# guxm2021/SVT_SpeechBrain

Measured on AMD Instinct MI355X. Metric: 10s@16kHz clips/sec encoder+CTC forward, wav2vec2-base, 1/2/4/8 MI355X, higher is better.
Workload: dtype bf16; 1 GPU; wav2vec2-base audio-only AMT forward (encoder + 20-way head + frame decode), 32 x 10 s @16 kHz mono clips per GPU; global_batch=32, per_gpu_batch=32, samples_per_clip=160000, frames_per_clip=499, parallelism=clips sharded over 1 rank(s), streams=2, inputs=resident in HBM

## Files before the change

include/svt_mi355.h:

```cpp
#ifndef SVT_MI355_H
#define SVT_MI355_H

#include <stddef.h>
#include <stdint.h>

#ifdef __cplusplus
extern "C" {
#endif

#define SVT_ABI_VERSION 1
#define SVT_MAX_CONV_LAYERS 8

typedef enum {
  SVT_OK = 0,
  SVT_ERR_INVALID = -1,
  SVT_ERR_KEY = -2,
  SVT_ERR_STATE = -3,
  SVT_ERR_WORKSPACE = -4,
  SVT_ERR_HIP = -5,
  SVT_ERR_NO_DEVICE = -6
} svt_status;

typedef enum { SVT_PREC_FP32 = 0, SVT_PREC_BF16 = 1, SVT_PREC_BF16X3 = 2, SVT_PREC_FP16X3 = 3 } svt_precision;
typedef enum { SVT_NORM_GROUP = 0, SVT_NORM_LAYER = 1 } svt_feat_norm;
typedef enum { SVT_F32 = 0 } svt_dtype;

typedef struct svt_encoder_config {
  int32_t struct_size;
  int32_t hidden_size;
  int32_t num_layers;
  int32_t num_heads;
  int32_t intermediate_size;
  int32_t num_conv_layers;
  int32_t conv_dim[SVT_MAX_CONV_LAYERS];
  int32_t conv_kernel[SVT_MAX_CONV_LAYERS];
  int32_t conv_stride[SVT_MAX_CONV_LAYERS];
  int32_t feat_extract_norm;
  int32_t conv_bias;
  int32_t stable_layer_norm;
  int32_t feat_proj_layer_norm;
  int32_t pos_conv_kernel;
  int32_t pos_conv_groups;
  float layer_norm_eps;
  int32_t normalize_wav;
  int32_t output_norm;
  int32_t precision;
  int32_t pos_conv_depth;
  int32_t rel_pos_buckets;
  int32_t rel_pos_max_distance;
  int32_t pos_conv_batch_norm;
} svt_encoder_config;

typedef struct svt_encoder svt_encoder;
typedef struct svt_linear svt_linear;
typedef struct svt_rca svt_rca;

typedef struct svt_frame {
  float p_on;
  float p_off;
  int32_t octave;
  int32_t pitch_class;
} svt_frame;

const char* svt_last_error(void);
int svt_abi_version(void);
int svt_operand_type(void);
int svt_device_count(void);

int svt_encoder_create(const svt_encoder_config* cfg, int device, svt_encoder** out);
void svt_encoder_destroy(svt_encoder* e);

typedef int (*svt_norm_reduce_fn)(double* sums_dev, int32_t n_doubles, void* stream, void* user);
int svt_encoder_set_norm_reduce(svt_encoder* enc, svt_norm_reduce_fn fn, void* user, int64_t global_clips);
int svt_encoder_load_param(svt_encoder* e, const char* key, const void* data_host, int dtype,
                           const int64_t* shape, int ndim);
int svt_encoder_finalize(svt_encoder* e);
int svt_encoder_get_param(svt_encoder* e, const char* key, void* out_host, int64_t capacity_elems);
int64_t svt_encoder_num_frames(const svt_encoder* e, int64_t n_samples);
int64_t svt_encoder_workspace_bytes(const svt_encoder* e, int32_t batch, int64_t n_samples);
int svt_encoder_forward(svt_encoder* e, const float* wav_dev, int32_t batch, int64_t n_samples,
                        float* feats_dev, void* workspace_dev, size_t workspace_bytes, void* stream);
int svt_encoder_forward_ex(svt_encoder* e, const float* wav_dev, int32_t batch, int64_t n_samples,
                           float* feats_dev, void* workspace_dev, size_t workspace_bytes, void* stream,
                           int32_t clips_per_norm_group);

int svt_encoder_forward_head(svt_encoder* enc, const svt_linear* head, const float* wav_dev, int32_t batch,
                             int64_t n_samples, float* logits_out_dev, svt_frame* frames_out_dev, int32_t n_octave,
                             int32_t n_class, void* workspace_dev, size_t workspace_bytes, void* stream,
                             int32_t clips_per_norm_group);

int svt_linear_create(int32_t in_features, int32_t out_features, int has_bias, int device, svt_linear** out);
void svt_linear_destroy(svt_linear* l);
int svt_linear_load(svt_linear* l, const float* weight_host , const float* bias_host );
int svt_linear_forward(svt_linear* l, const float* x_dev, int64_t rows, float* y_dev, void* stream);
int svt_decode_frames(const float* logits_dev, int64_t rows, int32_t n_out, int32_t n_octave,
                      int32_t n_class, svt_frame* frames_dev, int device, void* stream);
int svt_frames_to_notes(const svt_frame* frames_host, int32_t batch, int64_t frames_per_clip, const int64_t* n_frames,
                        float onset_thres, float offset_thres, double frame_size, int32_t n_octave, int32_t n_class,
                        double* t_on, double* t_off, int32_t* pitch, int32_t* lo, int32_t* hi, int64_t capacity_per_clip,
                        int64_t* n_notes);

int svt_rca_create(int32_t d_model, int32_t nhead, int32_t d_ffn, float alpha, int32_t max_len,
                   int32_t precision, int device, svt_rca** out);
void svt_rca_destroy(svt_rca* r);
int svt_rca_load_param(svt_rca* r, const char* key, const void* data_host, int dtype,
                       const int64_t* shape, int ndim);
int svt_rca_finalize(svt_rca* r);
int64_t svt_rca_workspace_bytes(const svt_rca* r, int32_t batch, int32_t t_audio);
int svt_rca_forward(svt_rca* r, const float* audio_dev, int32_t t_audio, const float* video_dev,
                    int32_t t_video, int32_t batch, float* out_dev, void* workspace_dev,
                    size_t workspace_bytes, void* stream);
int svt_rca_refresh_params(svt_rca* r, const float* const* params_dev, int32_t n, void* stream);
int64_t svt_rca_train_workspace_bytes(const svt_rca* r, int32_t batch, int32_t t_audio);
int svt_rca_forward_train(svt_rca* r, const float* audio_dev, int32_t t_audio, const float* video_dev, int32_t t_video, int32_t batch,
                          float* out_dev, void* workspace_dev, size_t workspace_bytes, void* stream);
int svt_rca_backward(svt_rca* r, const float* dout_dev, int32_t batch, int32_t t_audio, float* const* grads_dev, void* workspace_dev,
                     size_t workspace_bytes, void* stream);

int svt_ctc_greedy(const float* probs_dev, int32_t batch, int32_t t, int32_t v, const float* rel_lens_dev,
                   int32_t blank, int32_t* tokens_dev, int32_t* out_lens_dev, int device, void* stream);

int64_t svt_fbank_workspace_bytes(int32_t batch, int64_t n_samples, int32_t n_fft, int32_t hop, int32_t n_mels);
int svt_fbank(const float* wav_dev, int32_t batch, int64_t n_samples, int32_t sample_rate, int32_t n_fft,
              int32_t win_length, int32_t hop_length, int32_t n_mels, float f_min, float f_max, float top_db,
              float* out_dev, void* workspace_dev, size_t workspace_bytes, int device, void* stream);

int svt_debug_gemm(int32_t precision, const void* a_dev, const void* w_dev, void* c_dev, const float* bias_dev,
                   const float* resid_dev, int32_t m, int32_t n, int32_t k, int32_t a_rpb, int64_t a_bstride,
                   int64_t a_rstride, int64_t ldw, int32_t act, int32_t out_f32, int device, void* stream);

int svt_debug_gemm_pairs(int32_t precision, const float* a_dev, int64_t a_elems, const float* w_dev, float* c_dev, const float* bias_dev,
                         int32_t m, int32_t n, int32_t k, int32_t a_rpb, int64_t a_bstride, int64_t a_rstride, int32_t act,
                         int32_t out_kind, int device, void* stream, int32_t time_iters, float* ms_out);

typedef struct svt_debug_gemm_desc {
  int32_t struct_size;
  const void* a;
  const void* w;
  void* c;
  const float* bias;
  const float* resid;
  int32_t m, n, k;
  int32_t a_rpb;
  int64_t a_bstride, a_rstride;
  int64_t ldw, ldc;
  int32_t nz, nz2;
  int64_t a_z1, a_z2, w_z1, w_z2, c_z1, c_z2, bias_z2;
  float alpha;
  int32_t act, out_f32;
} svt_debug_gemm_desc;
int svt_debug_gemm_batched(int32_t precision, const svt_debug_gemm_desc* d, int device, void* stream);

typedef struct svt_video svt_video;
int svt_video_create(int32_t embed_dim, int32_t precision, int device, svt_video** out);
void svt_video_destroy(svt_video* v);
int svt_video_load_param(svt_video* v, const char* key, const void* data_host, int dtype, const int64_t* shape, int ndim);
int svt_video_finalize(svt_video* v);
int64_t svt_video_workspace_bytes(const svt_video* v, int32_t batch, int32_t t, int32_t h, int32_t w);
int svt_video_keep_workspace(svt_video* v, int keep);
int svt_video_forward(svt_video* v, const float* video_dev, int32_t batch, int32_t t, int32_t h, int32_t w, float* out_dev,
                      void* workspace_dev, size_t workspace_bytes, void* stream);
int svt_video_forward_ex(svt_video* v, const float* video_dev, int32_t batch, int32_t t, int32_t h, int32_t w, float* out_dev, int64_t out_ld,
                         int32_t zero_left, void* workspace_dev, size_t workspace_bytes, void* stream);
typedef struct svt_video_transform { double sub0, div0, mean, std; int32_t crop_h, crop_w; } svt_video_transform;
int svt_video_forward_u8(svt_video* v, const uint8_t* roi_dev, int32_t batch, int32_t t, int32_t h_in, int32_t w_in,
                         const svt_video_transform* tf, float* out_dev, int64_t out_ld, int32_t zero_left, void* workspace_dev,
                         size_t workspace_bytes, void* stream);

int svt_deltas(const float* x_dev, int64_t ldx, int32_t batch, int32_t t, int32_t c, int32_t window_length, float* out_dev,
               int64_t ldo, int device, void* stream);
int svt_context_window(const float* x_dev, int32_t batch, int32_t t, int32_t c, int32_t left_frames, int32_t right_frames,
                       float* out_dev, int device, void* stream);

int svt_bce_loss(const float* logits_dev, int64_t batch, int64_t t_pred, const float* targets_dev, int64_t t_tgt,
                 const float* rel_len_dev, const float* pos_weight_dev, int32_t allowed_len_diff, int32_t reduction,
                 float* out_dev, void* workspace_dev, size_t workspace_bytes, int device, void* stream);
int svt_nll_loss(const float* log_probs_dev, int64_t batch, int64_t t_pred, int32_t n_class, const int64_t* targets_dev,
                 int64_t t_tgt, const float* rel_len_dev, float label_smoothing, int32_t allowed_len_diff,
                 int32_t reduction, float* out_dev, void* workspace_dev, size_t workspace_bytes, int device, void* stream);
int svt_softmax(const float* x_dev, int64_t rows, int32_t n, int32_t apply_log, float* y_dev, int device, void* stream);

int svt_amt_objective_grad(const float* logits_dev, int64_t batch, int64_t t_pred, int32_t n_out, int32_t pitch_octave_num,
                           const float* onset_targets_dev, const float* offset_targets_dev, const int64_t* octave_targets_dev,
                           const int64_t* class_targets_dev, int64_t t_tgt, const float* rel_len_dev, float onset_pos_weight,
                           int32_t allowed_len_diff, float label_smoothing, float* terms_dev, float* terms_host, float* dlogits_dev,
                           void* workspace_dev, size_t* workspace_bytes, int device, void* stream);
int svt_linear_backward(const float* x_dev, const float* dy_dev, int64_t rows, int32_t in_features, int32_t out_features,
                        float* dweight_dev, float* dbias_dev, void* workspace_dev, size_t* workspace_bytes, int device, void* stream);
int svt_linear_backward_data(const float* dy_dev, const float* weight_dev, int64_t rows, int32_t in_features, int32_t out_features,
                             float* dx_dev, int device, void* stream);
int svt_clip_adadelta_step(int32_t n_tensors, float* const* params_dev, float* const* grads_dev, float* const* square_avg_dev,
                           float* const* acc_delta_dev, const int64_t* numels, float lr, double rho, float eps, float weight_decay,
                           int32_t maximize, float max_norm, float* total_norm_dev, void* workspace_dev, size_t* workspace_bytes,
                           int device, void* stream);

int svt_debug_attention(int32_t precision, const void* q, const void* k, const void* v, void* o, int32_t batch, int32_t t,
                        int32_t heads, int32_t head_dim, int64_t ldq, int64_t ldkv, int64_t ldo, float scale, int device,
                        void* stream);
int svt_debug_attention_bias(const void* q, const void* k, const void* v, void* o, int32_t batch, int32_t t, int32_t heads, int64_t ldq,
                             int64_t ldkv, int64_t ldo, float scale, const float* gate_dev, const float* pos_bias_dev, int device,
                             void* stream);
int svt_debug_attention_scores(int32_t precision, const void* q, const void* k, const void* v, void* o, int32_t batch, int32_t t,
                               int32_t heads, int32_t head_dim, int64_t ldq, int64_t ldkv, int64_t ldo, float scale,
                               const float* gate_dev, const float* pos_bias_dev, int device, void* stream);
int svt_debug_rca_wgrad(int32_t precision, const float* dy0, int64_t ldy0, const void* x0, const float* dy1, int64_t ldy1, const void* x1,
                        int64_t rows, int32_t n_out, int32_t n_in, float* dw, float* db, void* workspace_dev, size_t* workspace_bytes,
                        int device, void* stream);
int svt_debug_rca_attn_bwd(int32_t precision, const void* qkv, const void* qc, const void* o_self, const void* o_cross,
                           const float* dblend, float alpha, int32_t batch, int32_t t, int32_t heads, int32_t head_dim, float* dqkv,
                           float* dqc, void* workspace_dev, size_t* workspace_bytes, int device, void* stream);
int svt_debug_set(int key, int value);

int svt_prof_enable(int on);
int svt_prof_reset(void);
int svt_prof_read(int kind, int64_t* launches, double* total_ms, double* total_flops, double* total_bytes);
int svt_debug_clock(int64_t* out_dev, int device, void* stream);
int svt_debug_alloc(void** out, size_t bytes, int device);
int svt_debug_encoder_layout(const svt_encoder* e, int32_t batch, int64_t n_samples, int64_t* offsets, int n);
int svt_debug_free(void* p, int device);

#ifdef __cplusplus
}
#endif
#endif
```

svt_speechbrain_amd/_lib.py:

```python
from __future__ import annotations

import ctypes as C
import os
from typing import Optional

_HERE = os.path.dirname(os.path.abspath(__file__))
LIB_PATH = os.environ.get("SVT_LIB_PATH") or os.path.join(_HERE, "libsvt_mi355.so")
MAX_CONV = 8


class SvtError(RuntimeError):
    pass


class EncoderConfigC(C.Structure):
    _fields_ = [
        ("struct_size", C.c_int32),
        ("hidden_size", C.c_int32),
        ("num_layers", C.c_int32),
        ("num_heads", C.c_int32),
        ("intermediate_size", C.c_int32),
        ("num_conv_layers", C.c_int32),
        ("conv_dim", C.c_int32 * MAX_CONV),
        ("conv_kernel", C.c_int32 * MAX_CONV),
        ("conv_stride", C.c_int32 * MAX_CONV),
        ("feat_extract_norm", C.c_int32),
        ("conv_bias", C.c_int32),
        ("stable_layer_norm", C.c_int32),
        ("feat_proj_layer_norm", C.c_int32),
        ("pos_conv_kernel", C.c_int32),
        ("pos_conv_groups", C.c_int32),
        ("layer_norm_eps", C.c_float),
        ("normalize_wav", C.c_int32),
        ("output_norm", C.c_int32),
        ("precision", C.c_int32),
        ("pos_conv_depth", C.c_int32),
        ("rel_pos_buckets", C.c_int32),
        ("rel_pos_max_distance", C.c_int32),
        ("pos_conv_batch_norm", C.c_int32),
    ]


class VideoTransformC(C.Structure):
    _fields_ = [("sub0", C.c_double), ("div0", C.c_double), ("mean", C.c_double), ("std", C.c_double), ("crop_h", C.c_int32), ("crop_w", C.c_int32)]


class GemmDescC(C.Structure):
    _fields_ = [
        ("struct_size", C.c_int32),
        ("a", C.c_void_p), ("w", C.c_void_p), ("c", C.c_void_p), ("bias", C.c_void_p), ("resid", C.c_void_p),
        ("m", C.c_int32), ("n", C.c_int32), ("k", C.c_int32),
        ("a_rpb", C.c_int32),
        ("a_bstride", C.c_int64), ("a_rstride", C.c_int64),
        ("ldw", C.c_int64), ("ldc", C.c_int64),
        ("nz", C.c_int32), ("nz2", C.c_int32),
        ("a_z1", C.c_int64), ("a_z2", C.c_int64), ("w_z1", C.c_int64), ("w_z2", C.c_int64), ("c_z1", C.c_int64), ("c_z2", C.c_int64),
        ("bias_z2", C.c_int64),
        ("alpha", C.c_float),
        ("act", C.c_int32), ("out_f32", C.c_int32),
    ]


class FrameC(C.Structure):
    _fields_ = [("p_on", C.c_float), ("p_off", C.c_float), ("octave", C.c_int32), ("pitch_class", C.c_int32)]


_P = C.c_void_p
_I64P = C.POINTER(C.c_int64)
NORM_REDUCE_FN = C.CFUNCTYPE(C.c_int, C.c_void_p, C.c_int32, C.c_void_p, C.c_void_p)

SYMBOLS = {
    "svt_last_error": (C.c_char_p, []),
    "svt_abi_version": (C.c_int, []),
    "svt_device_count": (C.c_int, []),
    "svt_encoder_create": (C.c_int, [C.POINTER(EncoderConfigC), C.c_int, C.POINTER(_P)]),
    "svt_encoder_destroy": (None, [_P]),
    "svt_encoder_load_param": (C.c_int, [_P, C.c_char_p, _P, C.c_int, _I64P, C.c_int]),
    "svt_encoder_finalize": (C.c_int, [_P]),
    "svt_encoder_get_param": (C.c_int, [_P, C.c_char_p, _P, C.c_int64]),
    "svt_encoder_num_frames": (C.c_int64, [_P, C.c_int64]),
    "svt_encoder_workspace_bytes": (C.c_int64, [_P, C.c_int32, C.c_int64]),
    "svt_encoder_forward": (C.c_int, [_P, _P, C.c_int32, C.c_int64, _P, _P, C.c_size_t, _P]),
    "svt_encoder_forward_ex": (C.c_int, [_P, _P, C.c_int32, C.c_int64, _P, _P, C.c_size_t, _P, C.c_int32]),
    "svt_encoder_forward_head": (C.c_int, [_P, _P, _P, C.c_int32, C.c_int64, _P, _P, C.c_int32, C.c_int32, _P, C.c_size_t, _P, C.c_int32]),
    "svt_linear_create": (C.c_int, [C.c_int32, C.c_int32, C.c_int, C.c_int, C.POINTER(_P)]),
    "svt_linear_destroy": (None, [_P]),
    "svt_linear_load": (C.c_int, [_P, _P, _P]),
    "svt_linear_forward": (C.c_int, [_P, _P, C.c_int64, _P, _P]),
    "svt_decode_frames": (C.c_int, [_P, C.c_int64, C.c_int32, C.c_int32, C.c_int32, _P, C.c_int, _P]),
    "svt_rca_create": (C.c_int, [C.c_int32, C.c_int32, C.c_int32, C.c_float, C.c_int32, C.c_int32, C.c_int, C.POINTER(_P)]),
    "svt_rca_destroy": (None, [_P]),
    "svt_rca_load_param": (C.c_int, [_P, C.c_char_p, _P, C.c_int, _I64P, C.c_int]),
    "svt_rca_finalize": (C.c_int, [_P]),
    "svt_rca_workspace_bytes": (C.c_int64, [_P, C.c_int32, C.c_int32]),
    "svt_rca_forward": (C.c_int, [_P, _P, C.c_int32, _P, C.c_int32, C.c_int32, _P, _P, C.c_size_t, _P]),
    "svt_rca_refresh_params": (C.c_int, [_P, C.POINTER(_P), C.c_int32, _P]),
    "svt_rca_train_workspace_bytes": (C.c_int64, [_P, C.c_int32, C.c_int32]),
    "svt_rca_forward_train": (C.c_int, [_P, _P, C.c_int32, _P, C.c_int32, C.c_int32, _P, _P, C.c_size_t, _P]),
    "svt_rca_backward": (C.c_int, [_P, _P, C.c_int32, C.c_int32, C.POINTER(_P), _P, C.c_size_t, _P]),
    "svt_ctc_greedy": (C.c_int, [_P, C.c_int32, C.c_int32, C.c_int32, _P, C.c_int32, _P, _P, C.c_int, _P]),
    "svt_fbank_workspace_bytes": (C.c_int64, [C.c_int32, C.c_int64, C.c_int32, C.c_int32, C.c_int32]),
    "svt_fbank": (C.c_int, [_P, C.c_int32, C.c_int64, C.c_int32, C.c_int32, C.c_int32, C.c_int32, C.c_int32,
                            C.c_float, C.c_float, C.c_float, _P, _P, C.c_size_t, C.c_int, _P]),
    "svt_debug_gemm": (C.c_int, [C.c_int32, _P, _P, _P, _P, _P, C.c_int32, C.c_int32, C.c_int32, C.c_int32, C.c_int64,
                                 C.c_int64, C.c_int64, C.c_int32, C.c_int32, C.c_int, _P]),
    "svt_debug_gemm_batched": (C.c_int, [C.c_int32, C.POINTER(GemmDescC), C.c_int, _P]),
    "svt_debug_attention_scores": (C.c_int, [C.c_int32, _P, _P, _P, _P, C.c_int32, C.c_int32, C.c_int32, C.c_int32, C.c_int64, C.c_int64,
                                             C.c_int64, C.c_float, _P, _P, C.c_int, _P]),
    "svt_debug_gemm_pairs": (C.c_int, [C.c_int32, _P, C.c_int64, _P, _P, _P, C.c_int32, C.c_int32, C.c_int32, C.c_int32, C.c_int64,
                                       C.c_int64, C.c_int32, C.c_int32, C.c_int, _P, C.c_int32, C.POINTER(C.c_float)]),
    "svt_video_create": (C.c_int, [C.c_int32, C.c_int32, C.c_int, C.POINTER(C.c_void_p)]),
    "svt_video_destroy": (None, [C.c_void_p]),
    "svt_video_load_param": (C.c_int, [C.c_void_p, C.c_char_p, C.c_void_p, C.c_int, C.POINTER(C.c_int64), C.c_int]),
    "svt_video_finalize": (C.c_int, [C.c_void_p]),
    "svt_video_keep_workspace": (C.c_int, [C.c_void_p, C.c_int]),
    "svt_video_workspace_bytes": (C.c_int64, [C.c_void_p, C.c_int32, C.c_int32, C.c_int32, C.c_int32]),
    "svt_video_forward": (C.c_int, [C.c_void_p, C.c_void_p, C.c_int32, C.c_int32, C.c_int32, C.c_int32, C.c_void_p, C.c_void_p,
                                    C.c_size_t, C.c_void_p]),
    "svt_video_forward_ex": (C.c_int, [C.c_void_p, C.c_void_p, C.c_int32, C.c_int32, C.c_int32, C.c_int32, C.c_void_p, C.c_int64, C.c_int32,
                                       C.c_void_p, C.c_size_t, C.c_void_p]),
    "svt_video_forward_u8": (C.c_int, [C.c_void_p, C.c_void_p, C.c_int32, C.c_int32, C.c_int32, C.c_int32, C.POINTER(VideoTransformC),
                                       C.c_void_p, C.c_int64, C.c_int32, C.c_void_p, C.c_size_t, C.c_void_p]),
    "svt_deltas": (C.c_int, [C.c_void_p, C.c_int64, C.c_int32, C.c_int32, C.c_int32, C.c_int32, C.c_void_p, C.c_int64, C.c_int, C.c_void_p]),
    "svt_context_window": (C.c_int, [C.c_void_p, C.c_int32, C.c_int32, C.c_int32, C.c_int32, C.c_int32, C.c_void_p, C.c_int, C.c_void_p]),
    "svt_bce_loss": (C.c_int, [C.c_void_p, C.c_int64, C.c_int64, C.c_void_p, C.c_int64, C.c_void_p, C.c_void_p, C.c_int32,
                               C.c_int32, C.c_void_p, C.c_void_p, C.c_size_t, C.c_int, C.c_void_p]),
    "svt_nll_loss": (C.c_int, [C.c_void_p, C.c_int64, C.c_int64, C.c_int32, C.c_void_p, C.c_int64, C.c_void_p, C.c_float,
                               C.c_int32, C.c_int32, C.c_void_p, C.c_void_p, C.c_size_t, C.c_int, C.c_void_p]),
    "svt_softmax": (C.c_int, [C.c_void_p, C.c_int64, C.c_int32, C.c_int32, C.c_void_p, C.c_int, C.c_void_p]),
    "svt_amt_objective_grad": (C.c_int, [_P, C.c_int64, C.c_int64, C.c_int32, C.c_int32, _P, _P, _P, _P, C.c_int64, _P, C.c_float,
                                         C.c_int32, C.c_float, _P, C.POINTER(C.c_float), _P, _P, C.POINTER(C.c_size_t), C.c_int, _P]),
    "svt_linear_backward": (C.c_int, [_P, _P, C.c_int64, C.c_int32, C.c_int32, _P, _P, _P, C.POINTER(C.c_size_t), C.c_int, _P]),
    "svt_linear_backward_data": (C.c_int, [_P, _P, C.c_int64, C.c_int32, C.c_int32, _P, C.c_int, _P]),
    "svt_clip_adadelta_step": (C.c_int, [C.c_int32, C.POINTER(_P), C.POINTER(_P), C.POINTER(_P), C.POINTER(_P), _I64P, C.c_float,
                                         C.c_double, C.c_float, C.c_float, C.c_int32, C.c_float, _P, _P, C.POINTER(C.c_size_t), C.c_int,
                                         _P]),
    "svt_debug_attention": (C.c_int, [C.c_int32, C.c_void_p, C.c_void_p, C.c_void_p, C.c_void_p, C.c_int32, C.c_int32,
                                      C.c_int32, C.c_int32, C.c_int64, C.c_int64, C.c_int64, C.c_float, C.c_int, C.c_void_p]),
    "svt_debug_attention_bias": (C.c_int, [C.c_void_p, C.c_void_p, C.c_void_p, C.c_void_p, C.c_int32, C.c_int32, C.c_int32, C.c_int64,
                                           C.c_int64, C.c_int64, C.c_float, C.c_void_p, C.c_void_p, C.c_int, C.c_void_p]),
    "svt_debug_rca_wgrad": (C.c_int, [C.c_int32, _P, C.c_int64, _P, _P, C.c_int64, _P, C.c_int64, C.c_int32, C.c_int32, _P, _P, _P,
                                      C.POINTER(C.c_size_t), C.c_int, _P]),
    "svt_debug_rca_attn_bwd": (C.c_int, [C.c_int32, _P, _P, _P, _P, _P, C.c_float, C.c_int32, C.c_int32, C.c_int32, C.c_int32, _P, _P,
                                         _P, C.POINTER(C.c_size_t), C.c_int, _P]),
    "svt_debug_set": (C.c_int, [C.c_int, C.c_int]),
    "svt_debug_clock": (C.c_int, [C.c_void_p, C.c_int, C.c_void_p]),
    "svt_debug_encoder_layout": (C.c_int, [C.c_void_p, C.c_int32, C.c_int64, C.POINTER(C.c_int64), C.c_int]),
    "svt_operand_type": (C.c_int, []),
    "svt_encoder_set_norm_reduce": (C.c_int, [_P, C.c_void_p, C.c_void_p, C.c_int64]),
    "svt_frames_to_notes": (C.c_int, [C.c_void_p, C.c_int32, C.c_int64, C.c_void_p, C.c_float, C.c_float, C.c_double, C.c_int32, C.c_int32,
                                      C.c_void_p, C.c_void_p, C.c_void_p, C.c_void_p, C.c_void_p, C.c_int64, C.c_void_p]),
    "svt_debug_alloc": (C.c_int, [C.POINTER(C.c_void_p), C.c_size_t, C.c_int]),
    "svt_debug_free": (C.c_int, [C.c_void_p, C.c_int]),
    "svt_prof_enable": (C.c_int, [C.c_int]),
    "svt_prof_reset": (C.c_int, []),
    "svt_prof_read": (C.c_int, [C.c_int, _I64P, C.POINTER(C.c_double), C.POINTER(C.c_double), C.POINTER(C.c_double)]),
}

_lib: Optional[C.CDLL] = None
_libs: dict = {}


def load(variant: str = None) -> C.CDLL:
    global _lib
    key = variant or ""
    if key in _libs:
        return _libs[key]
    if not variant and os.environ.get("SVT_LIB_SUFFIX"):
        variant_path = LIB_PATH.replace("libsvt_mi355.so", f"libsvt_mi355_{os.environ['SVT_LIB_SUFFIX']}.so")
        if not os.path.exists(variant_path):
            raise SvtError(f"SVT_LIB_SUFFIX: {variant_path} not found")
        globals()["LIB_PATH"] = variant_path
    root, ext = os.path.splitext(LIB_PATH)
    path = LIB_PATH if not variant else f"{root}_{variant}{ext}"
    if not os.path.exists(path):
        raise SvtError(
            f"{path} not found: build it with `python -c 'import __graft_entry__ as g; g.build()'` "
            "(or `make -C svt_speechbrain_amd/csrc`). The MI355X path has no CPU fallback.")
    lib = C.CDLL(path)
    for name, (res, args) in SYMBOLS.items():
        fn = getattr(lib, name)
        fn.restype = res
        fn.argtypes = args
    if lib.svt_abi_version() != 1:
        raise SvtError(f"{os.path.basename(path)} ABI version mismatch")
    if lib.svt_operand_type() != (1 if variant == "f16" else 0):
        raise SvtError(f"{os.path.basename(path)} was built for another operand type")
    _libs[key] = lib
    if not variant:
        _lib = lib
    return lib


def last_error(lib: C.CDLL = None) -> str:
    return ((lib or load()).svt_last_error() or b"").decode("utf-8", "replace")


def check(rc: int, what: str = "", lib: C.CDLL = None) -> None:
    if rc != 0:
        raise SvtError(f"{what}: {last_error(lib)} (status {rc})")


def require_gpu() -> None:
    lib = load()
    if lib.svt_device_count() < 1:
        raise SvtError("no gfx950 (MI355X) device is visible: the HIP path cannot run and there is no CPU fallback")


def stream_ptr(device) -> int:
    import torch
    return int(torch.cuda.current_stream(device).cuda_stream)


def dev_index(device) -> int:
    import torch
    d = torch.device(device)
    if d.type != "cuda":
        raise SvtError(f"tensors must live on a ROCm device ('cuda:N'), got {d}")
    return d.index if d.index is not None else torch.cuda.current_device()


def ptr(t) -> int:
    return int(t.data_ptr())
```

svt_speechbrain_amd/csrc/api.hip:

```cpp
#include "../../include/svt_mi355.h"
#include "api.h"
#include "common.h"
#include "host.h"

#include <atomic>
#include <cmath>
#include <cstring>
#include <map>
#include <mutex>
#include <string>
#include <vector>

namespace svt {

int hip_fail(hipError_t e, const char* what, const char* file, int line) {
  set_error(std::string("HIP error ") + hipGetErrorName(e) + " (" + hipGetErrorString(e) + ") at " + file + ":" +
          std::to_string(line) + " in " + what);
  return SVT_ERR_HIP;
}

struct ProfState {
  bool on = false;
  int every = 1;
  unsigned tick = 0;
// ... 136 lines not shown
int begin_upload(bool& uploaded) {
  if (uploaded) SVT_HIP(hipDeviceSynchronize());
  uploaded = true;
  return SVT_OK;
}

bool use_flash(int prec, int dh, bool bias, int64_t T) {
  if (!(prec == 1 && (dh == 64 || dh == 128))) return false;
  return !bias || (dh == 64 && 2 * T - 1 <= 8192);
}
int attn_tp(int prec, int dh, int T, bool bias) {
  return use_flash(prec, dh, bias, T) ? round_up_int(T, 64) : round_up_int(T, 8);
}

int attention_scores_path(int prec, const void* Q, long ldq, const void* K, const void* V, long ldkv, int B,
                          int T, int H, int dh, float scale, const AttnBufs& ab, bool vt_ready, void* out,
                          long ldo, hipStream_t s, const float* gate, const float* relpb, int gp, int o_pairs) {
  if (gp < 0) gp = prec;
  if (gp >= 2 && !gate && flash_attention_x3_ok(dh) && ab.pl_qkv && ldkv == 3L * H * dh &&
      (const float*)V == (const float*)K + (long)H * dh) {
    const long D = (long)H * dh, rows = (long)B * T;
    const float* kv0 = (const float*)K - D;
    const long pl3 = rows * 3 * D;
    unsigned short* p3 = (unsigned short*)ab.pl_qkv;
    if (!vt_ready)
      if (int r = launch_split_planes(gp, kv0, 3 * D, rows, (int)(3 * D), p3, 3 * D, pl3, s)) return r;
    const unsigned short* qp;
    long qld, qpl;
    if ((const float*)Q == kv0 && ldq == 3 * D) { qp = p3; qld = 3 * D; qpl = pl3; }
    else {
      if (!ab.pl_q) { set_error("attention: no workspace for the query planes"); return -1; }
      if (int r = launch_split_planes(gp, (const float*)Q, ldq, rows, (int)D, ab.pl_q, D, rows * D, s)) return r;
      qp = (const unsigned short*)ab.pl_q; qld = D; qpl = rows * D;
    }
    return launch_flash_attention_x3(gp, qp, qld, (long)T * qld, qpl, p3 + D, p3 + 2 * D, 3 * D, (long)T * 3 * D, pl3, (float*)out, ldo,
                                     (long)T * ldo, B, T, H, dh, scale, s, o_pairs);
  }
  if (o_pairs) { set_error("attention: pair-row output is served by the fused split attention only"); return -1; }
  if (use_flash(prec, dh, gate != nullptr, T)) {
    (void)vt_ready;
    return launch_flash_attention(Q, ldq, (long)T * ldq, K, V, ldkv, (long)T * ldkv, out, ldo, (long)T * ldo, B, T, H, dh,
                                  scale, s, gate, gate ? relpb : nullptr);
  }
  const int Tp = round_up_int(T, 8);
  GemmArgs g;
  g.A = Q; g.W = K; g.C = ab.S;
  g.M = T; g.N = T; g.K = dh;
  g.a_rpb = T; g.a_bstride = 0; g.a_rstride = ldq;
  g.ldw = ldkv; g.ldc = Tp;
  g.nz = B * H; g.nz2 = H;
  g.a_z1 = (long)T * ldq; g.a_z2 = dh;
  g.w_z1 = (long)T * ldkv; g.w_z2 = dh;
  g.c_z1 = (long)H * T * Tp; g.c_z2 = (long)T * Tp;
  g.alpha = scale; g.out_f32 = 1;
  if (int r = launch_gemm(gp, g, s)) return r;
  if (gate)
    if (int r = launch_scores_add_relbias(ab.S, (int64_t)B * H, H, T, Tp, gate, relpb, s)) return r;
  if (int r = launch_softmax_rows(prec, ab.S, (int64_t)B * H * T, T, Tp, ab.P, s)) return r;
  if (!vt_ready)
    if (int r = launch_transpose_v(prec, V, B, T, H, dh, ldkv, 0, Tp, ab.Vt, s)) return r;
  GemmArgs o;
  o.A = ab.P; o.W = ab.Vt; o.C = out;
  o.M = T; o.N = dh; o.K = Tp;
  o.a_rpb = T; o.a_rstride = Tp;
  o.ldw = Tp; o.ldc = ldo;
  o.nz = B * H; o.nz2 = H;
  o.a_z1 = (long)H * T * Tp; o.a_z2 = (long)T * Tp;
  o.w_z1 = (long)H * dh * Tp; o.w_z2 = (long)dh * Tp;
  o.c_z1 = (long)T * ldo; o.c_z2 = dh;
  return launch_gemm(gp, o, s);
}

int check_device(int device) {
  int n = 0;
  if (hipGetDeviceCount(&n) != hipSuccess || n <= 0) { set_error("no HIP device visible: the MI355X path cannot run (there is no CPU fallback)"); return SVT_ERR_NO_DEVICE; }
  if (device < 0 || device >= n) { set_error("device index out of range"); return SVT_ERR_INVALID; }
  hipDeviceProp_t prop;
  SVT_HIP(hipGetDeviceProperties(&prop, device));
  if (std::string(prop.gcnArchName).find("gfx950") == std::string::npos) {
    set_error(std::string("device arch is ") + prop.gcnArchName + ", this library is built for gfx950 only");
    return SVT_ERR_NO_DEVICE;
  }
  SVT_HIP(hipSetDevice(device));
  return SVT_OK;
}

int ws_query(const char* who, void* ws, size_t* ws_bytes, size_t need, bool* query) {
  *query = false;
  if (!ws_bytes) { set_error(std::string(who) + ": workspace_bytes is null"); return SVT_ERR_INVALID; }
  if (!ws) { *ws_bytes = need; *query = true; return SVT_OK; }
  if (*ws_bytes < need) {
    set_error(std::string(who) + ": workspace too small (need " + std::to_string(need) + " bytes)");
    return SVT_ERR_WORKSPACE;
  }
  return SVT_OK;
}

int g_debug_keep_split = 0;

}

using namespace svt;

extern "C" {

int svt_abi_version(void) { return SVT_ABI_VERSION; }
int svt_operand_type(void) {
#ifdef SVT_OPERAND_F16
  return 1;
#else
  return 0;
#endif
}
int svt_device_count(void) {
  int n = 0;
  if (hipGetDeviceCount(&n) != hipSuccess) return 0;
  int ok = 0;
  for (int i = 0; i < n; ++i) {
    hipDeviceProp_t prop;
    if (hipGetDeviceProperties(&prop, i) == hipSuccess && std::string(prop.gcnArchName).find("gfx950") != std::string::npos) ++ok;
  }
  return ok;
}

int svt_debug_gemm(int32_t precision, const void* a, const void* w, void* c, const float* bias, const float* resid,
                   int32_t m, int32_t n, int32_t k, int32_t a_rpb, int64_t a_bstride, int64_t a_rstride, int64_t ldw,
                   int32_t act, int32_t out_f32, int device, void* stream) {
  if (!a || !w || !c) { set_error("svt_debug_gemm: null argument"); return SVT_ERR_INVALID; }
  SVT_HIP(hipSetDevice(device));
  GemmArgs g;
  g.A = a; g.W = w; g.C = c; g.bias = bias; g.resid = resid;
  g.M = m; g.N = n; g.K = k; g.a_rpb = a_rpb; g.a_bstride = a_bstride; g.a_rstride = a_rstride;
  g.ldw = ldw; g.ldc = n; g.act = act; g.out_f32 = out_f32;
  static const void* s_kept = nullptr;
  const bool split = precision >= 2 && ldw == k && k % 32 == 0;
  if (split && !(g_debug_keep_split && s_kept == w)) {
    if (split_weights_register(w, n, k, precision, (hipStream_t)stream)) return SVT_ERR_HIP;
    s_kept = w;
  }
  const int rc = launch_gemm(precision, g, (hipStream_t)stream);
  if (split && !g_debug_keep_split) {
    SVT_HIP(hipStreamSynchronize((hipStream_t)stream));
    split_weights_forget(w);
    s_kept = nullptr;
  }
  return rc ? SVT_ERR_INVALID : SVT_OK;
}

int svt_debug_gemm_batched(int32_t precision, const svt_debug_gemm_desc* d, int device, void* stream) {
  if (!d || d->struct_size != (int32_t)sizeof(svt_debug_gemm_desc)) { set_error("svt_debug_gemm_batched: struct_size"); return SVT_ERR_INVALID; }
  if (!d->a || !d->w || !d->c) { set_error("svt_debug_gemm_batched: null argument"); return SVT_ERR_INVALID; }
  if (!valid_precision(precision)) { set_error("svt_debug_gemm_batched: precision"); return SVT_ERR_INVALID; }
  if (d->nz < 1 || d->nz2 < 1 || d->k < 1) { set_error("svt_debug_gemm_batched: nz, nz2 and k must be positive"); return SVT_ERR_INVALID; }
  SVT_HIP(hipSetDevice(device));
  GemmArgs g;
  g.A = d->a; g.W = d->w; g.C = d->c; g.bias = d->bias; g.resid = d->resid;
  g.M = d->m; g.N = d->n; g.K = d->k; g.a_rpb = d->a_rpb; g.a_bstride = d->a_bstride; g.a_rstride = d->a_rstride;
  g.ldw = d->ldw; g.ldc = d->ldc;
  g.nz = d->nz; g.nz2 = d->nz2;
  g.a_z1 = d->a_z1; g.a_z2 = d->a_z2; g.w_z1 = d->w_z1; g.w_z2 = d->w_z2; g.c_z1 = d->c_z1; g.c_z2 = d->c_z2; g.bias_z2 = d->bias_z2;
  g.alpha = d->alpha; g.act = d->act; g.out_f32 = d->out_f32;
  const bool split = precision >= 2 && d->ldw == d->k && d->k % 32 == 0 && d->w_z1 >= 0 && d->w_z2 >= 0;
  if (split) {
    const size_t last_z_row = d->nz > 1 ? ((size_t)(d->nz / d->nz2 - 1) * d->w_z1 + (size_t)(d->nz2 - 1) * d->w_z2) / (size_t)d->k : 0;
    if (split_weights_register(d->w, (long)last_z_row + d->n, d->k, precision, (hipStream_t)stream)) return SVT_ERR_HIP;
  }
  const int rc = launch_gemm(precision, g, (hipStream_t)stream);
  if (split) {
    SVT_HIP(hipStreamSynchronize((hipStream_t)stream));
    split_weights_forget(d->w);
  }
  return rc ? SVT_ERR_INVALID : SVT_OK;
}

int svt_debug_gemm_pairs(int32_t precision, const float* a, int64_t a_elems, const float* w, float* c, const float* bias, int32_t m,
                         int32_t n, int32_t k, int32_t a_rpb, int64_t a_bstride, int64_t a_rstride, int32_t act, int32_t out_kind,
                         int device, void* stream, int32_t time_iters, float* ms_out) {
  if (!a || !w || !c) { set_error("svt_debug_gemm_pairs: null argument"); return SVT_ERR_INVALID; }
  if ((precision != SVT_PREC_BF16X3 && precision != SVT_PREC_FP16X3) || !valid_precision(precision)) {
    set_error("svt_debug_gemm_pairs: split-operand precisions only (they live in libsvt_mi355.so, not in the IEEE-half build)"); return SVT_ERR_INVALID; }
  if (out_kind < 0 || out_kind > 2 || a_elems % 32 || ((int64_t)m * n) % 32) { set_error("svt_debug_gemm_pairs: out_kind / sizes"); return SVT_ERR_INVALID; }
  SVT_HIP(hipSetDevice(device));
  hipStream_t s = (hipStream_t)stream;
  void *ap = nullptr, *cp = nullptr;
  hipEvent_t e0 = nullptr, e1 = nullptr;
  static std::mutex s_mu;
  static const void* s_kept = nullptr;
  std::lock_guard<std::mutex> lock(s_mu);
  bool registered = false;
  auto hip_ok = [](hipError_t e, const char* what) -> int {
    if (e == hipSuccess) return 0;
    set_error(std::string(what) + ": " + hipGetErrorString(e));
    return 1;
  };
  int rc = dev_alloc(&ap, (size_t)a_elems * 4);
  if (!rc && out_kind) rc = dev_alloc(&cp, (size_t)m * n * 4);
  if (!rc) rc = launch_f32_to_pairs(precision, a, ap, a_elems, s);
  if (!rc && !(g_debug_keep_split && s_kept == w)) {
    rc = split_weights_register(w, n, k, precision, s);
    if (!rc) { s_kept = w; registered = true; }
  } else if (!rc) {
    registered = true;
  }
  if (!rc) {
    GemmArgs g;
    g.A = ap; g.W = w; g.C = out_kind == 1 ? cp : (void*)c; g.bias = bias;
    g.M = m; g.N = n; g.K = k; g.a_rpb = a_rpb; g.a_bstride = a_bstride; g.a_rstride = a_rstride;
    g.ldw = k; g.ldc = n; g.act = act; g.out_f32 = 1; g.a_pairs = 1; g.c_pairs = out_kind == 1;
    if (out_kind == 2) { g.planes = (unsigned short*)cp; g.plane_stride = (long)m * n; }
    rc = launch_gemm(precision, g, s);
    if (!rc && time_iters > 0 && ms_out) {
      rc = hip_ok(hipEventCreate(&e0), "hipEventCreate") || hip_ok(hipEventCreate(&e1), "hipEventCreate") ||
           hip_ok(hipEventRecord(e0, s), "hipEventRecord");
      for (int i = 0; i < time_iters && !rc; ++i) rc = launch_gemm(precision, g, s);
      float ms = 0.f;
      if (!rc) rc = hip_ok(hipEventRecord(e1, s), "hipEventRecord") || hip_ok(hipEventSynchronize(e1), "hipEventSynchronize") ||
                    hip_ok(hipEventElapsedTime(&ms, e0, e1), "hipEventElapsedTime");
      if (!rc) *ms_out = ms / (float)time_iters;
    }
  }
  if (!rc && out_kind == 1) rc = launch_pairs_to_f32(precision, cp, nullptr, c, (int64_t)m * n, s);
  if (!rc && out_kind == 2) rc = launch_pairs_to_f32(precision, cp, (const unsigned short*)cp + (size_t)m * n, c, (int64_t)m * n, s);
  (void)hipStreamSynchronize(s);
  if (e0) (void)hipEventDestroy(e0);
  if (e1) (void)hipEventDestroy(e1);
  if (registered && !g_debug_keep_split) { split_weights_forget(w); s_kept = nullptr; }
  if (ap) dev_free(ap);
  if (cp) dev_free(cp);
  return rc ? SVT_ERR_INVALID : SVT_OK;
}

int svt_debug_attention(int32_t precision, const void* q, const void* k, const void* v, void* o, int32_t batch, int32_t t,
                        int32_t heads, int32_t head_dim, int64_t ldq, int64_t ldkv, int64_t ldo, float scale, int device,
                        void* stream) {
  if (!q || !k || !v || !o) { set_error("svt_debug_attention: null argument"); return SVT_ERR_INVALID; }
  if (!(precision >= 1 && precision <= 3) || !(head_dim == 64 || head_dim == 128)) {
    set_error("svt_debug_attention: only the fused kernels (bf16, or the split-operand modes on fp32 inputs; head_dim 64 / 128) are exposed"); return SVT_ERR_INVALID; }
  if (int r = check_device(device)) return r;
  SVT_HIP(hipSetDevice(device));
  if (precision >= 2) {
    const long D = (long)heads * head_dim, rows = (long)batch * t;
    if ((const float*)k != (const float*)q + D || (const float*)v != (const float*)q + 2 * D || ldq != 3 * D || ldkv != 3 * D) {
      set_error("svt_debug_attention: the split-operand kernel is exposed for a packed q|k|v projection"); return SVT_ERR_INVALID; }
    void* planes = nullptr;
    if (int r = dev_alloc(&planes, (size_t)rows * 3 * D * 4)) return r;
    AttnBufs ab{};
    ab.pl_qkv = planes;
    const int rc = attention_scores_path(0, q, ldq, k, v, ldkv, batch, t, heads, head_dim, scale, ab, false, o, ldo, (hipStream_t)stream,
                                         nullptr, nullptr, precision);
    (void)hipStreamSynchronize((hipStream_t)stream);
    dev_free(planes);
    return rc ? SVT_ERR_INVALID : SVT_OK;
  }
  if (launch_flash_attention(q, ldq, (long)t * ldq, k, v, ldkv, (long)t * ldkv, o, ldo, (long)t * ldo, batch, t, heads,
                             head_dim, scale, (hipStream_t)stream)) return SVT_ERR_INVALID;
  return SVT_OK;
}

int svt_debug_attention_bias(const void* q, const void* k, const void* v, void* o, int32_t batch, int32_t t, int32_t heads, int64_t ldq,
                             int64_t ldkv, int64_t ldo, float scale, const float* gate_dev, const float* pos_bias_dev, int device,
                             void* stream) {
  if (!q || !k || !v || !o || !gate_dev || !pos_bias_dev) { set_error("svt_debug_attention_bias: null argument"); return SVT_ERR_INVALID; }
  if (batch < 1 || t < 1 || heads < 1) { set_error("svt_debug_attention_bias: batch, t and heads must be positive"); return SVT_ERR_INVALID; }
  if (int r = check_device(device)) return r;
  SVT_HIP(hipSetDevice(device));
  if (launch_flash_attention(q, ldq, (long)t * ldq, k, v, ldkv, (long)t * ldkv, o, ldo, (long)t * ldo, batch, t, heads, 64, scale,
                             (hipStream_t)stream, gate_dev, pos_bias_dev)) return SVT_ERR_INVALID;
  return SVT_OK;
}

int svt_debug_attention_scores(int32_t precision, const void* q, const void* k, const void* v, void* o, int32_t batch, int32_t t,
                               int32_t heads, int32_t head_dim, int64_t ldq, int64_t ldkv, int64_t ldo, float scale,
                               const float* gate_dev, const float* pos_bias_dev, int device, void* stream) {
  if (!q || !k || !v || !o) { set_error("svt_debug_attention_scores: null argument"); return SVT_ERR_INVALID; }
  if (!valid_precision(precision)) { set_error("svt_debug_attention_scores: precision"); return SVT_ERR_INVALID; }
  if (batch < 1 || t < 1 || heads < 1 || head_dim < 1) { set_error("svt_debug_attention_scores: batch, t, heads and head_dim must be positive"); return SVT_ERR_INVALID; }
  if (!gate_dev != !pos_bias_dev) { set_error("svt_debug_attention_scores: gate and pos_bias come together"); return SVT_ERR_INVALID; }
  if (use_flash(precision, head_dim, gate_dev != nullptr, t)) {
    set_error("svt_debug_attention_scores: this geometry runs the fused kernel (svt_debug_attention / svt_debug_attention_bias)"); return SVT_ERR_INVALID; }
  if (int r = check_device(device)) return r;
  SVT_HIP(hipSetDevice(device));
  hipStream_t s = (hipStream_t)stream;
  const int prec = storage_prec(precision);
  const int Tp = attn_tp(precision, head_dim, t, gate_dev != nullptr);
  const size_t bh = (size_t)batch * heads;
  const size_t bytes[3] = {bh * t * Tp * 4, bh * t * Tp * esize(prec), bh * head_dim * Tp * esize(prec)};
  void* buf[3] = {nullptr, nullptr, nullptr};
  int rc = 0;
  for (int i = 0; i < 3 && !rc; ++i) {
    rc = dev_alloc(&buf[i], bytes[i]);
    if (!rc && hipMemsetAsync(buf[i], 0xFF, bytes[i], s) != hipSuccess) { set_error("svt_debug_attention_scores: hipMemsetAsync"); rc = SVT_ERR_HIP; }
  }
  if (!rc) {
    AttnBufs ab{};
    ab.S = (float*)buf[0]; ab.P = buf[1]; ab.Vt = buf[2];
    rc = attention_scores_path(prec, q, ldq, k, v, ldkv, batch, t, heads, head_dim, scale, ab, false, o, ldo, s, gate_dev, pos_bias_dev,
                               precision) ? SVT_ERR_INVALID : SVT_OK;
  }
  (void)hipStreamSynchronize(s);
  for (int i = 0; i < 3; ++i) dev_free(buf[i]);
  return rc;
}

int svt_debug_set(int key, int value) {
  if (key == 0) g_gemm_dbg = value;
  else if (key == 1) g_gemm_force_bm = value;
  else if (key == 2) g_gemm_ring = value;
  else if (key == 3) g_gemm_variant = value;
  else if (key == 5) {  }
  else if (key == 6) g_gemm_skinny = value;
  else if (key == 7) g_gemm_skinny_max_tiles = value;
  else if (key == 8) g_flash_wide = value;
  else if (key == 9) g_conv_ln_bf16 = value;
  else if (key == 10) {  }
  else if (key == 11) g_gemm_x3 = value;
  else if (key == 12) g_debug_keep_split = value;
  else if (key == 13) g_guard_alloc = value;
  else if (key == 15) g_stamp_ends = value;
  else if (key == 16) {  }
  else if (key == 18) {  }
  else if (key == 19) g_x3_pairs = value;
  else if (key == 20) g_ln_two_rows = value;
  else if (key == 21) {
    if (value != 0 && value != 3) { set_error("svt_debug_set(21): the attention A/B arms are retired"); return SVT_ERR_INVALID; }
  }
  else if (key == 22) g_conv0_mfma = value;
  else if (key == 23) g_conv3x3_c64 = value;
  else if (key == 24) return g_conv3x3_c64_launches;
  else if (key == 25) g_conv3x3_c64_form = value;
  else if (key == 26) g_stem_pool_fused = value;
  else if (key == 27) g_conv_down_fused = value;
  else if (key == 28) {
    if (value != 0) { set_error("svt_debug_set(28): the two-slot schedule is retired"); return SVT_ERR_INVALID; }
  }
  else if (key == 29) g_gemm_p1w = value;
  else if (key == 30) {
#ifndef SVT_DIAG
    if (value != 0) { set_error("svt_debug_set(30): gemm_p1x_kernel is built by `make DIAG=1` only"); return SVT_ERR_INVALID; }
#endif
    g_gemm_p1x = value;
  }
  else if (key == 31) return g_dev_frees.load(std::memory_order_relaxed);
  else if (key == 32) return set_ticket_fenced(value);
  else if (key == 33) g_gemm_skinny_small_tiles = value;
  else if (key == 34) g_gemm_walk = value;
  else if (key == 35) g_conv_kperm = value;
  else if (key == 36) g_ffn2_ksplit = value;
  else if (key == 37) { if (value < 8 || value > 256 || value % 8) { set_error("svt_debug_set(37): 8 .. 256, a multiple of 8"); return SVT_ERR_INVALID; } g_gemm_persist_wgs = value; }
  else if (key == 38) return g_flash_kernel_id;
  else if (key == 39) return g_gemm_kernel_id;
  else { set_error("svt_debug_set: unknown key"); return SVT_ERR_INVALID; }
  return SVT_OK;
}

int svt_debug_alloc(void** out, size_t bytes, int device) {
  if (!out) { set_error("svt_debug_alloc: null argument"); return SVT_ERR_INVALID; }
  if (int r = check_device(device)) return r;
  SVT_HIP(hipSetDevice(device));
  return dev_alloc(out, bytes);
}
int svt_debug_free(void* p, int device) {
  if (int r = check_device(device)) return r;
  SVT_HIP(hipSetDevice(device));
  dev_free(p);
  return SVT_OK;
}

int svt_debug_clock(int64_t* out_dev, int device, void* stream) {
  if (!out_dev) { set_error("svt_debug_clock: null argument"); return SVT_ERR_INVALID; }
  SVT_HIP(hipSetDevice(device));
  return launch_clock_stamp((long long*)out_dev, (hipStream_t)stream) ? SVT_ERR_HIP : SVT_OK;
}

int svt_prof_enable(int on) { g_prof.on = on != 0; g_prof.every = on > 1 ? on : 1; g_prof.tick = 0; return SVT_OK; }
int svt_prof_reset(void) {
  g_prof.used = 0;
  for (int k = 0; k < 3; ++k) g_prof.flops[k] = g_prof.bytes[k] = 0;
  return SVT_OK;
}
int svt_prof_read(int kind, int64_t* launches, double* total_ms, double* total_flops, double* total_bytes) {
  if (kind < 0 || kind > 2) { set_error("svt_prof_read: kind must be 0..2"); return SVT_ERR_INVALID; }
  double ms = 0;
  int64_t n = 0;
  for (size_t i = 0; i < g_prof.used; ++i) {
    if (g_prof.kind[i] != kind) continue;
    SVT_HIP(hipEventSynchronize(g_prof.ev[i].second));
    float t = 0;
    SVT_HIP(hipEventElapsedTime(&t, g_prof.ev[i].first, g_prof.ev[i].second));
    ms += t;
    ++n;
  }
  if (launches) *launches = n;
  if (total_ms) *total_ms = ms;
  if (total_flops) *total_flops = g_prof.flops[kind];
  if (total_bytes) *total_bytes = g_prof.bytes[kind];
  return SVT_OK;
}

}
```

svt_speechbrain_amd/csrc/api_encoder.hip:

```cpp
#include "../../include/svt_mi355.h"
#include "api.h"
#include "common.h"
#include "host.h"

#include <cmath>
#include <cstring>
#include <string>
#include <vector>

using namespace svt;

int svt::g_conv_ln_bf16 = 1;

struct ConvLayerW {
  DevBuf w;
  DevBuf w_kperm;
  DevBuf bias;
  DevBuf gamma, beta;
};
struct EncLayerW {
  DevBuf wqkv, bqkv, wo, bo, ln1g, ln1b, w1, b1, w2, b2, ln2g, ln2b;
  DevBuf g_wab, g_bab, g_const;
};

// ... 308 lines not shown

static const size_t kKsplitMaxRows = 2048;

EncWs carve_encoder(const svt_encoder* e, int B, int64_t L, void* base) {
  const svt_encoder_config& c = e->cfg;
  const int sp = storage_prec(c.precision);
  const size_t es = esize(sp);
  Carver cv(base);
  EncWs w;
  {
    const int64_t t1 = c.num_conv_layers > 0 ? (L - c.conv_kernel[0]) / c.conv_stride[0] + 1 : 1;
    w.mom_scr[0] = align_up((4 * (size_t)B + (size_t)B * 65) * sizeof(double));
    w.mom_scr[1] = w.mom_scr[0] + align_up(moments_scratch_bytes(B));
    w.mom_scr[2] = w.mom_scr[1] + align_up(moments_scratch_bytes(B));
    w.mom_scr[3] = w.mom_scr[2] + align_up(conv0_window_moments_scratch_bytes(B, t1 > 0 ? t1 : 1));
    w.mom_zero = w.mom_scr[3] + 256;
    int64_t t = L;
    for (int i = 0; i < c.num_conv_layers; ++i) t = (t - c.conv_kernel[i]) / c.conv_stride[i] + 1;
    w.mom_bytes = w.mom_scr[3] + align_up(head_scratch_bytes((int64_t)B * (t > 0 ? t : 1), B));
  }
  w.mom = (double*)cv.take(w.mom_bytes);
  w.coef = (float*)cv.take((size_t)B * c.conv_dim[0] * 11 * 4);
  w.c0tab = (sp || c.precision >= 2) ? cv.take(conv0_mfma_table_bytes(B)) : nullptr;
  size_t max_act = 0, max_f = 0;
  int64_t t = L;
  for (int i = 0; i < c.num_conv_layers; ++i) {
    t = (t - c.conv_kernel[i]) / c.conv_stride[i] + 1;
    const size_t n = (size_t)B * t * c.conv_dim[i];
    if (n * es > max_act) max_act = n * es;
    if (i > 0 && n * 4 > max_f) max_f = n * 4;
  }
  const int64_t T = t;
  if (c.num_conv_layers == 0) max_act = (size_t)B * T * c.conv_dim[0] * es;
  w.act[0] = cv.take(max_act);
  w.act[1] = cv.take(max_act);
  w.convF = c.feat_extract_norm == SVT_NORM_LAYER ? (float*)cv.take(max_f) : nullptr;
  const int D = c.hidden_size, F = c.intermediate_size, H = c.num_heads, dh = D / H;
  const size_t rows = (size_t)B * T;
  const int Tp = attn_tp(sp, dh, (int)T, c.rel_pos_buckets > 0);
  const bool flash = use_flash(sp, dh, c.rel_pos_buckets > 0, (int64_t)T);
  w.xln = cv.take(rows * c.conv_dim[c.num_conv_layers > 0 ? c.num_conv_layers - 1 : 0] * es);
  w.hF = (float*)cv.take(rows * D * 4);
  w.preF = (float*)cv.take(rows * D * 4);
  w.xb = cv.take(rows * D * es);
  w.xF = (sp || c.precision >= 2) ? (float*)cv.take(rows * D * 4) : (float*)w.xb;
  w.xlo = sp ? cv.take(rows * D * 2) : nullptr;
  {
    const int Pf = e->pos_P;
    const size_t Tq = Pf ? (T + Pf - 1) / Pf : 0;
    const size_t Tp = Pf ? Tq * Pf + c.pos_conv_kernel : (size_t)(T + c.pos_conv_kernel);
    w.posg = cv.take((size_t)B * Tp * D * es);
    w.posy = Pf ? cv.take((size_t)B * Tq * Pf * D * es) : nullptr;
  }
  w.qkv = cv.take(rows * 3 * D * es);
  const bool flash3 = c.precision >= 2 && flash_attention_x3_ok(dh) && !c.rel_pos_buckets;
  w.ab.S = (flash || flash3) ? nullptr : (float*)cv.take((size_t)B * H * T * Tp * 4);
  w.ab.P = (flash || flash3) ? nullptr : cv.take((size_t)B * H * T * Tp * es);
  w.ab.Vt = cv.take((size_t)B * H * dh * Tp * es);
  w.ab.pl_qkv = (c.precision >= 2 && flash_attention_x3_ok(dh) && !c.rel_pos_buckets) ? cv.take(rows * 3 * D * 4) : nullptr;
  w.attn_o = cv.take(rows * D * es);
  w.ffn = cv.take(rows * F * es);
  w.gate = c.rel_pos_buckets ? (float*)cv.take((size_t)B * H * T * 4) : nullptr;
  w.relpb = c.rel_pos_buckets ? (float*)cv.take((size_t)H * (2 * T - 1) * 4) : nullptr;
  w.dots = (float*)cv.take(rows * 32 * 4);
  w.ksplit = (sp && rows <= kKsplitMaxRows) ? (float*)cv.take((size_t)4 * rows * D * 4) : nullptr;
  w.total = cv.off;
  return w;
}

struct TailSpec {
  float* feats = nullptr;
  const svt_linear* head = nullptr;
  float* logits = nullptr;
  svt_frame* frames = nullptr;
  int n_oct = 0, n_cls = 0;
};

}

extern "C" {

int svt_debug_encoder_layout(const svt_encoder* e, int32_t batch, int64_t n_samples, int64_t* offsets, int n) {
  if (!e || batch < 1 || !offsets || n < 1) { set_error("svt_debug_encoder_layout: bad argument"); return SVT_ERR_INVALID; }
  if (svt_encoder_num_frames(e, n_samples) < 1) { set_error("waveform shorter than the receptive field"); return SVT_ERR_INVALID; }
  char* const fake = (char*)(uintptr_t)(1ull << 40);
  const EncWs w = carve_encoder(e, batch, n_samples, fake);
  const void* r[24] = {w.mom, w.coef, w.c0tab, w.act[0], w.act[1], w.convF, w.xln, w.hF, w.preF, w.xb, w.xF, w.xlo, w.posg, w.posy, w.qkv,
                       w.ab.S, w.ab.P, w.ab.Vt, w.ab.pl_qkv, w.attn_o, w.ffn, w.gate, w.relpb, w.dots};
  int k = 0;
  for (; k < 24 && k < n; ++k) offsets[k] = r[k] == nullptr ? -1 : (int64_t)((const char*)r[k] - fake);
  if (k < n) offsets[k++] = (int64_t)w.total;
  return k;
}

int64_t svt_encoder_workspace_bytes(const svt_encoder* e, int32_t batch, int64_t n_samples) {
  if (!e || batch < 1) { set_error("workspace_bytes: bad argument"); return -1; }
  if (svt_encoder_num_frames(e, n_samples) < 1) { set_error("waveform shorter than the receptive field"); return -1; }
  return (int64_t)carve_encoder(e, batch, n_samples, nullptr).total;
}

}

static int encoder_forward_impl(svt_encoder* e, const float* wav, int32_t B, int64_t L, const TailSpec& tail, void* workspace,
                                size_t workspace_bytes, void* stream, int32_t clips_per_norm_group);

extern "C" {

int svt_encoder_forward(svt_encoder* e, const float* wav, int32_t B, int64_t L, float* feats, void* workspace,
                        size_t workspace_bytes, void* stream) {
  return svt_encoder_forward_ex(e, wav, B, L, feats, workspace, workspace_bytes, stream, 0);
}

int svt_encoder_forward_ex(svt_encoder* e, const float* wav, int32_t B, int64_t L, float* feats, void* workspace,
                           size_t workspace_bytes, void* stream, int32_t clips_per_norm_group) {
  if (!feats) { set_error("encoder_forward: null argument"); return SVT_ERR_INVALID; }
  TailSpec t;
  t.feats = feats;
  return encoder_forward_impl(e, wav, B, L, t, workspace, workspace_bytes, stream, clips_per_norm_group);
}

int svt_encoder_forward_head(svt_encoder* e, const svt_linear* head, const float* wav, int32_t B, int64_t L, float* logits,
                             svt_frame* frames, int32_t n_octave, int32_t n_class, void* workspace, size_t workspace_bytes,
                             void* stream, int32_t clips_per_norm_group) {
  if (!head || !logits) { set_error("encoder_forward_head: null argument"); return SVT_ERR_INVALID; }
  if (!head->loaded) { set_error("encoder_forward_head: head weights not loaded"); return SVT_ERR_STATE; }
  if (!e || head->in_f != e->cfg.hidden_size || head->device != e->device) {
    set_error("encoder_forward_head: the head must take hidden_size inputs and live on the encoder's device"); return SVT_ERR_INVALID; }
  if (!linear_head_eligible(head->in_f, head->out_f)) {
    set_error("encoder_forward_head: the fused tail is built for hidden sizes 512 / 768 / 1024 and at most 32 outputs"); return SVT_ERR_INVALID; }
  if (frames && head->out_f != 2 + n_octave + 1 + n_class + 1) {
    set_error("encoder_forward_head: n_out != 2 + (n_octave+1) + (n_class+1)"); return SVT_ERR_INVALID; }
  TailSpec t;
  t.head = head; t.logits = logits; t.frames = frames; t.n_oct = n_octave; t.n_cls = n_class;
  return encoder_forward_impl(e, wav, B, L, t, workspace, workspace_bytes, stream, clips_per_norm_group);
}

}

static int encoder_forward_impl(svt_encoder* e, const float* wav, int32_t B, int64_t L, const TailSpec& tail, void* workspace,
                                size_t workspace_bytes, void* stream, int32_t clips_per_norm_group) {
  float* feats = tail.feats;
  if (!e || !wav || !workspace) { set_error("encoder_forward: null argument"); return SVT_ERR_INVALID; }
  if (!e->finalized) { set_error("encoder_forward: parameters not finalized"); return SVT_ERR_STATE; }
  if (B < 1) { set_error("encoder_forward: batch < 1"); return SVT_ERR_INVALID; }
  const int64_t T = svt_encoder_num_frames(e, L);
  if (T < 1) { set_error("encoder_forward: waveform shorter than the receptive field"); return SVT_ERR_INVALID; }
  const svt_encoder_config& c = e->cfg;
  const int prec = storage_prec(c.precision);
  const int gp = c.precision;
  EncWs w = carve_encoder(e, B, L, workspace);
  if (w.total > workspace_bytes) { set_error("encoder_forward: workspace too small (" + std::to_string(workspace_bytes) + " < " + std::to_string(w.total) + ")"); return SVT_ERR_WORKSPACE; }
  hipStream_t s = (hipStream_t)stream;
  SVT_HIP(hipSetDevice(e->device));
  const int cpg = clips_per_norm_group > 0 ? clips_per_norm_group : B;
  if (B % cpg) { set_error("encoder_forward: batch must be a multiple of clips_per_norm_group"); return SVT_ERR_INVALID; }
  const int groups = B / cpg;
  if (groups > 1 && c.num_conv_layers > 0 && (L & 3)) {
    set_error("encoder_forward: norm groups need a waveform length that is a multiple of 4 samples");
    return SVT_ERR_INVALID;
  }
  if (groups > 1 && c.num_conv_layers == 0 && c.normalize_wav) {
    set_error("encoder_forward: features-in mode has no input norm to group");
    return SVT_ERR_INVALID;
  }
  if (launch_zero_bytes(w.mom, w.mom_zero, s)) return SVT_ERR_HIP;
  double* wav_mom = c.normalize_wav ? w.mom : nullptr;
  double* out_mom = w.mom + 2 * (size_t)B;
  double* wm = w.mom + 4 * (size_t)B;
  int64_t n_wav = (int64_t)cpg * L;
  if (c.normalize_wav)
    if (int r = launch_moments(wav, n_wav, wav_mom, (char*)w.mom + w.mom_scr[0], B, s, groups)) return r;
  struct ReduceCtx { svt_encoder* e; double* mom; hipStream_t s; } rctx{e, nullptr, s};
  auto reduce_now = [](void* a) -> int {
    ReduceCtx* rc = (ReduceCtx*)a;
    if (rc->e->reduce_fn(rc->mom, 2, (void*)rc->s, rc->e->reduce_user)) { set_error("encoder_forward: the norm-reduce callback reported an error"); return SVT_ERR_INVALID; }
    return 0;
  };
  const bool global_norm = e->reduce_fn != nullptr;
  if (global_norm) {
    if (groups != 1) { set_error("encoder_forward: the cross-rank norm reduction applies to whole-batch norms (clips_per_norm_group = 0)"); return SVT_ERR_INVALID; }
    if (e->reduce_global_clips < B) { set_error("encoder_forward: global_clips of the norm reduction is smaller than this batch"); return SVT_ERR_INVALID; }
    if (c.normalize_wav) {
      rctx.mom = wav_mom;
      if (int r = reduce_now(&rctx)) return r;
      n_wav = e->reduce_global_clips * L;
    }
  }

  const int pk_mode = (gp >= 2 && g_x3_pairs && g_gemm_x3) ? gp : 0;
  auto x3q_fits = [&](const void* A, int M, int N, int K, int a_rpb, long a_bstride, long a_rstride, const void* Wp, int c_pairs, long ldc) -> bool {
    GemmArgs g;
    g.A = A; g.W = Wp; g.C = const_cast<void*>(A); g.M = M; g.N = N; g.K = K; g.a_rpb = a_rpb; g.a_bstride = a_bstride; g.a_rstride = a_rstride;
    g.ldw = K; g.ldc = ldc; g.a_pairs = 1; g.c_pairs = c_pairs;
    return gemm_x3q_eligible(g);
  };
  bool pk_front_ok = pk_mode != 0 && c.num_conv_layers >= 2 && c.conv_dim[0] % 32 == 0 && c.conv_dim[0] <= 512 && c.conv_stride[0] <= 5;
  if (pk_front_ok) {
    int64_t ti_ = (L - c.conv_kernel[0]) / c.conv_stride[0] + 1;
    for (int i = 1; i < c.num_conv_layers && pk_front_ok; ++i) {
      const int cin = c.conv_dim[i - 1], co = c.conv_dim[i], k = c.conv_kernel[i], st = c.conv_stride[i];
      const int64_t to_ = (ti_ - k) / st + 1;
      if ((int64_t)B * to_ > 2147483647LL) { pk_front_ok = false; break; }
      pk_front_ok = x3q_fits(w.act[0], (int)((int64_t)B * to_), co, k * cin, (int)to_, ti_ * cin, (long)st * cin, e->conv[i].w.p, 1, co) &&
                    (c.feat_extract_norm != SVT_NORM_LAYER || co == 512 || co == 768 || co == 1024);
      ti_ = to_;
    }
    const int Cl = c.conv_dim[c.num_conv_layers - 1];
    const int64_t rows_ = (int64_t)B * T;
    pk_front_ok = pk_front_ok && x3q_fits(w.xln, (int)rows_, c.hidden_size, Cl, (int)rows_, 0, Cl, e->proj_w.p, 0, c.hidden_size) &&
                  (!c.feat_proj_layer_norm || Cl == 512 || Cl == 768 || Cl == 1024);
  }
  const int pk_front = pk_front_ok ? pk_mode : 0;

  int64_t tin = L;
  int cur = 0;
  if (c.num_conv_layers == 0) {
    const int64_t n = (int64_t)B * L * c.conv_dim[0];
    if (prec) { if (int r = launch_f32_to_bf16(wav, (bf16_t*)w.act[0], n, s)) return r; }
    else if (launch_copy_f32(wav, (float*)w.act[0], n, s)) return SVT_ERR_HIP;
  } else {
  int64_t t1 = (L - c.conv_kernel[0]) / c.conv_stride[0] + 1;
  const ConvLayerW& c0 = e->conv[0];
  if (c.feat_extract_norm == SVT_NORM_GROUP) {
    if (int r = launch_conv0_window_moments(wav, B, L, c.conv_kernel[0], c.conv_stride[0], t1, wm, (char*)w.mom + w.mom_scr[2], s)) return r;
    if (int r = launch_conv0_group_coef(wav_mom, n_wav, wm, B, t1, c.conv_dim[0], c.conv_kernel[0], c0.w.as<float>(),
                                        c.conv_bias ? c0.bias.as<float>() : nullptr, c0.gamma.as<float>(),
                                        c0.beta.as<float>(), 1e-5f, 1e-5f, w.coef, s, cpg)) return r;
    if (conv0_mfma_ok(prec, pk_front, c.conv_kernel[0], c.conv_stride[0], c.conv_dim[0]) && w.c0tab) {
      if (int r = launch_conv0_mfma_group(wav, B, L, c.conv_stride[0], t1, w.coef, w.c0tab, w.act[0], s, pk_front)) return r;
    } else
    if (int r = launch_conv0_group_apply(prec, wav, B, L, c.conv_kernel[0], c.conv_stride[0], t1, c.conv_dim[0], w.coef,
                                         w.act[0], s, pk_front)) return r;
  } else {
    if (conv0_mfma_ok(prec, pk_front, c.conv_kernel[0], c.conv_stride[0], c.conv_dim[0]) && w.c0tab) {
      if (int r = launch_conv0_mfma_layer(wav, B, L, c.conv_stride[0], t1, wav_mom, n_wav, 1e-5f, c0.w.as<float>(),
                                          c.conv_bias ? c0.bias.as<float>() : nullptr, c0.gamma.as<float>(), c0.beta.as<float>(), 1e-5f,
                                          w.c0tab, w.act[0], s, cpg, pk_front)) return r;
    } else
    if (int r = launch_conv0_layer(prec, wav, B, L, c.conv_kernel[0], c.conv_stride[0], t1, c.conv_dim[0], wav_mom, n_wav,
                                   1e-5f, c0.w.as<float>(), c.conv_bias ? c0.bias.as<float>() : nullptr,
                                   c0.gamma.as<float>(), c0.beta.as<float>(), 1e-5f, w.act[0], s, cpg, pk_front)) return r;
  }
  tin = t1;
  }
  for (int i = 1; i < c.num_conv_layers; ++i) {
    const int cin = c.conv_dim[i - 1], co = c.conv_dim[i], k = c.conv_kernel[i], st = c.conv_stride[i];
    const int64_t tout = (tin - k) / st + 1;
    const ConvLayerW& Lw = e->conv[i];
    GemmArgs g;
    g.A = w.act[cur]; g.W = Lw.w.p;
    g.M = (int)((int64_t)B * tout); g.N = co; g.K = k * cin;
    g.a_rpb = (int)tout; g.a_bstride = tin * cin; g.a_rstride = (long)st * cin;
    g.ldw = g.K; g.ldc = co;
    if (Lw.w_kperm.p) { g.W_kperm = Lw.w_kperm.p; g.kperm_taps = k; g.kperm_cin = cin; }
    g.bias = c.conv_bias ? Lw.bias.as<float>() : nullptr;
    if ((int64_t)B * tout > 2147483647LL) { set_error("encoder_forward: batch*frames exceeds 2^31"); return SVT_ERR_INVALID; }
    g.a_pairs = pk_front ? 1 : 0;
    const bool pairs_out = pk_front && !(i + 1 == c.num_conv_layers && c.feat_proj_layer_norm);
    if (pk_front && c.feat_extract_norm == SVT_NORM_LAYER) {
      g.C = w.convF; g.out_f32 = 1; g.act = ACT_NONE;
      if (int r = launch_gemm(gp, g, s)) return r;
      if (int r = launch_layernorm(prec, w.convF, 1, (int64_t)B * tout, co, Lw.gamma.as<float>(), Lw.beta.as<float>(), 1e-5f, 1,
                                   pairs_out ? nullptr : w.act[cur ^ 1], nullptr, s, nullptr, nullptr, pairs_out ? w.act[cur ^ 1] : nullptr,
                                   pk_front)) return r;
    } else if (pk_front) {
      g.C = w.act[cur ^ 1]; g.act = ACT_GELU; g.out_f32 = 1; g.c_pairs = pairs_out ? 1 : 0;
      if (int r = launch_gemm(gp, g, s)) return r;
    } else
    if (c.feat_extract_norm == SVT_NORM_LAYER && prec && co == 512 && g_conv_ln_bf16) {
      g.C = w.act[cur ^ 1]; g.out_f32 = 0; g.act = ACT_NONE;
      if (int r = launch_gemm(gp, g, s)) return r;
      if (int r = launch_layernorm(prec, w.act[cur ^ 1], 0, (int64_t)B * tout, co, Lw.gamma.as<float>(), Lw.beta.as<float>(),
                                   1e-5f, 1, w.act[cur ^ 1], nullptr, s)) return r;
    } else if (c.feat_extract_norm == SVT_NORM_LAYER) {
      g.C = w.convF; g.out_f32 = 1; g.act = ACT_NONE;
      if (int r = launch_gemm(gp, g, s)) return r;
      if (int r = launch_layernorm(prec, w.convF, 1, (int64_t)B * tout, co, Lw.gamma.as<float>(), Lw.beta.as<float>(),
                                   1e-5f, 1, w.act[cur ^ 1], nullptr, s)) return r;
    } else {
      g.C = w.act[cur ^ 1]; g.act = ACT_GELU;
      if (int r = launch_gemm(gp, g, s)) return r;
    }
    cur ^= 1;
    tin = tout;
  }
  const int C = c.conv_dim[c.num_conv_layers > 0 ? c.num_conv_layers - 1 : 0];
  const int D = c.hidden_size, F = c.intermediate_size, H = c.num_heads, dh = D / H;
  const int64_t rows = (int64_t)B * T;
  const float eps = c.layer_norm_eps;

  const void* proj_in = w.act[cur];
  if (c.feat_proj_layer_norm) {
    if (int r = launch_layernorm(prec, w.act[cur], prec ? 0 : 1, rows, C, e->fp_g.as<float>(), e->fp_b.as<float>(), eps, 0,
                                 pk_front ? nullptr : w.xln, nullptr, s, nullptr, nullptr, pk_front ? w.xln : nullptr, pk_front)) return r;
    proj_in = w.xln;
  }
  {
    GemmArgs g;
    g.A = proj_in; g.W = e->proj_w.p; g.C = w.hF; g.bias = e->proj_b.as<float>();
    g.M = (int)rows; g.N = D; g.K = C; g.a_rpb = (int)rows; g.a_rstride = C; g.ldw = C; g.ldc = D; g.out_f32 = 1;
    g.a_pairs = pk_front ? 1 : 0;
    if (int r = launch_gemm(gp, g, s)) return r;
  }
  {
    const int kp = c.pos_conv_kernel, G = c.pos_conv_groups, cg = D / G;
    const int Pf = e->pos_P;
    const float* bn_sc = c.pos_conv_batch_norm ? e->pos_bn_sc.as<float>() : nullptr;
    const float* bn_sh = c.pos_conv_batch_norm ? e->pos_bn_sh.as<float>() : nullptr;
    if (c.pos_conv_depth > 1) {
      const float* cur = w.hF;
      float* lnout = w.xF;
      for (int i = 0; i < c.pos_conv_depth; ++i) {
        if (int r = launch_posconv_gather(prec, cur, B, (int)T, D, G, kp, (int)T + kp, w.posg, s)) return r;
        GemmArgs g;
        g.A = w.posg; g.W = e->pos_ws[i].p; g.C = w.preF; g.bias = e->pos_bs[i].as<float>();
        g.M = (int)T; g.N = cg; g.K = kp * cg;
        g.a_rpb = (int)T; g.a_rstride = cg;
        g.ldw = g.K; g.ldc = D;
        g.nz = B * G; g.nz2 = G;
        g.a_z1 = (long)G * (T + kp) * cg; g.a_z2 = (long)(T + kp) * cg;
        g.w_z1 = 0; g.w_z2 = (long)cg * g.K;
        g.c_z1 = (long)T * D; g.c_z2 = cg; g.bias_z2 = cg;
        g.act = ACT_NONE; g.out_f32 = 1;
        if (int r = launch_gemm(gp, g, s)) return r;
        if (int r = launch_layernorm(prec, w.preF, 1, rows, D, e->ones.as<float>(), e->zeros.as<float>(), 1e-5f, 1, nullptr,
                                     lnout, s)) return r;
        cur = lnout;
      }
      if (int r = launch_add_f32(w.hF, cur, w.preF, rows * (int64_t)D, s)) return r;
    } else if (Pf && (int64_t)B * ((T + Pf - 1) / Pf) >= 128) {
      const int Tq = (int)((T + Pf - 1) / Pf), Tp = Tq * Pf + kp;
      if (int r = launch_posconv_gather(prec, w.hF, B, (int)T, D, G, kp, Tp, w.posg, s, bn_sc, bn_sh)) return r;
      GemmArgs g;
      g.A = w.posg; g.W = e->pos_wP.p; g.C = w.posy; g.bias = e->pos_bP.as<float>();
      g.M = B * Tq; g.N = Pf * cg; g.K = (kp + Pf - 1) * cg;
      g.a_rpb = Tq; g.a_bstride = (long)G * Tp * cg; g.a_rstride = (long)Pf * cg;
      g.ldw = g.K; g.ldc = g.N;
      g.nz = G; g.nz2 = G;
      g.a_z2 = (long)Tp * cg; g.w_z2 = (long)g.N * g.K; g.c_z2 = (long)B * Tq * g.N; g.bias_z2 = g.N;
      g.act = ACT_GELU; g.out_f32 = 0;
      if (int r = launch_gemm(gp, g, s)) return r;
      if (int r = launch_posconv_scatter_add(w.hF, w.posy, B, (int)T, D, G, Pf, Tq, w.preF, s, prec ? 0 : 1)) return r;
    } else {
    if (int r = launch_posconv_gather(prec, w.hF, B, (int)T, D, G, kp, (int)T + kp, w.posg, s, bn_sc, bn_sh)) return r;
    GemmArgs g;
    g.A = w.posg; g.W = e->pos_w.p; g.C = w.preF; g.bias = e->pos_b.as<float>(); g.resid = w.hF;
    g.M = (int)T; g.N = cg; g.K = kp * cg;
    g.a_rpb = (int)T; g.a_rstride = cg;
    g.ldw = g.K; g.ldc = D;
    g.nz = B * G; g.nz2 = G;
    g.a_z1 = (long)G * (T + kp) * cg; g.a_z2 = (long)(T + kp) * cg;
    g.w_z1 = 0; g.w_z2 = (long)cg * g.K;
    g.c_z1 = (long)T * D; g.c_z2 = cg; g.bias_z2 = cg;
    g.act = ACT_GELU; g.out_f32 = 1;
    if (int r = launch_gemm(gp, g, s)) return r;
    }
  }
  const float scale = 1.0f / std::sqrt((float)dh);
  if (c.rel_pos_buckets)
    if (int r = launch_relpos_table(e->rel_embed.as<float>(), H, (int)T, c.rel_pos_buckets, c.rel_pos_max_distance, w.relpb, s)) return r;
  const bool qkv_planes = gp >= 2 && !c.rel_pos_buckets && flash_attention_x3_ok(dh) && w.ab.pl_qkv != nullptr;
  unsigned short* const qkv_pl = qkv_planes ? (unsigned short*)w.ab.pl_qkv : nullptr;
  const bool pk_enc_ok = pk_mode != 0 && qkv_planes && c.num_layers > 0 && (D == 512 || D == 768 || D == 1024) && dh % 32 == 0 &&
                         x3q_fits(w.xb, (int)rows, 3 * D, D, (int)rows, 0, D, e->layers[0].wqkv.p, 0, 3 * D) &&
                         x3q_fits(w.attn_o, (int)rows, D, D, (int)rows, 0, D, e->layers[0].wo.p, 0, D) &&
                         x3q_fits(w.xb, (int)rows, F, D, (int)rows, 0, D, e->layers[0].w1.p, 1, F) &&
                         x3q_fits(w.ffn, (int)rows, D, F, (int)rows, 0, F, e->layers[0].w2.p, 0, D);
  const int pk_enc = pk_enc_ok ? pk_mode : 0;
  if (!prec && !pk_enc) w.xF = (float*)w.xb;
  int cur_layer = 0;
  auto attention = [&](void) -> int {
    const float* gate = nullptr;
    if (c.rel_pos_buckets) {
      const EncLayerW& Lg = e->layers[cur_layer];
      if (int r = launch_relpos_gate(prec, w.xb, rows, (int)T, H, dh, Lg.g_wab.as<float>(), Lg.g_bab.as<float>(),
                                     Lg.g_const.as<float>(), w.gate, s)) return r;
      gate = w.gate;
    }
    ++cur_layer;
    return attention_scores_path(prec, w.qkv, 3L * D, (const char*)w.qkv + (size_t)D * esize(prec),
                                 (const char*)w.qkv + (size_t)2 * D * esize(prec), 3L * D, B, (int)T, H, dh, scale, w.ab,
                                 qkv_planes, w.attn_o, D, s, gate, w.relpb, gp, pk_enc ? 1 : 0);
  };
  auto gemm_rows = [&](const void* A, int K, const DevBuf& W, const DevBuf& bias, int N, void* Cout, int out_f32, int act,
                       const float* resid, unsigned short* planes = nullptr, int c_pairs = 0) -> int {
    GemmArgs g;
    g.A = A; g.W = W.p; g.C = Cout; g.bias = bias.as<float>(); g.resid = resid;
    g.M = (int)rows; g.N = N; g.K = K; g.a_rpb = (int)rows; g.a_rstride = K; g.ldw = K; g.ldc = N;
    g.out_f32 = out_f32; g.act = act;
    g.planes = planes; g.plane_stride = (long)rows * N;
    g.a_pairs = pk_enc ? 1 : 0; g.c_pairs = c_pairs;
    return launch_gemm(gp, g, s);
  };

  float* final_x = nullptr;
  float* tmp = w.hF;
  const bool vecD = (D == 512 || D == 768 || D == 1024);
  const int tmp_f32 = (prec && vecD) ? 0 : 1;
  if (!c.stable_layer_norm && prec && layernorm_hilo_ok(D) && c.num_layers > 0) {
    bf16_t* xh = (bf16_t*)w.xb;
    bf16_t* xl = (bf16_t*)w.xlo;
    if (int r = launch_layernorm_hilo(nullptr, nullptr, nullptr, w.preF, rows, D, e->enc_g.as<float>(), e->enc_b.as<float>(), eps,
                                      xh, xl, nullptr, s)) return r;
    bool ffn2_split = false;
    if (g_ffn2_ksplit && w.ksplit && gp == 1 && F % 256 == 0 && F >= 2048 && g_ln_two_rows) {
      GemmArgs g;
      g.A = w.ffn; g.W = e->layers[0].w2.p; g.C = tmp; g.M = (int)rows; g.N = D; g.K = F; g.a_rpb = (int)rows; g.a_rstride = F; g.ldw = F; g.ldc = D;
      ffn2_split = g_gemm_skinny && gemm_skinny_eligible(g) && (long)((rows + 31) / 32) * (D / 32) <= 256;
    }
    for (int l = 0; l < c.num_layers; ++l) {
      const EncLayerW& Lw = e->layers[l];
      const bool last = l + 1 == c.num_layers;
      if (int r = gemm_rows(w.xb, D, Lw.wqkv, Lw.bqkv, 3 * D, w.qkv, 0, ACT_NONE, nullptr, qkv_pl)) return r;
      if (int r = attention()) return r;
      if (int r = gemm_rows(w.attn_o, D, Lw.wo, Lw.bo, D, tmp, 0, ACT_NONE, nullptr)) return r;
      if (int r = launch_layernorm_hilo((const bf16_t*)tmp, xh, xl, nullptr, rows, D, Lw.ln1g.as<float>(), Lw.ln1b.as<float>(), eps,
                                        xh, xl, nullptr, s)) return r;
      if (int r = gemm_rows(w.xb, D, Lw.w1, Lw.b1, F, w.ffn, 0, ACT_GELU, nullptr)) return r;
      if (ffn2_split) {
        GemmArgs g;
        g.A = w.ffn; g.W = Lw.w2.p; g.C = w.ksplit; g.M = (int)rows; g.N = D; g.K = F; g.a_rpb = (int)rows; g.a_rstride = F; g.ldw = F; g.ldc = D;
        g.out_f32 = 1; g.ksplit = 4; g.ksplit_stride = (long)rows * D;
        if (int r = launch_gemm_skinny(g, s)) return r;
        if (int r = launch_layernorm_hilo_parts(w.ksplit, 4, (long)rows * D, Lw.b2.as<float>(), xh, xl, rows, D, Lw.ln2g.as<float>(), Lw.ln2b.as<float>(),
                                                eps, xh, xl, last ? w.xF : nullptr, s)) return r;
        continue;
      }
      if (int r = gemm_rows(w.ffn, F, Lw.w2, Lw.b2, D, tmp, 0, ACT_NONE, nullptr)) return r;
      if (int r = launch_layernorm_hilo((const bf16_t*)tmp, xh, xl, nullptr, rows, D, Lw.ln2g.as<float>(), Lw.ln2b.as<float>(), eps,
                                        xh, xl, last ? w.xF : nullptr, s)) return r;
    }
    final_x = w.xF;
  } else if (!c.stable_layer_norm && pk_enc) {
    const bool pair_resid = pk_enc == 3;
    float* const keepF = pair_resid ? nullptr : w.xF;
    if (int r = launch_layernorm(prec, w.preF, 1, rows, D, e->enc_g.as<float>(), e->enc_b.as<float>(), eps, 0, nullptr, keepF, s, nullptr,
                                 nullptr, w.xb, pk_enc)) return r;
    auto ln_resid = [&](const float* g_, const float* b_, bool want_f32) -> int {
      if (pair_resid)
        return launch_layernorm(prec, tmp, 1, rows, D, g_, b_, eps, 0, nullptr, want_f32 ? w.xF : nullptr, s, nullptr, nullptr, w.xb,
                                pk_enc, w.xb);
      return launch_layernorm(prec, tmp, 1, rows, D, g_, b_, eps, 0, nullptr, w.xF, s, w.xF, nullptr, w.xb, pk_enc, nullptr);
    };
    for (int l = 0; l < c.num_layers; ++l) {
      const EncLayerW& Lw = e->layers[l];
      const bool last = l + 1 == c.num_layers;
      if (int r = gemm_rows(w.xb, D, Lw.wqkv, Lw.bqkv, 3 * D, w.qkv, 0, ACT_NONE, nullptr, qkv_pl)) return r;
      if (int r = attention()) return r;
      if (int r = gemm_rows(w.attn_o, D, Lw.wo, Lw.bo, D, tmp, 1, ACT_NONE, nullptr)) return r;
      if (int r = ln_resid(Lw.ln1g.as<float>(), Lw.ln1b.as<float>(), false)) return r;
      if (int r = gemm_rows(w.xb, D, Lw.w1, Lw.b1, F, w.ffn, 1, ACT_GELU, nullptr, nullptr, 1)) return r;
      if (int r = gemm_rows(w.ffn, F, Lw.w2, Lw.b2, D, tmp, 1, ACT_NONE, nullptr)) return r;
      if (int r = ln_resid(Lw.ln2g.as<float>(), Lw.ln2b.as<float>(), last)) return r;
    }
    final_x = w.xF;
  } else if (!c.stable_layer_norm) {
    if (int r = launch_layernorm(prec, w.preF, 1, rows, D, e->enc_g.as<float>(), e->enc_b.as<float>(), eps, 0, w.xb,
                                 prec ? w.xF : nullptr, s)) return r;
    for (int l = 0; l < c.num_layers; ++l) {
      const EncLayerW& Lw = e->layers[l];
      if (int r = gemm_rows(w.xb, D, Lw.wqkv, Lw.bqkv, 3 * D, w.qkv, 0, ACT_NONE, nullptr, qkv_pl)) return r;
      if (int r = attention()) return r;
      if (int r = gemm_rows(w.attn_o, D, Lw.wo, Lw.bo, D, tmp, tmp_f32, ACT_NONE, nullptr)) return r;
      if (int r = launch_layernorm(prec, tmp, tmp_f32, rows, D, Lw.ln1g.as<float>(), Lw.ln1b.as<float>(), eps, 0, w.xb,
                                   prec ? w.xF : nullptr, s, w.xF)) return r;
      if (int r = gemm_rows(w.xb, D, Lw.w1, Lw.b1, F, w.ffn, 0, ACT_GELU, nullptr)) return r;
      if (int r = gemm_rows(w.ffn, F, Lw.w2, Lw.b2, D, tmp, tmp_f32, ACT_NONE, nullptr)) return r;
      if (int r = launch_layernorm(prec, tmp, tmp_f32, rows, D, Lw.ln2g.as<float>(), Lw.ln2b.as<float>(), eps, 0, w.xb,
                                   prec ? w.xF : nullptr, s, w.xF)) return r;
    }
    final_x = w.xF;
  } else {
    float* h = w.preF;
    const void* pending = nullptr;
    auto ln_add = [&](const float* g_, const float* b_, const void* branch, void* y_op, float* y_f32) -> int {
      if (pk_enc && y_op)
        return launch_layernorm(prec, h, 1, rows, D, g_, b_, eps, 0, nullptr, nullptr, s, (const float*)branch, branch ? h : nullptr, y_op, pk_enc);
      if (!branch) return launch_layernorm(prec, h, 1, rows, D, g_, b_, eps, 0, y_op, y_f32, s, nullptr, nullptr);
      if (!tmp_f32)
        return launch_layernorm(prec, branch, 0, rows, D, g_, b_, eps, 0, y_op, y_f32, s, h, y_op ? h : nullptr);
      return launch_layernorm(y_op ? prec : 0, h, 1, rows, D, g_, b_, eps, 0, y_op ? y_op : (void*)y_f32, nullptr, s,
                              (const float*)branch, y_op ? h : nullptr);
    };
    for (int l = 0; l < c.num_layers; ++l) {
      const EncLayerW& Lw = e->layers[l];
      if (int r = ln_add(Lw.ln1g.as<float>(), Lw.ln1b.as<float>(), pending, w.xb, nullptr)) return r;
      if (int r = gemm_rows(w.xb, D, Lw.wqkv, Lw.bqkv, 3 * D, w.qkv, 0, ACT_NONE, nullptr, qkv_pl)) return r;
      if (int r = attention()) return r;
      if (int r = gemm_rows(w.attn_o, D, Lw.wo, Lw.bo, D, tmp, tmp_f32, ACT_NONE, nullptr)) return r;
      if (int r = ln_add(Lw.ln2g.as<float>(), Lw.ln2b.as<float>(), tmp, w.xb, nullptr)) return r;
      if (int r = gemm_rows(w.xb, D, Lw.w1, Lw.b1, F, w.ffn, 0, ACT_GELU, nullptr, nullptr, pk_enc ? 1 : 0)) return r;
      if (int r = gemm_rows(w.ffn, F, Lw.w2, Lw.b2, D, tmp, tmp_f32, ACT_NONE, nullptr)) return r;
      pending = tmp;
    }
    float* fin = (float*)w.qkv;
    if (int r = ln_add(e->enc_g.as<float>(), e->enc_b.as<float>(), pending, nullptr, fin)) return r;
    final_x = fin;
  }
  const int64_t n_out = rows * D;
  const double n_out_stat = global_norm ? (double)e->reduce_global_clips * (double)(rows / B) * (double)D : 0.0;
  rctx.mom = out_mom;
  if (tail.head) {
    static_assert(sizeof(svt_frame) == sizeof(FrameOut), "frame layout");
    if (launch_head_fused(final_x, rows, D, tail.head->w.as<float>(), tail.head->wsum.as<float>(),
                          tail.head->has_bias ? tail.head->b.as<float>() : nullptr, tail.head->out_f, w.dots,
                          c.output_norm ? out_mom : nullptr, rows / groups, 1e-5f, tail.logits, (FrameOut*)tail.frames, tail.n_oct,
                          tail.n_cls, s, n_out_stat, global_norm && c.output_norm ? +reduce_now : nullptr, &rctx,
                          (char*)w.mom + w.mom_scr[3])) return SVT_ERR_HIP;
    return SVT_OK;
  }
  if (c.output_norm) {
    if (int r = launch_moments(final_x, n_out / groups, out_mom, (char*)w.mom + w.mom_scr[1], B, s, groups)) return r;
    if (global_norm) { if (int r = reduce_now(&rctx)) return r; }
    if (int r = launch_global_norm(final_x, feats, n_out / groups, out_mom, 1e-5f, s, groups, n_out_stat)) return r;
  } else {
    if (launch_copy_f32(final_x, feats, n_out, s)) return SVT_ERR_HIP;
  }
  return SVT_OK;
}
```

svt_speechbrain_amd/csrc/common.h:

```cpp
#pragma once
#include <hip/hip_runtime.h>
#include <stdint.h>
#include <string>

typedef __bf16 real_bf16x8 __attribute__((ext_vector_type(8)));
#ifdef SVT_OPERAND_F16
typedef _Float16 bf16_t;
#define SVT_MFMA_16x16x32(a, b, c) __builtin_amdgcn_mfma_f32_16x16x32_f16(a, b, c, 0, 0, 0)
#define SVT_MFMA_32x32x16(a, b, c) __builtin_amdgcn_mfma_f32_32x32x16_f16(a, b, c, 0, 0, 0)
#else
typedef __bf16 bf16_t;
#define SVT_MFMA_16x16x32(a, b, c) __builtin_amdgcn_mfma_f32_16x16x32_bf16(a, b, c, 0, 0, 0)
#define SVT_MFMA_32x32x16(a, b, c) __builtin_amdgcn_mfma_f32_32x32x16_bf16(a, b, c, 0, 0, 0)
#endif
typedef bf16_t bf16x8 __attribute__((ext_vector_type(8)));
typedef bf16_t bf16x4 __attribute__((ext_vector_type(4)));
typedef float f32x4 __attribute__((ext_vector_type(4)));

namespace svt {

#if defined(__HIPCC__)
__device__ __forceinline__ float gelu_fast(float x) {
  const float z = fabsf(x) * 0.70710678118654752440f;
  const float t = __builtin_amdgcn_rcpf(fmaf(0.3275911f, z, 1.0f));
  float poly = fmaf(1.061405429f, t, -1.453152027f);
  poly = fmaf(poly, t, 1.421413741f);
  poly = fmaf(poly, t, -0.284496736f);
  poly = fmaf(poly, t, 0.254829592f);
  const float e = __builtin_amdgcn_exp2f(-1.44269504088896340736f * z * z);
  const float erf_abs = fmaf(-poly * t, e, 1.0f);
  const float half_x = 0.5f * x;
  return fmaf(half_x, copysignf(erf_abs, x), half_x);
}
__device__ __forceinline__ float gelu_erf(float x) { return gelu_fast(x); }
typedef float f32x2_t __attribute__((ext_vector_type(2)));
__device__ __forceinline__ f32x2_t gelu_fast2(f32x2_t x) {
  const f32x2_t z = __builtin_elementwise_abs(x) * 0.70710678118654752440f;
  const f32x2_t d = z * 0.3275911f + 1.0f;
  const f32x2_t t = {__builtin_amdgcn_rcpf(d.x), __builtin_amdgcn_rcpf(d.y)};
  f32x2_t poly = t * 1.061405429f + (-1.453152027f);
  poly = poly * t + 1.421413741f;
  poly = poly * t + (-0.284496736f);
  poly = poly * t + 0.254829592f;
  const f32x2_t zz = z * z * (-1.44269504088896340736f);
  const f32x2_t e = {__builtin_amdgcn_exp2f(zz.x), __builtin_amdgcn_exp2f(zz.y)};
  const f32x2_t erf_abs = 1.0f - poly * t * e;
  const f32x2_t hx = x * 0.5f;
  const f32x2_t sg = {copysignf(erf_abs.x, x.x), copysignf(erf_abs.y, x.y)};
  return hx * sg + hx;
}
#ifdef SVT_OPERAND_F16
__device__ __forceinline__ f32x2_t gelu_bf16x2(f32x2_t x) {
  f32x2_t z = x * 0.70710678118654752440f;
  z.x = __builtin_amdgcn_fmed3f(z.x, -3.0f, 3.0f);
  z.y = __builtin_amdgcn_fmed3f(z.y, -3.0f, 3.0f);
  const f32x2_t u = z * z;
  f32x2_t q = u * 4.074456683e-08f + (-1.944940095e-06f);
  q = q * u + 4.106299457e-05f;
  q = q * u + (-5.110675702e-04f);
  q = q * u + 4.235681612e-03f;
  q = q * u + (-2.510436811e-02f);
  q = q * u + 1.110860035e-01f;
  q = q * u + (-3.753373921e-01f);
  q = q * u + 1.128336072e+00f;
  f32x2_t pe = z * q;
  pe.x = __builtin_amdgcn_fmed3f(pe.x, -1.0f, 1.0f);
  pe.y = __builtin_amdgcn_fmed3f(pe.y, -1.0f, 1.0f);
  const f32x2_t hx = x * 0.5f;
  return hx * pe + hx;
}
template <int NP>
__device__ __forceinline__ void gelu_bf16x2_xn(f32x2_t (&x)[NP]) {
  f32x2_t z[NP], u[NP], q[NP];
#pragma unroll
  for (int i = 0; i < NP; ++i) {
    z[i] = x[i] * 0.70710678118654752440f;
    z[i].x = __builtin_amdgcn_fmed3f(z[i].x, -3.0f, 3.0f);
    z[i].y = __builtin_amdgcn_fmed3f(z[i].y, -3.0f, 3.0f);
  }
#pragma unroll
  for (int i = 0; i < NP; ++i) u[i] = z[i] * z[i];
#pragma unroll
  for (int i = 0; i < NP; ++i) q[i] = u[i] * 4.074456683e-08f + (-1.944940095e-06f);
  constexpr float c[7] = {4.106299457e-05f, -5.110675702e-04f, 4.235681612e-03f, -2.510436811e-02f,
                          1.110860035e-01f, -3.753373921e-01f, 1.128336072e+00f};
#pragma unroll
  for (int k = 0; k < 7; ++k) {
#pragma unroll
    for (int i = 0; i < NP; ++i) q[i] = q[i] * u[i] + c[k];
  }
#pragma unroll
  for (int i = 0; i < NP; ++i) {
    f32x2_t pe = z[i] * q[i];
    pe.x = __builtin_amdgcn_fmed3f(pe.x, -1.0f, 1.0f);
    pe.y = __builtin_amdgcn_fmed3f(pe.y, -1.0f, 1.0f);
    const f32x2_t hx = x[i] * 0.5f;
    x[i] = hx * pe + hx;
  }
}
#else
#define SVT_GELU_C0 3.9867674568e-01f
#define SVT_GELU_C1 (-6.5719787820e-02f)
#define SVT_GELU_C2 9.3166354115e-03f
#define SVT_GELU_C3 (-9.3154765044e-04f)
#define SVT_GELU_C4 6.0684808363e-05f
#define SVT_GELU_C5 (-2.2724625145e-06f)
#define SVT_GELU_C6 3.6657791326e-08f
#define SVT_GELU_HALF 0.4999907314777374f
__device__ __forceinline__ f32x2_t gelu_bf16x2(f32x2_t x) {
  f32x2_t t;
  t.x = __builtin_amdgcn_fmed3f(x.x, -3.8f, 3.8f);
  t.y = __builtin_amdgcn_fmed3f(x.y, -3.8f, 3.8f);
  const f32x2_t u = t * t;
  f32x2_t q = u * SVT_GELU_C6 + SVT_GELU_C5;
  q = q * u + SVT_GELU_C4;
  q = q * u + SVT_GELU_C3;
  q = q * u + SVT_GELU_C2;
  q = q * u + SVT_GELU_C1;
  q = q * u + SVT_GELU_C0;
  return x * (t * q + SVT_GELU_HALF);
}
template <int NP>
__device__ __forceinline__ void gelu_bf16x2_xn(f32x2_t (&x)[NP]) {
  f32x2_t t[NP], u[NP], q[NP];
#pragma unroll
  for (int i = 0; i < NP; ++i) {
    t[i].x = __builtin_amdgcn_fmed3f(x[i].x, -3.8f, 3.8f);
    t[i].y = __builtin_amdgcn_fmed3f(x[i].y, -3.8f, 3.8f);
  }
#pragma unroll
  for (int i = 0; i < NP; ++i) u[i] = t[i] * t[i];
#pragma unroll
  for (int i = 0; i < NP; ++i) q[i] = u[i] * SVT_GELU_C6 + SVT_GELU_C5;
  constexpr float c[5] = {SVT_GELU_C4, SVT_GELU_C3, SVT_GELU_C2, SVT_GELU_C1, SVT_GELU_C0};
#pragma unroll
  for (int k = 0; k < 5; ++k) {
#pragma unroll
    for (int i = 0; i < NP; ++i) q[i] = q[i] * u[i] + c[k];
  }
#pragma unroll
  for (int i = 0; i < NP; ++i) x[i] = x[i] * (t[i] * q[i] + SVT_GELU_HALF);
}
#endif
__device__ __forceinline__ void gelu_bf16x2_x4(f32x2_t (&x)[4]) { gelu_bf16x2_xn<4>(x); }
#endif

void set_error(const std::string& msg);
int hip_fail(hipError_t e, const char* what, const char* file, int line);

#define SVT_HIP(expr)                                                        \
  do {                                                                       \
    hipError_t _e = (expr);                                                  \
    if (_e != hipSuccess) return svt::hip_fail(_e, #expr, __FILE__, __LINE__); \
  } while (0)

#define SVT_LAUNCH_CHECK() SVT_HIP(hipGetLastError())

enum Act { ACT_NONE = 0, ACT_GELU = 1, ACT_RELU = 2, ACT_PRELU = 3 };

struct GemmArgs {
  const void* A = nullptr;
  const void* W = nullptr;
  void* C = nullptr;
  const float* bias = nullptr;
  const float* resid = nullptr;
  int M = 0, N = 0, K = 0;
  int a_rpb = 1;
  long a_bstride = 0, a_rstride = 0;
  long ldw = 0, ldc = 0;
  int nz = 1, nz2 = 1;
  long a_z1 = 0, a_z2 = 0, w_z1 = 0, w_z2 = 0, c_z1 = 0, c_z2 = 0, bias_z2 = 0;
  float alpha = 1.f;
  int act = ACT_NONE;
  int out_f32 = 0;
  int dbg = 0;
  int k_taps = 1, k_cin = 0;
  const void* W_kperm = nullptr;
  int kperm_taps = 0, kperm_cin = 0;
  int ksplit = 1;
  long ksplit_stride = 0;
  int walk_pm = 0;
  int c_vec = 1;
  int raster_gm = 8;
  int gen = 0;
  int a_d1 = 1, a_d2 = 1;
  long a_e1 = 0, a_e2 = 0;
  int kseg = 0;
  long kseg_stride = 0;
  int c_d1 = 1, c_d2 = 1;
  long c_e1 = 0, c_e2 = 0, c_base = 0;
  int c_nsplit = 0;
  long c_nstride = 0;
  const float* slope = nullptr;
  int resid_first = 0;
  int resid_op_type = 0;
  unsigned short* planes = nullptr;
  long plane_stride = 0;
  int planes_f16 = 0;
  int a_pairs = 0;
  int c_pairs = 0;
  int stamp_ends = 0;
  long long* trace = nullptr;
};

int launch_gemm(int prec, const GemmArgs& a, hipStream_t s);
int launch_gemm_skinny(const GemmArgs& a, hipStream_t s);

bool gemm_dma_eligible(const GemmArgs& a);
bool gemm_pps_eligible(const GemmArgs& a);
int launch_gemm_pps(const GemmArgs& a, int bm, hipStream_t s);
int launch_gemm_p1w(const GemmArgs& a, int bm, hipStream_t s);
bool gemm_skinny_eligible(const GemmArgs& a);
int split_weights_register(const void* w_f32_dev, long n_rows, int K, int kind, hipStream_t s);
void split_weights_forget(const void* w_f32_dev);
bool gemm_x3p_eligible(const GemmArgs& a);
int launch_gemm_x3p(int kind, const GemmArgs& a, const void* packed, hipStream_t s);
bool gemm_x3q_eligible(const GemmArgs& a);
int launch_gemm_x3q(int kind, const GemmArgs& a, const void* packed, int bm, hipStream_t s);
int launch_gemm_p1x(int kind, const GemmArgs& a, const void* packed, int bm, hipStream_t s);
#pragma GCC visibility push(hidden)
int launch_gemm_staged(int prec, const GemmArgs& a, int bn, hipStream_t s);
int launch_gemm_pp8(const GemmArgs& a, int bm, int bn, hipStream_t s);
int launch_gemm_pers(const GemmArgs& a, int bm, hipStream_t s);
int launch_gemm_skinny_tile(const GemmArgs& a, int tile, hipStream_t s);
const void* split_weights_find(const void* W, int kind, int K, long rows_needed);
int launch_gemm_x3s(int kind, const GemmArgs& a, const void* packed, int nbs, int form, hipStream_t s);
inline bool tile_span_fits(const GemmArgs& a) {
  const unsigned long clips = 255 / (unsigned long)(a.a_rpb > 0 ? a.a_rpb : 1) + 1;
  const unsigned long bs = (unsigned long)(a.a_bstride > 0 ? a.a_bstride : 0), rs = (unsigned long)(a.a_rstride > 0 ? a.a_rstride : 0);
  return a.a_bstride >= 0 && a.a_rstride > 0 && (clips * bs + 256ul * rs + (unsigned long)a.K) * 4 < 0xF0000000ul &&
         (unsigned long)a.N * a.K * 4 < 0xF0000000ul;
}
inline int persistent_blocks(int ntiles, int cap) { return ntiles < cap ? ((ntiles + 7) / 8) * 8 : cap; }
#pragma GCC visibility pop

__device__ __forceinline__ void tile_walk(int logical, int tiles_m, int tiles_n, int pm, int& tile_m, int& tile_n) {
  if (pm <= 0) { tile_n = logical % tiles_n; tile_m = logical / tiles_n; return; }
  const int per_panel = pm * tiles_n;
  const int pnl = logical / per_panel, rem = logical - pnl * per_panel;
  const int rows = min(pm, tiles_m - pnl * pm);
  tile_n = rem / rows;
  tile_m = pnl * pm + (rem - tile_n * rows);
}

extern int g_gemm_dbg;
extern int g_gemm_force_bm;
extern int g_gemm_ring;
extern int g_gemm_variant;
extern int g_gemm_skinny;
extern int g_gemm_skinny_max_tiles;
extern int g_gemm_x3;
extern int g_stamp_ends;
extern int g_x3_pairs;
extern int g_gemm_p1w;
extern int g_gemm_p1x;
extern int g_gemm_skinny_small_tiles;
extern int g_gemm_walk;
extern int g_conv_kperm;
extern int g_gemm_persist_wgs;
extern int g_gemm_kernel_id;

extern int g_ln_two_rows;
extern int g_flash_wide;
extern int g_flash_kernel_id;
extern int g_ffn2_ksplit;
#pragma GCC visibility push(hidden)
extern int g_conv_ln_bf16;
extern int g_debug_keep_split;
extern int g_conv_down_fused;
#pragma GCC visibility pop

int ensure_dyn_lds(const void* kernel, int bytes);

int dev_alloc(void** out, size_t bytes);
void dev_free(void* p);
extern int g_guard_alloc;

void prof_begin(hipStream_t s);
void prof_end(hipStream_t s, double flops, double bytes, int kind = 1);

int set_ticket_fenced(int on);
int launch_moments(const float* x, int64_t n, double* moments, void* scratch, int groups_max, hipStream_t s, int groups = 1);
size_t moments_scratch_bytes(int groups_max);
int launch_global_norm(const float* x, float* y, int64_t n, const double* moments, float eps, hipStream_t s, int groups = 1,
                       double n_stat = 0);
int launch_conv0_window_moments(const float* wav, int B, int64_t L, int k, int stride, int64_t T1,
                                double* wm , void* scratch , hipStream_t s);
size_t conv0_window_moments_scratch_bytes(int B, int64_t T1);
int launch_conv0_group_coef(const double* wav_moments , int64_t n_wav, const double* wm, int B,
                            int64_t T1, int C, int k, const float* w0 , const float* b0 ,
                            const float* gamma, const float* beta, float eps_wav, float eps_gn,
                            float* coef , hipStream_t s, int clips_per_norm_group);
struct FrameOut { float p_on, p_off; int32_t octave, pitch_class; };
int launch_head_fused(const float* x, int64_t rows, int K, const float* w, const float* wsum, const float* b, int N, float* dots,
                      double* mom, int64_t rows_per_group, float eps, float* logits, FrameOut* frames, int n_oct, int n_cls,
                      hipStream_t s,
                      double n_stat = 0, int (*between)(void*) = nullptr, void* between_arg = nullptr, void* scratch = nullptr);
size_t head_scratch_bytes(int64_t rows, int groups_max);

int launch_layernorm(int prec, const void* x, int x_is_f32, int64_t rows, int D, const float* gamma,
                     const float* beta, float eps, int gelu, void* yT, float* yF, hipStream_t s,
                     const float* add = nullptr, float* sumF = nullptr,
                     void* yP = nullptr, int pair_kind = 0,
                     const void* addP = nullptr);
bool layernorm_hilo_ok(int D);
int launch_layernorm_hilo_parts(const float* parts, int nparts, long part_stride, const float* pbias, const bf16_t* rh, const bf16_t* rl, int64_t rows,
                                int D, const float* gamma, const float* beta, float eps, bf16_t* yh, bf16_t* yl, float* yF, hipStream_t s);
int launch_layernorm_hilo(const bf16_t* branch, const bf16_t* rh, const bf16_t* rl, const float* x32, int64_t rows, int D,
                          const float* gamma, const float* beta, float eps, bf16_t* yh, bf16_t* yl, float* yF, hipStream_t s);

int launch_conv0_group_apply(int prec, const float* wav, int B, int64_t L, int k, int stride, int64_t T1, int C,
                             const float* coef, void* out , hipStream_t s, int pair_kind = 0);
int launch_conv0_layer(int prec, const float* wav, int B, int64_t L, int k, int stride, int64_t T1, int C,
                       const double* wav_moments, int64_t n_wav, float eps_wav, const float* w0, const float* b0,
                       const float* gamma, const float* beta, float eps, void* out, hipStream_t s, int clips_per_norm_group,
                       int pair_kind = 0);
int launch_f32_to_pairs(int kind, const float* x, void* out, int64_t n, hipStream_t s);
int launch_pairs_to_f32(int kind, const void* in, const void* lo_plane, float* y, int64_t n, hipStream_t s);

bool conv0_mfma_ok(int prec, int pair_kind, int k, int stride, int C);
size_t conv0_mfma_table_bytes(int B);
int launch_conv0_mfma_group(const float* wav, int B, int64_t L, int stride, int64_t T1, const float* coef, void* table_ws, void* out,
                            hipStream_t s, int pair_kind = 0);
int launch_conv0_mfma_layer(const float* wav, int B, int64_t L, int stride, int64_t T1, const double* wav_moments, int64_t n_wav,
                            float eps_wav, const float* w0, const float* b0, const float* gamma, const float* beta, float eps, void* table_ws,
                            void* out, hipStream_t s, int clips_per_norm_group, int pair_kind = 0);
extern int g_conv0_mfma;

int launch_f32_to_bf16(const float* in, bf16_t* out, int64_t n, hipStream_t s);
int launch_zero_bytes(void* p, size_t bytes, hipStream_t s);
int launch_copy_f32(const float* in, float* out, int64_t n, hipStream_t s);
int launch_zero_cols(float* p, int64_t rows, int cols, int64_t ld, hipStream_t s);
int launch_posconv_gather(int prec, const float* h, int B, int T, int D, int G, int kp, int Tp, void* out, hipStream_t s,
                          const float* sc = nullptr, const float* sh = nullptr);
int launch_posconv_scatter_add(const float* h, const void* y, int B, int T, int D, int G, int P, int Tq, float* pre, hipStream_t s,
                               int y_f32 = 0);
int launch_softmax_rows(int prec, const float* S, int64_t rows, int T, int Tp, void* P, hipStream_t s);
int launch_transpose_v(int prec, const void* qkv, int B, int T, int H, int dh, long ld, long voff, int Tp,
                       void* Vt, hipStream_t s);
int launch_axpby(int prec, const void* x, const void* y, float a, float b, void* out, int64_t n, hipStream_t s);
int launch_add_pe(int prec, const float* x, int B, int T, int Tsrc, int D, const float* pe, float* outF, void* outT,
                  hipStream_t s);
int launch_add_f32(const float* a, const float* b, float* out, int64_t n, hipStream_t s);
int launch_relpos_table(const float* embed, int H, int T, int num_buckets, int max_distance, float* pb, hipStream_t s);
int launch_relpos_gate(int prec, const void* u, int64_t rows, int T, int H, int dh, const float* wab, const float* bab,
                       const float* cst, float* gate, hipStream_t s);
int launch_scores_add_relbias(float* S, int64_t BH, int H, int T, int Tp, const float* gate, const float* pb, hipStream_t s);
int launch_clock_stamp(long long* out16, hipStream_t s);

int launch_flash_attention(const void* Q, long ldq, long q_bstride, const void* K, const void* V, long ldk, long k_bstride,
                           void* O, long ldo, long o_bstride, int B, int T, int H, int dh, float scale, hipStream_t s,
                           const float* gate = nullptr, const float* pb = nullptr);

int launch_split_planes(int kind, const float* src, long ld_src, long rows, int cols, void* dst, long ld_dst, long plane, hipStream_t s);
bool flash_attention_x3_ok(int dh);
int launch_flash_attention_x3(int kind, const void* Q, long ldq, long q_bstride, long q_plane, const void* K, const void* V, long ldk,
                              long k_bstride, long k_plane, float* O, long ldo, long o_bstride, int B, int T, int H, int dh, float scale,
                              hipStream_t s, int o_pairs = 0);

int launch_linear_f32(const float* x, int64_t rows, int K, const float* w, const float* b, int N, float* y,
                      hipStream_t s);
bool linear_head_eligible(int K, int N);
int launch_linear_head(const float* x, int64_t rows, int K, const float* w, const float* b, int N, float* y, hipStream_t s);
int launch_bce_loss(const float* x, int64_t B, int64_t t_pred, const float* y, int64_t t_tgt, int64_t T, const float* rel_len,
                    const float* pos_weight, float* per_frame, double* sums, hipStream_t s);
int launch_nll_loss(const float* logp, int64_t B, int64_t t_pred, int C, const int64_t* tgt, int64_t t_tgt, int64_t T,
                    const float* rel_len, float* per_frame, double* sums, int* bad_target, hipStream_t s);
int launch_loss_reduce(const double* sums, int B, int reduction, float smoothing, float* out, hipStream_t s);
int launch_softmax_small(const float* x, int64_t rows, int n, int apply_log, float* y, hipStream_t s);
int launch_deltas(const float* x, long ldx, int B, int T, int C, int n, float inv_denom, float* out, long ldo, hipStream_t s);
int launch_context_window(const float* x, int B, int T, int C, int ctx, int lag, int pad, float* out, hipStream_t s);
int launch_fbank_frames(const float* wav, int B, int64_t L, int n_fft, int hop, int64_t nframes, const float* window,
                        float* frames , hipStream_t s);
int launch_power_spectrum(const float* reim , int64_t rows, int nb,
                          int imoff, int ld, float* power , int ldp, hipStream_t s);
int launch_fbank_db(float* fb, int B, int64_t per_seq, float top_db, hipStream_t s);
int launch_decode_frames(const float* logits, int64_t rows, int n_out, int n_oct, int n_cls, FrameOut* out,
                         hipStream_t s);
int launch_ctc_greedy(const float* probs, int B, int T, int V, const float* rel_lens, int blank, int32_t* tokens,
                      int32_t* out_lens, hipStream_t s);

int launch_video_pad(int prec, const float* v, int B, int T, int H, int W, int Hp, int Wp, void* out, hipStream_t s);
struct VideoTransform { double sub0, div0, mean, std; };
int launch_video_pad_u8(int prec, const unsigned char* v, int B, int T, int Hin, int Win, int dy, int dx, int H, int W, int Hp, int Wp,
                        const VideoTransform& tf, void* out, hipStream_t s);
int launch_conv3d_front(int prec, const void* vp, const void* w, const float* bias, const float* slope, long F, int T, int Hp,
                        int Wp, int H0, int W0, void* out, hipStream_t s);
int launch_maxpool_3x3s2(int prec, const void* in, long F, int H0, int W0, int C, int H1, int W1, void* out, hipStream_t s);
extern int g_stem_pool_fused;
bool conv3d_front_pool_ok(int prec, int Hp, int Wp, int W0);
int launch_conv3d_front_pool(const void* vp, const void* w, const float* bias, const float* slope, long F, int T, int Hp, int Wp, int H0,
                             int W0, int H1, int W1, void* out, hipStream_t s);
int launch_zero_halo(int prec, void* buf, long F, int Hp, int Wp, int C, hipStream_t s);
int launch_avgpool_interior(int prec, const void* in, long F, int H, int W, int C, void* out, hipStream_t s);
extern int g_conv3x3_c64, g_conv3x3_c64_launches, g_conv3x3_c64_form;
bool conv3x3_c64_ok(int prec, int Hs, int Ws);
int launch_conv3x3_c64(const void* in, const void* wimg, const float* bias, const float* slope, const void* resid, void* out, long F,
                       int Hs, int Ws, hipStream_t s);
bool conv3x3_c128_ok(int prec, int Hs, int Ws);
int launch_conv3x3_c128(const void* in, const void* wimg, const float* bias, const float* slope, const void* resid, void* out, long F,
                        int Hs, int Ws, hipStream_t s);
int launch_amt_objective_grad(const float* x, int64_t B, int64_t t_pred, int n_out, int n_oct_cols, const float* on_t,
                              const float* off_t, const int64_t* oct_t, const int64_t* cls_t, int64_t t_tgt, int64_t T,
                              const float* rel_len, float pos_weight, float smoothing, float* dx, float* terms, void* ws,
                              hipStream_t s);
size_t amt_objective_status_offset(int64_t B);
size_t amt_objective_workspace_bytes(int64_t B);
int64_t linear_wgrad_slabs(int64_t rows, int D);
size_t linear_wgrad_workspace_bytes(int64_t rows, int D, int N);
int launch_linear_wgrad(const float* x, const float* dy, int64_t rows, int D, int N, float* dw, float* db, void* ws, hipStream_t s);
constexpr int kAdaMaxTensors = 32;
constexpr int64_t kAdaChunk = 4096;
size_t ada_workspace_bytes(const int64_t* numels, int count);
int launch_clip_adadelta(int count, float* const* params, float* const* grads, float* const* square_avg, float* const* acc_delta,
                         const int64_t* numels, float lr, float rho, float one_minus_rho, float eps, float weight_decay, int maximize,
                         float max_norm, float* total_norm, void* ws, hipStream_t s);
struct RcaRefreshJob {
  const float* src;
  void* dst;
  int64_t rows, cols;
  int transpose, f32;
};
constexpr int kRcaMaxRefreshJobs = 32;
struct RcaRefreshJobs {
  RcaRefreshJob j[kRcaMaxRefreshJobs];
  int n;
};
int launch_rca_refresh(int prec, const RcaRefreshJobs& jobs, hipStream_t s);
int launch_rca_attn_lse(int prec, const void* Q, long ldq, const void* K, long ldk, int B, int T, int H, int dh, float scale, float* lse,
                        hipStream_t s);
struct RcaAttnBwd {
  const void *q[2], *k, *v, *o[2];
  long ldq[2], ldkv;
  const float* dbl;
  float coef[2];
  const float* lse;
  float* delta;
  float* dq[2];
  long lddq[2];
  float *dk, *dv;
  long lddkv;
  int B, T, H, dh;
  float scale;
};
int launch_rca_attn_bwd(int prec, const RcaAttnBwd& p, hipStream_t s);
size_t rca_ln_bwd_scratch_bytes(int64_t rows, int D);
int launch_rca_ln_bwd(int prec, const float* x, const float* add, const float* gamma, const float* dy, int64_t rows, int D, float eps,
                      float* dxF, void* dxT, float* dgamma, float* dbeta, void* scratch, hipStream_t s);
int launch_rca_relu_mask(int prec, float* dh, const void* h, int64_t n, void* dhT, hipStream_t s);
struct RcaWgrad {
  const float* dy[2];
  const void* x[2];
  long ldy[2], ldx[2];
  int nseg;
  int64_t rows;
  int N, C;
};
size_t rca_wgrad_scratch_bytes(int64_t vrows, int N, int C);
int launch_rca_wgrad(int prec, const RcaWgrad& w, float* dw, float* db, void* scratch, hipStream_t s);
int launch_linear_dgrad(const float* dy, const float* w, int64_t rows, int D, int N, float* dx, hipStream_t s);

}
```

svt_speechbrain_amd/csrc/layernorm.hip:

```cpp
#include "device_util.h"
#include <type_traits>

namespace svt {
namespace {
template <typename TI, typename TO>
__global__ __launch_bounds__(256) void layernorm_kernel(const TI* x, const float* add, float* sumF, int64_t rows, int D,
                                                        const float* gamma, const float* beta, float eps, int gelu,
                                                        TO* yT, float* yF) {
  const int lane = threadIdx.x & 63;
  const int64_t row = (int64_t)blockIdx.x * 4 + (threadIdx.x >> 6);
  if (row >= rows) return;
  const TI* xr = x + row * D;
  const float* ar = add ? add + row * D : nullptr;
  float s = 0.f;
  for (int i = lane; i < D; i += 64) s += ld<TI>(xr, i) + (ar ? ar[i] : 0.f);
  const float mean = wave_sum(s) / (float)D;
  float q = 0.f;
  for (int i = lane; i < D; i += 64) { const float d = ld<TI>(xr, i) + (ar ? ar[i] : 0.f) - mean; q += d * d; }
  const float rstd = rsqrtf(wave_sum(q) / (float)D + eps);
  for (int i = lane; i < D; i += 64) {
    const float xv = ld<TI>(xr, i) + (ar ? ar[i] : 0.f);
    if (sumF) sumF[row * D + i] = xv;
    float v = (xv - mean) * rstd * gamma[i] + beta[i];
    if (gelu) v = gelu_erf(v);
    if (yT) st<TO>(yT, row * D + i, v);
    if (yF) yF[row * D + i] = v;
  }
}

template <int VPT, typename TO, typename TI = float, int PK = 0>
__global__ __launch_bounds__(256) void layernorm_f32_vec_kernel(const TI* x, const float* add, float* sumF,
                                                                int64_t rows, const float* gamma, const float* beta,
                                                                float eps, int gelu, TO* yT, float* yF, void* yP = nullptr,
                                                                const void* addP = nullptr) {
  constexpr int D = 64 * VPT, NV = VPT / 4;
  const int lane = threadIdx.x & 63;
  const int64_t row = (int64_t)blockIdx.x * 4 + (threadIdx.x >> 6);
  if (row >= rows) return;
  float v[VPT];
  float s = 0.f;
#pragma unroll
  for (int j = 0; j < NV; ++j) {
    float4 t;
    if constexpr (sizeof(TI) == 4) {
      t = ((const float4*)(x + row * D))[lane + 64 * j];
    } else {
      const bf16x4 tb = ((const bf16x4*)(x + row * D))[lane + 64 * j];
      t = float4{(float)tb[0], (float)tb[1], (float)tb[2], (float)tb[3]};
    }
    if (add) {
      const float4 a = ((const float4*)(add + row * D))[lane + 64 * j];
      t.x += a.x; t.y += a.y; t.z += a.z; t.w += a.w;
    }
    if constexpr (PK != 0) {
      if (addP) {
        const int64_t e = row * D + (lane + 64 * j) * 4;
        const char* pp = (const char*)addP + (e >> 5) * 128 + (e & 31) * 2;
        const uint2 h = *(const uint2*)pp, l = *(const uint2*)(pp + 64);
        const unsigned hw[2] = {h.x, h.y}, lw[2] = {l.x, l.y};
        float a[4];
#pragma unroll
        for (int i = 0; i < 4; ++i) {
          const unsigned short hs = (unsigned short)(hw[i >> 1] >> (16 * (i & 1))), ls = (unsigned short)(lw[i >> 1] >> (16 * (i & 1)));
          if constexpr (PK == 3) a[i] = (float)__builtin_bit_cast(_Float16, hs) + (float)__builtin_bit_cast(_Float16, ls);
          else a[i] = (float)__builtin_bit_cast(__bf16, hs) + (float)__builtin_bit_cast(__bf16, ls);
        }
        t.x += a[0]; t.y += a[1]; t.z += a[2]; t.w += a[3];
      }
    }
    if (sumF) ((float4*)(sumF + row * D))[lane + 64 * j] = t;
    v[4 * j] = t.x; v[4 * j + 1] = t.y; v[4 * j + 2] = t.z; v[4 * j + 3] = t.w;
    s += (t.x + t.y) + (t.z + t.w);
  }
  const float mean = wave_sum(s) * (1.f / D);
  float q = 0.f;
#pragma unroll
  for (int i = 0; i < VPT; ++i) { v[i] -= mean; q = fmaf(v[i], v[i], q); }
  const float rstd = rsqrtf(wave_sum(q) * (1.f / D) + eps);
#pragma unroll
  for (int j = 0; j < NV; ++j) {
    const int c = (lane + 64 * j) * 4;
    const float4 g = *(const float4*)(gamma + c), b = *(const float4*)(beta + c);
    float o0 = fmaf(v[4 * j] * rstd, g.x, b.x), o1 = fmaf(v[4 * j + 1] * rstd, g.y, b.y);
    float o2 = fmaf(v[4 * j + 2] * rstd, g.z, b.z), o3 = fmaf(v[4 * j + 3] * rstd, g.w, b.w);
    if (gelu) {
      if (sizeof(TO) == 2 && PK == 0 && !yF) {
        f32x2_t ga = {o0, o1}, gb = {o2, o3};
        ga = gelu_bf16x2(ga); gb = gelu_bf16x2(gb);
        o0 = ga.x; o1 = ga.y; o2 = gb.x; o3 = gb.y;
      } else {
        o0 = gelu_erf(o0); o1 = gelu_erf(o1); o2 = gelu_erf(o2); o3 = gelu_erf(o3);
      }
    }
    if (yT) {
      if constexpr (sizeof(TO) == 2) {
        bf16x4 o;
        o[0] = (bf16_t)o0; o[1] = (bf16_t)o1; o[2] = (bf16_t)o2; o[3] = (bf16_t)o3;
        *(bf16x4*)((bf16_t*)yT + row * D + c) = o;
      } else {
        *(float4*)((float*)yT + row * D + c) = float4{o0, o1, o2, o3};
      }
    }
    if (yF) *(float4*)(yF + row * D + c) = float4{o0, o1, o2, o3};
    if constexpr (PK != 0) {
      const float ov[4] = {o0, o1, o2, o3};
      store_pairs<PK, 4>(yP, row * D + c, ov);
    }
  }
}

template <int D>
__global__ __launch_bounds__(256) void layernorm_op16_rows2_kernel(const bf16_t* x, int64_t rows, const float* gamma, const float* beta,
                                                                   float eps, int gelu, bf16_t* y) {
  constexpr int NC = D / 256;
  const int lane = threadIdx.x & 63, sub = lane & 31;
  const int64_t row = (int64_t)blockIdx.x * 8 + (threadIdx.x >> 6) * 2 + (lane >> 5);
  if (row >= rows) return;
  float v[NC][8];
  float s = 0.f;
#pragma unroll
  for (int j = 0; j < NC; ++j) {
    const bf16x8 h = *(const bf16x8*)(x + row * D + (sub + 32 * j) * 8);
#pragma unroll
    for (int i = 0; i < 8; ++i) v[j][i] = (float)h[i];
    s += ((v[j][0] + v[j][1]) + (v[j][2] + v[j][3])) + ((v[j][4] + v[j][5]) + (v[j][6] + v[j][7]));
  }
#pragma unroll
  for (int o = 16; o > 0; o >>= 1) s += __shfl_xor(s, o, 64);
  const float mean = s * (1.f / D);
  float q = 0.f;
#pragma unroll
  for (int j = 0; j < NC; ++j)
#pragma unroll
    for (int i = 0; i < 8; ++i) { v[j][i] -= mean; q = fmaf(v[j][i], v[j][i], q); }
#pragma unroll
  for (int o = 16; o > 0; o >>= 1) q += __shfl_xor(q, o, 64);
  const float rstd = rsqrtf(q * (1.f / D) + eps);
#pragma unroll
  for (int j = 0; j < NC; ++j) {
    const int c = (sub + 32 * j) * 8;
    const float4 g0 = *(const float4*)(gamma + c), g1 = *(const float4*)(gamma + c + 4);
    const float4 b0 = *(const float4*)(beta + c), b1 = *(const float4*)(beta + c + 4);
    const float gg[8] = {g0.x, g0.y, g0.z, g0.w, g1.x, g1.y, g1.z, g1.w}, bb[8] = {b0.x, b0.y, b0.z, b0.w, b1.x, b1.y, b1.z, b1.w};
    f32x2_t o2[4];
#pragma unroll
    for (int i = 0; i < 4; ++i) o2[i] = f32x2_t{fmaf(v[j][2 * i] * rstd, gg[2 * i], bb[2 * i]), fmaf(v[j][2 * i + 1] * rstd, gg[2 * i + 1], bb[2 * i + 1])};
    if (gelu) gelu_bf16x2_x4(o2);
    bf16x8 ob;
#pragma unroll
    for (int i = 0; i < 4; ++i) { ob[2 * i] = (bf16_t)o2[i].x; ob[2 * i + 1] = (bf16_t)o2[i].y; }
    *(bf16x8*)(y + row * D + c) = ob;
  }
}

template <class F> void ln_width(int D, F&& f) {
  if (D == 512) f(std::integral_constant<int, 8>{});
  else if (D == 768) f(std::integral_constant<int, 12>{});
  else f(std::integral_constant<int, 16>{});
}
}
int g_ln_two_rows = 1;
int launch_layernorm(int prec, const void* x, int x_is_f32, int64_t rows, int D, const float* gamma,
                     const float* beta, float eps, int gelu, void* yT, float* yF, hipStream_t s, const float* add,
                     float* sumF, void* yP, int pair_kind, const void* addP) {
  if (addP && !yP) { set_error("layernorm: a pair-row addend needs the pair-row output form"); return -1; }
  const dim3 grid((unsigned)((rows + 3) / 4)), grid2((unsigned)((rows + 7) / 8)), block(256);
  const bool wide = D == 512 || D == 768 || D == 1024;
  if (yP) {
    if (prec || !x_is_f32 || yT || !wide || (pair_kind != 2 && pair_kind != 3) || !aligned(15, x, yF, add, sumF, gamma, beta) || !aligned(127, yP)) { set_error("layernorm: the pair-row output needs an fp32 input, D in {512, 768, 1024} and aligned buffers"); return -1; }
    ln_width(D, [&](auto vpt) {
      constexpr int VPT = decltype(vpt)::value;
      if (pair_kind == 3) hipLaunchKernelGGL((layernorm_f32_vec_kernel<VPT, float, float, 3>), grid, block, 0, s, (const float*)x, add, sumF, rows, gamma, beta, eps, gelu, (float*)nullptr, yF, yP, addP);
      else hipLaunchKernelGGL((layernorm_f32_vec_kernel<VPT, float, float, 2>), grid, block, 0, s, (const float*)x, add, sumF, rows, gamma, beta, eps, gelu, (float*)nullptr, yF, yP, addP);
    });
  } else if (prec && !x_is_f32 && wide && yT && !yF && !add && !sumF && g_ln_two_rows && aligned(15, x, yT, gamma, beta)) {
    ln_width(D, [&](auto vpt) {
      hipLaunchKernelGGL((layernorm_op16_rows2_kernel<64 * decltype(vpt)::value>), grid2, block, 0, s, (const bf16_t*)x, rows, gamma, beta, eps, gelu, (bf16_t*)yT);
    });
  } else if (prec && !x_is_f32 && wide && aligned(7, x) && aligned(15, yT, yF, add, sumF)) {
    ln_width(D, [&](auto vpt) {
      hipLaunchKernelGGL((layernorm_f32_vec_kernel<decltype(vpt)::value, bf16_t, bf16_t>), grid, block, 0, s, (const bf16_t*)x, add, sumF, rows, gamma, beta, eps, gelu, (bf16_t*)yT, yF);
    });
  } else if (add && !x_is_f32) {
    set_error("layernorm: the addend form needs an fp32 input (or bf16 with D in {512,768,1024})");
    return -1;
  } else if (x_is_f32 && wide && aligned(15, x, yT, yF, gamma, beta, add, sumF)) {
    ln_width(D, [&](auto vpt) {
      constexpr int VPT = decltype(vpt)::value;
      if (prec) hipLaunchKernelGGL((layernorm_f32_vec_kernel<VPT, bf16_t>), grid, block, 0, s, (const float*)x, add, sumF, rows, gamma, beta, eps, gelu, (bf16_t*)yT, yF);
      else hipLaunchKernelGGL((layernorm_f32_vec_kernel<VPT, float>), grid, block, 0, s, (const float*)x, add, sumF, rows, gamma, beta, eps, gelu, (float*)yT, yF);
    });
  } else if (!prec) {
    hipLaunchKernelGGL((layernorm_kernel<float, float>), grid, block, 0, s, (const float*)x, add, sumF, rows, D, gamma, beta, eps, gelu, (float*)yT, yF);
  } else if (x_is_f32) {
    hipLaunchKernelGGL((layernorm_kernel<float, bf16_t>), grid, block, 0, s, (const float*)x, add, sumF, rows, D, gamma, beta, eps, gelu, (bf16_t*)yT, yF);
  } else {
    hipLaunchKernelGGL((layernorm_kernel<bf16_t, bf16_t>), grid, block, 0, s, (const bf16_t*)x, add, sumF, rows, D, gamma, beta, eps, gelu, (bf16_t*)yT, yF);
  }
  SVT_LAUNCH_CHECK();
  return 0;
}

namespace {
template <int VPT>
__global__ __launch_bounds__(256) void layernorm_hilo_kernel(const bf16_t* branch, const bf16_t* rh, const bf16_t* rl,
                                                             int64_t rows, const float* gamma, const float* beta, float eps,
                                                             bf16_t* yh, bf16_t* yl, float* yF) {
  constexpr int D = 64 * VPT, NV = VPT / 4;
  const int lane = threadIdx.x & 63;
  const int64_t row = (int64_t)blockIdx.x * 4 + (threadIdx.x >> 6);
  if (row >= rows) return;
  float v[VPT];
  float s = 0.f;
#pragma unroll
  for (int j = 0; j < NV; ++j) {
    const long o = row * D + (lane + 64 * j) * 4;
    const bf16x4 h = *(const bf16x4*)(rh + o), l = *(const bf16x4*)(rl + o);
    float4 t = float4{(float)h[0] + (float)l[0], (float)h[1] + (float)l[1], (float)h[2] + (float)l[2], (float)h[3] + (float)l[3]};
    if (branch) {
      const bf16x4 a = *(const bf16x4*)(branch + o);
      t.x += (float)a[0]; t.y += (float)a[1]; t.z += (float)a[2]; t.w += (float)a[3];
    }
    v[4 * j] = t.x; v[4 * j + 1] = t.y; v[4 * j + 2] = t.z; v[4 * j + 3] = t.w;
    s += (t.x + t.y) + (t.z + t.w);
  }
  const float mean = wave_sum(s) * (1.f / D);
  float q = 0.f;
#pragma unroll
  for (int i = 0; i < VPT; ++i) { v[i] -= mean; q = fmaf(v[i], v[i], q); }
  const float rstd = rsqrtf(wave_sum(q) * (1.f / D) + eps);
#pragma unroll
  for (int j = 0; j < NV; ++j) {
    const int c = (lane + 64 * j) * 4;
    const float4 g = *(const float4*)(gamma + c), b = *(const float4*)(beta + c);
    const float o[4] = {fmaf(v[4 * j] * rstd, g.x, b.x), fmaf(v[4 * j + 1] * rstd, g.y, b.y),
                        fmaf(v[4 * j + 2] * rstd, g.z, b.z), fmaf(v[4 * j + 3] * rstd, g.w, b.w)};
    bf16x4 oh, ol;
#pragma unroll
    for (int i = 0; i < 4; ++i) { oh[i] = (bf16_t)o[i]; ol[i] = (bf16_t)(o[i] - (float)oh[i]); }
    *(bf16x4*)(yh + row * D + c) = oh;
    *(bf16x4*)(yl + row * D + c) = ol;
    if (yF) *(float4*)(yF + row * D + c) = float4{o[0], o[1], o[2], o[3]};
  }
}

template <int D, bool PARTS = false>
__global__ __launch_bounds__(256) void layernorm_hilo2_kernel(const bf16_t* branch, const bf16_t* rh, const bf16_t* rl,
                                                              int64_t rows, const float* gamma, const float* beta, float eps,
                                                              bf16_t* yh, bf16_t* yl, float* yF, const float* parts = nullptr, int nparts = 0,
                                                              long part_stride = 0, const float* pbias = nullptr) {
  constexpr int NC = D / 256;
  const int lane = threadIdx.x & 63, sub = lane & 31;
  const int64_t row = (int64_t)blockIdx.x * 8 + (threadIdx.x >> 6) * 2 + (lane >> 5);
  if (row >= rows) return;
  float v[NC][8];
  float s = 0.f;
#pragma unroll
  for (int j = 0; j < NC; ++j) {
    const long o = row * D + (sub + 32 * j) * 8;
    const bf16x8 h = *(const bf16x8*)(rh + o), l = *(const bf16x8*)(rl + o);
#pragma unroll
    for (int i = 0; i < 8; ++i) v[j][i] = (float)h[i] + (float)l[i];
    if constexpr (PARTS) {
      float a[8];
      {
        const float4 t0 = *(const float4*)(parts + o), t1 = *(const float4*)(parts + o + 4);
        a[0] = t0.x; a[1] = t0.y; a[2] = t0.z; a[3] = t0.w; a[4] = t1.x; a[5] = t1.y; a[6] = t1.z; a[7] = t1.w;
      }
      for (int k = 1; k < nparts; ++k) {
        const float4 t0 = *(const float4*)(parts + k * part_stride + o), t1 = *(const float4*)(parts + k * part_stride + o + 4);
        a[0] += t0.x; a[1] += t0.y; a[2] += t0.z; a[3] += t0.w; a[4] += t1.x; a[5] += t1.y; a[6] += t1.z; a[7] += t1.w;
      }
      const int c = (sub + 32 * j) * 8;
      const float4 b0 = *(const float4*)(pbias + c), b1 = *(const float4*)(pbias + c + 4);
      const float bb[8] = {b0.x, b0.y, b0.z, b0.w, b1.x, b1.y, b1.z, b1.w};
#pragma unroll
      for (int i = 0; i < 8; ++i) v[j][i] += (float)(bf16_t)(a[i] + bb[i]);
    } else if (branch) {
      const bf16x8 a = *(const bf16x8*)(branch + o);
#pragma unroll
      for (int i = 0; i < 8; ++i) v[j][i] += (float)a[i];
    }
    s += ((v[j][0] + v[j][1]) + (v[j][2] + v[j][3])) + ((v[j][4] + v[j][5]) + (v[j][6] + v[j][7]));
  }
#pragma unroll
  for (int o = 16; o > 0; o >>= 1) s += __shfl_xor(s, o, 64);
  const float mean = s * (1.f / D);
  float q = 0.f;
#pragma unroll
  for (int j = 0; j < NC; ++j)
#pragma unroll
    for (int i = 0; i < 8; ++i) { v[j][i] -= mean; q = fmaf(v[j][i], v[j][i], q); }
#pragma unroll
  for (int o = 16; o > 0; o >>= 1) q += __shfl_xor(q, o, 64);
  const float rstd = rsqrtf(q * (1.f / D) + eps);
#pragma unroll
  for (int j = 0; j < NC; ++j) {
    const int c = (sub + 32 * j) * 8;
    const float4 g0 = *(const float4*)(gamma + c), g1 = *(const float4*)(gamma + c + 4);
    const float4 b0 = *(const float4*)(beta + c), b1 = *(const float4*)(beta + c + 4);
    const float gg[8] = {g0.x, g0.y, g0.z, g0.w, g1.x, g1.y, g1.z, g1.w}, bb[8] = {b0.x, b0.y, b0.z, b0.w, b1.x, b1.y, b1.z, b1.w};
    float o[8];
    bf16x8 oh, ol;
#pragma unroll
    for (int i = 0; i < 8; ++i) {
      o[i] = fmaf(v[j][i] * rstd, gg[i], bb[i]);
      oh[i] = (bf16_t)o[i];
      ol[i] = (bf16_t)(o[i] - (float)oh[i]);
    }
    *(bf16x8*)(yh + row * D + c) = oh;
    *(bf16x8*)(yl + row * D + c) = ol;
    if (yF) {
      *(float4*)(yF + row * D + c) = float4{o[0], o[1], o[2], o[3]};
      *(float4*)(yF + row * D + c + 4) = float4{o[4], o[5], o[6], o[7]};
    }
  }
}
template <int VPT>
__global__ __launch_bounds__(256) void layernorm_f32_to_hilo_kernel(const float* x, int64_t rows, const float* gamma,
                                                                    const float* beta, float eps, bf16_t* yh, bf16_t* yl) {
  constexpr int D = 64 * VPT, NV = VPT / 4;
  const int lane = threadIdx.x & 63;
  const int64_t row = (int64_t)blockIdx.x * 4 + (threadIdx.x >> 6);
  if (row >= rows) return;
  float v[VPT];
  float s = 0.f;
#pragma unroll
  for (int j = 0; j < NV; ++j) {
    const float4 t = ((const float4*)(x + row * D))[lane + 64 * j];
    v[4 * j] = t.x; v[4 * j + 1] = t.y; v[4 * j + 2] = t.z; v[4 * j + 3] = t.w;
    s += (t.x + t.y) + (t.z + t.w);
  }
  const float mean = wave_sum(s) * (1.f / D);
  float q = 0.f;
#pragma unroll
  for (int i = 0; i < VPT; ++i) { v[i] -= mean; q = fmaf(v[i], v[i], q); }
  const float rstd = rsqrtf(wave_sum(q) * (1.f / D) + eps);
#pragma unroll
  for (int j = 0; j < NV; ++j) {
    const int c = (lane + 64 * j) * 4;
    const float4 g = *(const float4*)(gamma + c), b = *(const float4*)(beta + c);
    const float o[4] = {fmaf(v[4 * j] * rstd, g.x, b.x), fmaf(v[4 * j + 1] * rstd, g.y, b.y),
                        fmaf(v[4 * j + 2] * rstd, g.z, b.z), fmaf(v[4 * j + 3] * rstd, g.w, b.w)};
    bf16x4 oh, ol;
#pragma unroll
    for (int i = 0; i < 4; ++i) { oh[i] = (bf16_t)o[i]; ol[i] = (bf16_t)(o[i] - (float)oh[i]); }
    *(bf16x4*)(yh + row * D + c) = oh;
    *(bf16x4*)(yl + row * D + c) = ol;
  }
}
}
bool layernorm_hilo_ok(int D) { return D == 512 || D == 768 || D == 1024; }
int launch_layernorm_hilo_parts(const float* parts, int nparts, long part_stride, const float* pbias, const bf16_t* rh, const bf16_t* rl, int64_t rows,
                                int D, const float* gamma, const float* beta, float eps, bf16_t* yh, bf16_t* yl, float* yF, hipStream_t s) {
  if (!parts || nparts < 1 || !pbias || !(D == 512 || D == 768 || D == 1024) || (part_stride & 3) || !aligned(15, parts, pbias, rh, rl, yh, yl, yF, gamma, beta)) { set_error("layernorm (K-split branch): D in {512, 768, 1024} and 16-byte aligned buffers"); return -1; }
  const dim3 grid2((unsigned)((rows + 7) / 8)), block(256);
  ln_width(D, [&](auto vpt) {
    hipLaunchKernelGGL((layernorm_hilo2_kernel<64 * decltype(vpt)::value, true>), grid2, block, 0, s, nullptr, rh, rl, rows, gamma, beta, eps, yh, yl, yF, parts, nparts, part_stride, pbias);
  });
  SVT_LAUNCH_CHECK();
  return 0;
}
int launch_layernorm_hilo(const bf16_t* branch, const bf16_t* rh, const bf16_t* rl, const float* x32, int64_t rows, int D,
                          const float* gamma, const float* beta, float eps, bf16_t* yh, bf16_t* yl, float* yF, hipStream_t s) {
  const dim3 grid((unsigned)((rows + 3) / 4)), grid2((unsigned)((rows + 7) / 8)), block(256);
  ln_width(D, [&](auto vpt) {
    constexpr int VPT = decltype(vpt)::value;
    if (x32) hipLaunchKernelGGL((layernorm_f32_to_hilo_kernel<VPT>), grid, block, 0, s, x32, rows, gamma, beta, eps, yh, yl);
    else if (g_ln_two_rows && aligned(15, branch, rh, rl, yh, yl, yF, gamma, beta)) hipLaunchKernelGGL((layernorm_hilo2_kernel<64 * VPT>), grid2, block, 0, s, branch, rh, rl, rows, gamma, beta, eps, yh, yl, yF);
    else hipLaunchKernelGGL((layernorm_hilo_kernel<VPT>), grid, block, 0, s, branch, rh, rl, rows, gamma, beta, eps, yh, yl, yF);
  });
  SVT_LAUNCH_CHECK();
  return 0;
}

}
```

svt_speechbrain_amd/csrc/stats.hip:

```cpp
#include "device_util.h"

namespace svt {
namespace {
__device__ __forceinline__ void st_partial(double* p, double v) {
  __hip_atomic_store((unsigned long long*)p, __builtin_bit_cast(unsigned long long, v), __ATOMIC_RELAXED, __HIP_MEMORY_SCOPE_AGENT);
}
__device__ int d_ticket_fenced = 0;
__device__ __forceinline__ bool last_workgroup(unsigned* ticket, unsigned n_groups) {
  __shared__ unsigned s_last;
  asm volatile("s_waitcnt vmcnt(0)" ::: "memory");
  __syncthreads();
  if (threadIdx.x == 0) {
    const unsigned t = d_ticket_fenced ? __hip_atomic_fetch_add(ticket, 1u, __ATOMIC_ACQ_REL, __HIP_MEMORY_SCOPE_AGENT)
                                       : __hip_atomic_fetch_add(ticket, 1u, __ATOMIC_RELAXED, __HIP_MEMORY_SCOPE_AGENT);
    s_last = t == n_groups - 1 ? 1u : 0u;
    if (s_last) __hip_atomic_store(ticket, 0u, __ATOMIC_RELAXED, __HIP_MEMORY_SCOPE_AGENT);
  }
  __syncthreads();
  return s_last != 0;
}
__device__ __forceinline__ double ld_partial(const double* p) {
  return __builtin_bit_cast(double, __hip_atomic_load((const unsigned long long*)p, __ATOMIC_RELAXED, __HIP_MEMORY_SCOPE_AGENT));
}
}
int set_ticket_fenced(int on) {
  const int v = on ? 1 : 0;
  SVT_HIP(hipMemcpyToSymbol(HIP_SYMBOL(d_ticket_fenced), &v, sizeof(int)));
  return 0;
}

namespace {
__global__ __launch_bounds__(256) void moments_kernel(const float* x, int64_t n, double* mom, double* part, unsigned* ticket) {
  __shared__ double sh[2][4];
  x += (int64_t)blockIdx.y * n;
  mom += 2 * blockIdx.y;
  part += (size_t)blockIdx.y * gridDim.x * 2;
  double s = 0.0, ss = 0.0;
  const int64_t n4 = n >> 2;
  const float4* x4 = (const float4*)x;
  int64_t i = (int64_t)blockIdx.x * blockDim.x + threadIdx.x;
  const int64_t stride = (int64_t)gridDim.x * blockDim.x;
  for (; i < n4; i += stride) {
    const float4 v = x4[i];
    const float a = (v.x + v.y) + (v.z + v.w);
    const float b = (v.x * v.x + v.y * v.y) + (v.z * v.z + v.w * v.w);
    s += (double)a;
    ss += (double)b;
  }
  if (blockIdx.x == 0 && threadIdx.x == 0) {
    for (int64_t j = n4 << 2; j < n; ++j) { s += (double)x[j]; ss += (double)x[j] * (double)x[j]; }
  }
  s = wave_sum(s);
  ss = wave_sum(ss);
  const int lane = threadIdx.x & 63, wave = threadIdx.x >> 6;
  if (lane == 0) { sh[0][wave] = s; sh[1][wave] = ss; }
  __syncthreads();
  if (threadIdx.x == 0) {
    st_partial(part + blockIdx.x * 2, sh[0][0] + sh[0][1] + sh[0][2] + sh[0][3]);
    st_partial(part + blockIdx.x * 2 + 1, sh[1][0] + sh[1][1] + sh[1][2] + sh[1][3]);
  }
  if (!last_workgroup(ticket + blockIdx.y, gridDim.x)) return;
  s = 0.0; ss = 0.0;
  for (unsigned b = threadIdx.x; b < gridDim.x; b += 256) { s += ld_partial(part + b * 2); ss += ld_partial(part + b * 2 + 1); }
  s = wave_sum(s);
  ss = wave_sum(ss);
  if (lane == 0) { sh[0][wave] = s; sh[1][wave] = ss; }
  __syncthreads();
  if (threadIdx.x == 0) {
    mom[0] = sh[0][0] + sh[0][1] + sh[0][2] + sh[0][3];
    mom[1] = sh[1][0] + sh[1][1] + sh[1][2] + sh[1][3];
  }
}

__global__ void global_norm_kernel(const float* x, float* y, int64_t n, const double* mom, float eps, double n_stat) {
  x += (int64_t)blockIdx.y * n;
  y += (int64_t)blockIdx.y * n;
  mom += 2 * blockIdx.y;
  const double mean = mom[0] / n_stat;
  const double var = mom[1] / n_stat - mean * mean;
  const float mu = (float)mean;
  const float rs = (float)(1.0 / sqrt(var + (double)eps));
  const int64_t n4 = n >> 2;
  int64_t i = (int64_t)blockIdx.x * blockDim.x + threadIdx.x;
  const int64_t stride = (int64_t)gridDim.x * blockDim.x;
  for (; i < n4; i += stride) {
    float4 v = ((const float4*)x)[i];
    v.x = (v.x - mu) * rs; v.y = (v.y - mu) * rs; v.z = (v.z - mu) * rs; v.w = (v.w - mu) * rs;
    ((float4*)y)[i] = v;
  }
  if (blockIdx.x == 0 && threadIdx.x == 0)
    for (int64_t j = n4 << 2; j < n; ++j) y[j] = (x[j] - mu) * rs;
}
}
static int moments_grid(int64_t n, int groups) {
  return groups > 1 ? grid_for(n / 4 + 1, 256, 512 / (groups < 64 ? groups : 64) + 1) : grid_for(n / 4 + 1, 256, 512);
}
static size_t moments_ticket_bytes(int groups) { return ((size_t)groups * 4 + 255) & ~(size_t)255; }
size_t moments_scratch_bytes(int groups_max) {
  const size_t wgs = (size_t)(groups_max < 64 ? 512 + groups_max : 576) + 9 * (size_t)groups_max;
  return moments_ticket_bytes(groups_max) + wgs * 2 * sizeof(double);
}

int launch_moments(const float* x, int64_t n, double* moments, void* scratch, int groups_max, hipStream_t s, int groups) {
  if (groups > 1 && (n & 3)) { set_error("moments: per-group length must be a multiple of 4 elements"); return -1; }
  if (groups > groups_max || !scratch || ((uintptr_t)scratch & 7)) { set_error("moments: scratch"); return -1; }
  const int gx = moments_grid(n, groups);
  if (moments_ticket_bytes(groups_max) + (size_t)gx * groups * 2 * sizeof(double) > moments_scratch_bytes(groups_max)) { set_error("moments: scratch too small"); return -1; }
  unsigned* ticket = (unsigned*)scratch;
  double* part = (double*)((char*)scratch + moments_ticket_bytes(groups_max));
  hipLaunchKernelGGL(moments_kernel, dim3(gx, groups), dim3(256), 0, s, x, n, moments, part, ticket);
  SVT_LAUNCH_CHECK();
  return 0;
}

int launch_global_norm(const float* x, float* y, int64_t n, const double* moments, float eps, hipStream_t s, int groups, double n_stat) {
  if (groups > 1 && (n & 3)) { set_error("global_norm: per-group length must be a multiple of 4 elements"); return -1; }
  hipLaunchKernelGGL(global_norm_kernel, dim3(grid_for(n / 4 + 1), groups), dim3(256), 0, s, x, y, n, moments, eps,
                     n_stat > 0 ? n_stat : (double)n);
  SVT_LAUNCH_CHECK();
  return 0;
}

namespace {
__global__ __launch_bounds__(256) void conv0_window_moments_kernel(const float* wav, int64_t L, int stride, int64_t T1,
                                                                   double* wm, double* part, unsigned* ticket) {
  __shared__ double sh[4][NWM];
  const int b = blockIdx.y;
  const float* x = wav + (int64_t)b * L;
  double acc[NWM];
#pragma unroll
  for (int i = 0; i < NWM; ++i) acc[i] = 0.0;
  constexpr int WPT = 8;
  const int64_t t0 = ((int64_t)blockIdx.x * blockDim.x + threadIdx.x) * WPT;
  for (int w = 0; w < WPT; ++w) {
    const int64_t t = t0 + w;
    if (t >= T1) break;
    float v[K0];
#pragma unroll
    for (int j = 0; j < K0; ++j) v[j] = x[t * stride + j];
    int idx = K0;
#pragma unroll
    for (int j = 0; j < K0; ++j) {
      acc[j] += (double)v[j];
#pragma unroll
      for (int j2 = j; j2 < K0; ++j2) acc[idx++] += (double)(v[j] * v[j2]);
    }
  }
  const int lane = threadIdx.x & 63, wave = threadIdx.x >> 6;
#pragma unroll
  for (int i = 0; i < NWM; ++i) {
    const double r = wave_sum(acc[i]);
    if (lane == 0) sh[wave][i] = r;
  }
  __syncthreads();
  part += (size_t)b * gridDim.x * NWM;
  if (threadIdx.x < NWM)
    st_partial(part + blockIdx.x * NWM + threadIdx.x, sh[0][threadIdx.x] + sh[1][threadIdx.x] + sh[2][threadIdx.x] + sh[3][threadIdx.x]);
  if (!last_workgroup(ticket + b, gridDim.x)) return;
  if (threadIdx.x < NWM) {
    double t = 0.0;
    unsigned k = 0;
    for (; k + 8 <= gridDim.x; k += 8) {
      double v[8];
#pragma unroll
      for (int j = 0; j < 8; ++j) v[j] = ld_partial(part + (k + j) * NWM + threadIdx.x);
#pragma unroll
      for (int j = 0; j < 8; ++j) t += v[j];
    }
    for (; k < gridDim.x; ++k) t += ld_partial(part + k * NWM + threadIdx.x);
    wm[b * NWM + threadIdx.x] = t;
  }
}

__global__ void conv0_group_coef_kernel(const double* wav_mom, int64_t n_wav, const double* wm, int64_t T1, int C,
                                        const float* w0, const float* b0, const float* gamma, const float* beta,
                                        float eps_wav, float eps_gn, float* coef, int cpg) {
  const int b = blockIdx.y;
  if (wav_mom) wav_mom += 2 * (b / cpg);
  const int c = blockIdx.x * blockDim.x + threadIdx.x;
  if (c >= C) return;
  double mu = 0.0, r = 1.0;
  if (wav_mom) {
    mu = wav_mom[0] / (double)n_wav;
    const double var = wav_mom[1] / (double)n_wav - mu * mu;
    r = 1.0 / sqrt(var + (double)eps_wav);
  }
  const double* m = wm + b * NWM;
  const double invT = 1.0 / (double)T1;
  double w[K0], mn[K0];
  double wsum = 0.0;
  for (int j = 0; j < K0; ++j) { w[j] = (double)w0[c * K0 + j]; wsum += w[j]; mn[j] = r * (m[j] * invT - mu); }
  const double bias = b0 ? (double)b0[c] : 0.0;
  double dot = 0.0;
  for (int j = 0; j < K0; ++j) dot += w[j] * mn[j];
  double quad = 0.0;
  int idx = K0;
  for (int j = 0; j < K0; ++j)
    for (int j2 = j; j2 < K0; ++j2) {
      const double R = r * r * (m[idx] * invT - mu * m[j] * invT - mu * m[j2] * invT + mu * mu);
      quad += (j == j2 ? 1.0 : 2.0) * w[j] * w[j2] * R;
      ++idx;
    }
  const double mean = dot + bias;
  const double e2 = quad + 2.0 * bias * dot + bias * bias;
  double var = e2 - mean * mean;
  if (var < 0.0) var = 0.0;
  const double a = (double)gamma[c] / sqrt(var + (double)eps_gn);
  const double shift = (double)beta[c] - mean * a;
  float* o = coef + ((int64_t)b * C + c) * (K0 + 1);
  for (int j = 0; j < K0; ++j) o[j] = (float)(a * r * w[j]);
  o[K0] = (float)(a * (bias - r * mu * wsum) + shift);
}
}
size_t conv0_window_moments_scratch_bytes(int B, int64_t T1) {
  const size_t gx = (size_t)((T1 + 2047) / 2048);
  return moments_ticket_bytes(B) + (size_t)B * gx * NWM * sizeof(double);
}

int launch_conv0_window_moments(const float* wav, int B, int64_t L, int k, int stride, int64_t T1, double* wm, void* scratch,
                                hipStream_t s) {
  if (k != K0) { set_error("conv layer 0 kernel size must be 10"); return -1; }
  if (!scratch || ((uintptr_t)scratch & 7)) { set_error("conv0 window moments: scratch"); return -1; }
  const int per_block = 256 * 8;
  dim3 grid((unsigned)((T1 + per_block - 1) / per_block), B);
  unsigned* ticket = (unsigned*)scratch;
  double* part = (double*)((char*)scratch + moments_ticket_bytes(B));
  hipLaunchKernelGGL(conv0_window_moments_kernel, grid, dim3(256), 0, s, wav, L, stride, T1, wm, part, ticket);
  SVT_LAUNCH_CHECK();
  return 0;
}

int launch_conv0_group_coef(const double* wav_moments, int64_t n_wav, const double* wm, int B, int64_t T1, int C,
                            int k, const float* w0, const float* b0, const float* gamma, const float* beta,
                            float eps_wav, float eps_gn, float* coef, hipStream_t s, int cpg) {
  if (k != K0) { set_error("conv layer 0 kernel size must be 10"); return -1; }
  dim3 grid((C + 63) / 64, B);
  hipLaunchKernelGGL(conv0_group_coef_kernel, grid, dim3(64), 0, s, wav_moments, n_wav, wm, T1, C, w0, b0, gamma, beta,
                     eps_wav, eps_gn, coef, cpg);
  SVT_LAUNCH_CHECK();
  return 0;
}

namespace {
template <int KC>
__global__ __launch_bounds__(256) void head_dots_kernel(const float* __restrict__ x, int64_t rows, const float* __restrict__ w, int N,
                                                        float* __restrict__ dots, double* __restrict__ mom, int64_t rows_per_group,
                                                        double* __restrict__ slots, unsigned* __restrict__ ticket, int slots_per_group) {
  constexpr int K = KC * 256;
  extern __shared__ __attribute__((aligned(16))) float wl[];
  for (int i = threadIdx.x * 4; i < N * K; i += 1024) *(float4*)(wl + i) = *(const float4*)(w + i);
  __syncthreads();
  const int lane = threadIdx.x & 63, wave = threadIdx.x >> 6;
  const bool hi32 = (lane & 32) != 0, hi16 = (lane & 16) != 0;
  const int myrow = (hi32 ? 2 : 0) + (hi16 ? 1 : 0);
  const int NW = (int)gridDim.x * 4, W = (int)blockIdx.x * 4 + wave;
  int64_t cur_g = -1, g_end = 0;
  float la = 0.f, lq = 0.f;
  auto flush = [&]() {
    if (cur_g < 0) return;
    const double sa = wave_sum((double)la), sq = wave_sum((double)lq);
    if (lane == 0) {
      const int64_t ja = (cur_g * rows_per_group) >> 2;
      const int p = (int)(((W - ja) % NW + NW) % NW);
      double* sl = slots + ((size_t)cur_g * slots_per_group + p) * 2;
      st_partial(sl, sa);
      st_partial(sl + 1, sq);
    }
    la = 0.f; lq = 0.f;
  };
  for (int64_t r0 = ((int64_t)blockIdx.x * 4 + wave) * 4; r0 < rows; r0 += (int64_t)gridDim.x * 16) {
    float4 xv[4][KC];
#pragma unroll
    for (int rr = 0; rr < 4; ++rr) {
      const int64_t row = r0 + rr < rows ? r0 + rr : rows - 1;
      const auto xrs = __builtin_amdgcn_make_buffer_rsrc((void*)x, 0, 0x7FFFFFF0, 0x00020000);
#pragma unroll
      for (int c = 0; c < KC; ++c) {
        typedef float f4v __attribute__((ext_vector_type(4)));
        const f4v t = __builtin_bit_cast(f4v, __builtin_amdgcn_raw_buffer_load_b128(xrs, (unsigned)((row * K + c * 256 + lane * 4) * 4), 0, 0));
        xv[rr][c] = float4{t[0], t[1], t[2], t[3]};
      }
    }
    if (mom) {
#pragma unroll
      for (int rr = 0; rr < 4; ++rr) {
        if (r0 + rr >= rows) break;
        if (r0 + rr >= g_end || cur_g < 0) {
          flush();
          cur_g = (r0 + rr) / rows_per_group;
          g_end = (cur_g + 1) * rows_per_group;
        }
        float a = 0.f, q = 0.f;
#pragma unroll
        for (int c = 0; c < KC; ++c) {
          const float4 v = xv[rr][c];
          a += (v.x + v.y) + (v.z + v.w);
          q += (v.x * v.x + v.y * v.y) + (v.z * v.z + v.w * v.w);
        }
        la += a;
        lq += q;
      }
    }
    float out0 = 0.f, out1 = 0.f;
    for (int n = 0; n < N; ++n) {
      float sacc[4] = {0.f, 0.f, 0.f, 0.f};
#pragma unroll
      for (int c = 0; c < KC; ++c) {
        const float4 wv = *(const float4*)(wl + n * K + c * 256 + lane * 4);
#pragma unroll
        for (int rr = 0; rr < 4; ++rr) {
          sacc[rr] = fmaf(xv[rr][c].x, wv.x, sacc[rr]);
          sacc[rr] = fmaf(xv[rr][c].y, wv.y, sacc[rr]);
          sacc[rr] = fmaf(xv[rr][c].z, wv.z, sacc[rr]);
          sacc[rr] = fmaf(xv[rr][c].w, wv.w, sacc[rr]);
        }
      }
      float k0 = hi32 ? sacc[2] : sacc[0], k1 = hi32 ? sacc[3] : sacc[1];
      const float g0 = hi32 ? sacc[0] : sacc[2], g1 = hi32 ? sacc[1] : sacc[3];
      k0 += __shfl_xor(g0, 32, 64);
      k1 += __shfl_xor(g1, 32, 64);
      float v = hi16 ? k1 : k0;
      v += __shfl_xor(hi16 ? k0 : k1, 16, 64);
#pragma unroll
      for (int o = 8; o > 0; o >>= 1) v += __shfl_xor(v, o, 64);
      if ((lane & 15) == (n & 15)) { if (n < 16) out0 = v; else out1 = v; }
    }
    const int64_t row = r0 + myrow;
    if (row < rows) {
      const int n0 = lane & 15;
      if (n0 < N) dots[row * N + n0] = out0;
      if (n0 + 16 < N) dots[row * N + n0 + 16] = out1;
    }
  }
  if (mom) {
    flush();
    if (!last_workgroup(ticket, gridDim.x)) return;
    const int64_t n_groups = (rows + rows_per_group - 1) / rows_per_group;
    for (int64_t g = wave; g < n_groups; g += 4) {
      const int64_t a = g * rows_per_group, b = (g + 1) * rows_per_group < rows ? (g + 1) * rows_per_group : rows;
      const int64_t nj = ((b - 1) >> 2) - (a >> 2) + 1;
      const int n = (int)(nj < NW ? nj : NW);
      const double* sl = slots + (size_t)g * slots_per_group * 2;
      double ta = 0.0, tq = 0.0;
      int i = lane;
      for (; i + 3 * 64 < n; i += 4 * 64) {
        double va[4], vq[4];
#pragma unroll
        for (int j = 0; j < 4; ++j) { va[j] = ld_partial(sl + 2 * (i + 64 * j)); vq[j] = ld_partial(sl + 2 * (i + 64 * j) + 1); }
#pragma unroll
        for (int j = 0; j < 4; ++j) { ta += va[j]; tq += vq[j]; }
      }
      for (; i < n; i += 64) { ta += ld_partial(sl + 2 * i); tq += ld_partial(sl + 2 * i + 1); }
      ta = wave_sum(ta);
      tq = wave_sum(tq);
      if (lane == 0) { mom[2 * g] = ta; mom[2 * g + 1] = tq; }
    }
  }
}

__global__ void head_finish_kernel(const float* __restrict__ dots, int64_t rows, int N, const float* __restrict__ wsum,
                                   const float* __restrict__ bias, const double* __restrict__ mom, int64_t rows_per_group,
                                   double group_elems, float eps, float* __restrict__ logits, FrameOut* __restrict__ frames,
                                   int n_oct, int n_cls) {
  const int64_t r = (int64_t)blockIdx.x * blockDim.x + threadIdx.x;
  if (r >= rows) return;
  float mu = 0.f, rs = 1.f;
  if (mom) {
    const int64_t g = r / rows_per_group;
    const double mean = mom[2 * g] / group_elems;
    const double var = mom[2 * g + 1] / group_elems - mean * mean;
    mu = (float)mean;
    rs = (float)(1.0 / sqrt(var + (double)eps));
  }
  float l[32];
#pragma unroll
  for (int j = 0; j < 32; ++j)
    if (j < N) {
      l[j] = fmaf(dots[r * N + j] - mu * wsum[j], rs, bias ? bias[j] : 0.f);
      logits[r * N + j] = l[j];
    }
  if (frames) {
    FrameOut f;
    f.p_on = 1.f / (1.f + expf(-l[0]));
    f.p_off = 1.f / (1.f + expf(-l[1]));
    int bo = 0;
    float bv = l[2];
#pragma unroll
    for (int j = 3; j < 32; ++j)
      if (j <= 2 + n_oct && l[j] > bv) { bv = l[j]; bo = j - 2; }
    int bc = 0;
    const int c0 = 2 + n_oct + 1;
    bv = -3.4e38f;
#pragma unroll
    for (int j = 3; j < 32; ++j)
      if (j >= c0 && j <= c0 + n_cls) {
        if (j == c0) { bv = l[j]; bc = 0; }
        else if (l[j] > bv) { bv = l[j]; bc = j - c0; }
      }
    f.octave = bo;
    f.pitch_class = bc;
    frames[r] = f;
  }
}
}
static unsigned head_dots_grid(int64_t rows) {
  const int64_t blocks = (rows + 15) / 16;
  return (unsigned)(blocks < 512 ? blocks : 512);
}
static int head_slots_per_group(int64_t rows, int64_t rpg) {
  const int64_t nw = (int64_t)head_dots_grid(rows) * 4, per = (rpg + 3) / 4 + 1;
  return (int)(per < nw ? per : nw);
}
size_t head_scratch_bytes(int64_t rows, int groups_max) {
  return 256 + ((size_t)rows / 4 + 2 * (size_t)groups_max + 8) * 2 * sizeof(double);
}

template <int KC>
static int launch_head_dots_kc(const float* x, int64_t rows, const float* w, int N, float* dots, double* mom, int64_t rpg, void* scratch,
                               hipStream_t s) {
  const size_t lds = (size_t)N * KC * 256 * 4;
  if (int r_ = ensure_dyn_lds((const void*)head_dots_kernel<KC>, 32 * KC * 256 * 4)) return r_;
  const unsigned grid = head_dots_grid(rows);
  if (mom && (!scratch || ((uintptr_t)scratch & 7))) { set_error("head_fused: scratch"); return -1; }
  if ((unsigned long)rows * KC * 256 * 4 > 0x7FFFFFF0ul) { set_error("head_fused: more than 2 GiB of encoder output (32-bit buffer offsets)"); return -1; }
  unsigned* ticket = (unsigned*)scratch;
  double* slots = scratch ? (double*)((char*)scratch + 256) : nullptr;
  hipLaunchKernelGGL((head_dots_kernel<KC>), dim3(grid), dim3(256), lds, s, x, rows, w, N, dots, mom, rpg, slots, ticket,
                     mom ? head_slots_per_group(rows, rpg) : 0);
  SVT_LAUNCH_CHECK();
  return 0;
}
int launch_head_fused(const float* x, int64_t rows, int K, const float* w, const float* wsum, const float* b, int N, float* dots,
                      double* mom , int64_t rows_per_group, float eps, float* logits,
                      FrameOut* frames, int n_oct, int n_cls, hipStream_t s, double n_stat, int (*between)(void*), void* between_arg,
                      void* scratch ) {
  if (!linear_head_eligible(K, N)) { set_error("head_fused: unsupported head geometry"); return -1; }
  if (frames && (N != 2 + n_oct + 1 + n_cls + 1 || N > 32)) { set_error("head_fused: n_out != 2 + (n_octave+1) + (n_class+1)"); return -1; }
  if (mom) {
    const int64_t groups = (rows + rows_per_group - 1) / rows_per_group;
    if (256 + (size_t)groups * head_slots_per_group(rows, rows_per_group) * 16 > head_scratch_bytes(rows, (int)groups)) { set_error("head_fused: scratch too small"); return -1; }
  }
  int r = K == 512 ? launch_head_dots_kc<2>(x, rows, w, N, dots, mom, rows_per_group, scratch, s)
        : K == 768 ? launch_head_dots_kc<3>(x, rows, w, N, dots, mom, rows_per_group, scratch, s)
                   : launch_head_dots_kc<4>(x, rows, w, N, dots, mom, rows_per_group, scratch, s);
  if (r) return r;
  if (between) { if (int rb = between(between_arg)) return rb; }
  hipLaunchKernelGGL(head_finish_kernel, dim3((unsigned)((rows + 255) / 256)), dim3(256), 0, s, dots, rows, N, wsum, b, mom,
                     rows_per_group, n_stat > 0 ? n_stat : (double)rows_per_group * (double)K, eps, logits, frames, n_oct, n_cls);
  SVT_LAUNCH_CHECK();
  return 0;
}

}
```

Measured before the change: 5941 clips/s.

## Fuse posconv add into layernorm, skip bf16 writes on last LN, faster head dots

Several side-pass optimizations are gated by a new g_side_passes flag that defaults on. The positional-conv scatter-add is fused into the first encoder layernorm, removing one fp32 round trip. The final layer's layernorm now writes only the fp32 output and skips the unused bf16 hi/lo stores. The head dot-product kernel gets an 8-rows-per-wave variant that uses permlane/DPP cross-lane reductions, and the moments kernel is unrolled. A debug entry point is added for testing these paths. The inline asm permlane instructions tie the code to gfx950, and the fused path depends on the layout and alignment conditions holding.

```diff
diff --git a/include/svt_mi355.h b/include/svt_mi355.h
--- a/include/svt_mi355.h
+++ b/include/svt_mi355.h
@@ -203,6 +203,7 @@
 int svt_debug_attention_scores(int32_t precision, const void* q, const void* k, const void* v, void* o, int32_t batch, int32_t t,
                                int32_t heads, int32_t head_dim, int64_t ldq, int64_t ldkv, int64_t ldo, float scale,
                                const float* gate_dev, const float* pos_bias_dev, int device, void* stream);
+int svt_debug_side_pass(int32_t kind, void* const* bufs, const int64_t* dims, int device, void* stream);
 int svt_debug_rca_wgrad(int32_t precision, const float* dy0, int64_t ldy0, const void* x0, const float* dy1, int64_t ldy1, const void* x1,
                         int64_t rows, int32_t n_out, int32_t n_in, float* dw, float* db, void* workspace_dev, size_t* workspace_bytes,
                         int device, void* stream);
diff --git a/svt_speechbrain_amd/_lib.py b/svt_speechbrain_amd/_lib.py
--- a/svt_speechbrain_amd/_lib.py
+++ b/svt_speechbrain_amd/_lib.py
@@ -144,6 +144,7 @@
     "svt_debug_rca_attn_bwd": (C.c_int, [C.c_int32, _P, _P, _P, _P, _P, C.c_float, C.c_int32, C.c_int32, C.c_int32, C.c_int32, _P, _P,
                                          _P, C.POINTER(C.c_size_t), C.c_int, _P]),
     "svt_debug_set": (C.c_int, [C.c_int, C.c_int]),
+    "svt_debug_side_pass": (C.c_int, [C.c_int32, C.POINTER(C.c_void_p), C.POINTER(C.c_int64), C.c_int, _P]),
     "svt_debug_clock": (C.c_int, [C.c_void_p, C.c_int, C.c_void_p]),
     "svt_debug_encoder_layout": (C.c_int, [C.c_void_p, C.c_int32, C.c_int64, C.POINTER(C.c_int64), C.c_int]),
     "svt_operand_type": (C.c_int, []),
diff --git a/svt_speechbrain_amd/csrc/api.hip b/svt_speechbrain_amd/csrc/api.hip
--- a/svt_speechbrain_amd/csrc/api.hip
+++ b/svt_speechbrain_amd/csrc/api.hip
@@ -462,6 +462,54 @@
   return rc;
 }
 
+int svt_debug_side_pass(int32_t kind, void* const* bufs, const int64_t* dims, int device, void* stream) {
+  if (!bufs || !dims) { set_error("svt_debug_side_pass: null argument"); return SVT_ERR_INVALID; }
+  if (int r = check_device(device)) return r;
+  SVT_HIP(hipSetDevice(device));
+  hipStream_t s = (hipStream_t)stream;
+  void* scratch = nullptr;
+  auto with_scratch = [&](size_t bytes) -> int {
+    if (int r = dev_alloc(&scratch, bytes)) return r;
+    if (hipMemsetAsync(scratch, 0, bytes, s) != hipSuccess) { set_error("svt_debug_side_pass: hipMemsetAsync"); return SVT_ERR_HIP; }
+    return 0;
+  };
+  int rc = 0;
+  if (kind == 1) {
+    const int groups = (int)dims[1];
+    if (groups < 1 || dims[0] < 1) { set_error("svt_debug_side_pass(1): n, groups"); return SVT_ERR_INVALID; }
+    rc = with_scratch(moments_scratch_bytes(groups));
+    if (!rc) rc = launch_moments((const float*)bufs[0], dims[0], (double*)bufs[1], scratch, groups, s, groups);
+  } else if (kind == 2) {
+    const int B = (int)dims[0], T = (int)dims[1], D = (int)dims[2], G = (int)dims[3], P = (int)dims[4];
+    if (B < 1 || T < 1 || P < 1 || !layernorm_hilo_ok(D) || G < 1 || D % G || (D / G) % 8) { set_error("svt_debug_side_pass(2): geometry"); return SVT_ERR_INVALID; }
+    const int Tq = (T + P - 1) / P;
+    if (posconv_add_layernorm_hilo_ok(D, G)) {
+      rc = launch_posconv_add_layernorm_hilo((const float*)bufs[0], (const bf16_t*)bufs[1], B, T, D, G, P, Tq, (const float*)bufs[2], (const float*)bufs[3],
+                                             1e-5f, (bf16_t*)bufs[5], (bf16_t*)bufs[6], s);
+    } else {
+      rc = launch_posconv_scatter_add((const float*)bufs[0], bufs[1], B, T, D, G, P, Tq, (float*)bufs[4], s, 0);
+      if (!rc) rc = launch_layernorm_hilo(nullptr, nullptr, nullptr, (const float*)bufs[4], (int64_t)B * T, D, (const float*)bufs[2], (const float*)bufs[3],
+                                          1e-5f, (bf16_t*)bufs[5], (bf16_t*)bufs[6], nullptr, s);
+    }
+  } else if (kind == 3) {
+    if (dims[0] < 1 || !layernorm_hilo_ok((int)dims[1])) { set_error("svt_debug_side_pass(3): geometry"); return SVT_ERR_INVALID; }
+    rc = launch_layernorm_hilo((const bf16_t*)bufs[0], (const bf16_t*)bufs[1], (const bf16_t*)bufs[2], nullptr, dims[0], (int)dims[1], (const float*)bufs[3],
+                               (const float*)bufs[4], 1e-5f, (bf16_t*)bufs[5], (bf16_t*)bufs[6], (float*)bufs[7], s, (int)dims[2]);
+  } else if (kind == 4) {
+    const int64_t rows = dims[0], rpg = dims[3];
+    if (rows < 1 || rpg < 1 || !linear_head_eligible((int)dims[1], (int)dims[2])) { set_error("svt_debug_side_pass(4): geometry"); return SVT_ERR_INVALID; }
+    rc = with_scratch(head_scratch_bytes(rows, (int)((rows + rpg - 1) / rpg)));
+    if (!rc) rc = launch_head_fused((const float*)bufs[0], rows, (int)dims[1], (const float*)bufs[1], (const float*)bufs[2], (const float*)bufs[3], (int)dims[2],
+                                    (float*)bufs[4], (double*)bufs[5], rpg, 1e-5f, (float*)bufs[6], nullptr, 0, 0, s, 0.0, nullptr, nullptr, scratch);
+  } else {
+    set_error("svt_debug_side_pass: unknown kind");
+    return SVT_ERR_INVALID;
+  }
+  (void)hipStreamSynchronize(s);
+  if (scratch) dev_free(scratch);
+  return rc ? (rc > 0 ? rc : SVT_ERR_INVALID) : SVT_OK;
+}
+
 int svt_debug_set(int key, int value) {
   if (key == 0) g_gemm_dbg = value;
   else if (key == 1) g_gemm_force_bm = value;
@@ -509,6 +557,7 @@
   else if (key == 37) { if (value < 8 || value > 256 || value % 8) { set_error("svt_debug_set(37): 8 .. 256, a multiple of 8"); return SVT_ERR_INVALID; } g_gemm_persist_wgs = value; }
   else if (key == 38) return g_flash_kernel_id;
   else if (key == 39) return g_gemm_kernel_id;
+  else if (key == 40) g_side_passes = value;
   else { set_error("svt_debug_set: unknown key"); return SVT_ERR_INVALID; }
   return SVT_OK;
 }
diff --git a/svt_speechbrain_amd/csrc/api_encoder.hip b/svt_speechbrain_amd/csrc/api_encoder.hip
--- a/svt_speechbrain_amd/csrc/api_encoder.hip
+++ b/svt_speechbrain_amd/csrc/api_encoder.hip
@@ -634,6 +634,8 @@
     g.a_pairs = pk_front ? 1 : 0;
     if (int r = launch_gemm(gp, g, s)) return r;
   }
+  bool pos_add_in_ln = false;
+  int pos_Tq = 0;
   {
     const int kp = c.pos_conv_kernel, G = c.pos_conv_groups, cg = D / G;
     const int Pf = e->pos_P;
@@ -672,6 +674,9 @@
       g.a_z2 = (long)Tp * cg; g.w_z2 = (long)g.N * g.K; g.c_z2 = (long)B * Tq * g.N; g.bias_z2 = g.N;
       g.act = ACT_GELU; g.out_f32 = 0;
       if (int r = launch_gemm(gp, g, s)) return r;
+      pos_add_in_ln = prec && !c.stable_layer_norm && c.num_layers > 0 && posconv_add_layernorm_hilo_ok(D, G);
+      pos_Tq = Tq;
+      if (!pos_add_in_ln)
       if (int r = launch_posconv_scatter_add(w.hF, w.posy, B, (int)T, D, G, Pf, Tq, w.preF, s, prec ? 0 : 1)) return r;
     } else {
     if (int r = launch_posconv_gather(prec, w.hF, B, (int)T, D, G, kp, (int)T + kp, w.posg, s, bn_sc, bn_sh)) return r;
@@ -732,6 +737,10 @@
   if (!c.stable_layer_norm && prec && layernorm_hilo_ok(D) && c.num_layers > 0) {
     bf16_t* xh = (bf16_t*)w.xb;
     bf16_t* xl = (bf16_t*)w.xlo;
+    if (pos_add_in_ln) {
+      if (int r = launch_posconv_add_layernorm_hilo(w.hF, (const bf16_t*)w.posy, B, (int)T, D, c.pos_conv_groups, e->pos_P, pos_Tq,
+                                                    e->enc_g.as<float>(), e->enc_b.as<float>(), eps, xh, xl, s)) return r;
+    } else
     if (int r = launch_layernorm_hilo(nullptr, nullptr, nullptr, w.preF, rows, D, e->enc_g.as<float>(), e->enc_b.as<float>(), eps,
                                       xh, xl, nullptr, s)) return r;
     bool ffn2_split = false;
@@ -760,7 +769,7 @@
       }
       if (int r = gemm_rows(w.ffn, F, Lw.w2, Lw.b2, D, tmp, 0, ACT_NONE, nullptr)) return r;
       if (int r = launch_layernorm_hilo((const bf16_t*)tmp, xh, xl, nullptr, rows, D, Lw.ln2g.as<float>(), Lw.ln2b.as<float>(), eps,
-                                        xh, xl, last ? w.xF : nullptr, s)) return r;
+                                        xh, xl, last ? w.xF : nullptr, s, last ? 1 : 0)) return r;
     }
     final_x = w.xF;
   } else if (!c.stable_layer_norm && pk_enc) {
diff --git a/svt_speechbrain_amd/csrc/common.h b/svt_speechbrain_amd/csrc/common.h
--- a/svt_speechbrain_amd/csrc/common.h
+++ b/svt_speechbrain_amd/csrc/common.h
@@ -260,6 +260,7 @@
 extern int g_gemm_persist_wgs;
 extern int g_gemm_kernel_id;
 
+extern int g_side_passes;
 extern int g_ln_two_rows;
 extern int g_flash_wide;
 extern int g_flash_kernel_id;
@@ -307,7 +308,11 @@
 int launch_layernorm_hilo_parts(const float* parts, int nparts, long part_stride, const float* pbias, const bf16_t* rh, const bf16_t* rl, int64_t rows,
                                 int D, const float* gamma, const float* beta, float eps, bf16_t* yh, bf16_t* yl, float* yF, hipStream_t s);
 int launch_layernorm_hilo(const bf16_t* branch, const bf16_t* rh, const bf16_t* rl, const float* x32, int64_t rows, int D,
-                          const float* gamma, const float* beta, float eps, bf16_t* yh, bf16_t* yl, float* yF, hipStream_t s);
+                          const float* gamma, const float* beta, float eps, bf16_t* yh, bf16_t* yl, float* yF, hipStream_t s,
+                          int f32_only = 0);
+bool posconv_add_layernorm_hilo_ok(int D, int G);
+int launch_posconv_add_layernorm_hilo(const float* h, const bf16_t* y, int B, int T, int D, int G, int P, int Tq, const float* gamma,
+                                      const float* beta, float eps, bf16_t* yh, bf16_t* yl, hipStream_t s);
 
 int launch_conv0_group_apply(int prec, const float* wav, int B, int64_t L, int k, int stride, int64_t T1, int C,
                              const float* coef, void* out , hipStream_t s, int pair_kind = 0);
diff --git a/svt_speechbrain_amd/csrc/layernorm.hip b/svt_speechbrain_amd/csrc/layernorm.hip
--- a/svt_speechbrain_amd/csrc/layernorm.hip
+++ b/svt_speechbrain_amd/csrc/layernorm.hip
@@ -244,7 +244,7 @@
   }
 }
 
-template <int D, bool PARTS = false>
+template <int D, bool PARTS = false, bool F32_ONLY = false>
 __global__ __launch_bounds__(256) void layernorm_hilo2_kernel(const bf16_t* branch, const bf16_t* rh, const bf16_t* rl,
                                                               int64_t rows, const float* gamma, const float* beta, float eps,
                                                               bf16_t* yh, bf16_t* yl, float* yF, const float* parts = nullptr, int nparts = 0,
@@ -308,12 +308,36 @@
       oh[i] = (bf16_t)o[i];
       ol[i] = (bf16_t)(o[i] - (float)oh[i]);
     }
-    *(bf16x8*)(yh + row * D + c) = oh;
-    *(bf16x8*)(yl + row * D + c) = ol;
+    if constexpr (!F32_ONLY) {
+      *(bf16x8*)(yh + row * D + c) = oh;
+      *(bf16x8*)(yl + row * D + c) = ol;
+    }
     if (yF) {
       *(float4*)(yF + row * D + c) = float4{o[0], o[1], o[2], o[3]};
       *(float4*)(yF + row * D + c + 4) = float4{o[4], o[5], o[6], o[7]};
     }
+  }
+}
+template <int VPT>
+__device__ __forceinline__ void ln_row_to_hilo(float (&v)[VPT], float s, int lane, int64_t row, const float* gamma, const float* beta, float eps,
+                                               bf16_t* yh, bf16_t* yl) {
+  constexpr int D = 64 * VPT, NV = VPT / 4;
+  const float mean = wave_sum(s) * (1.f / D);
+  float q = 0.f;
+#pragma unroll
+  for (int i = 0; i < VPT; ++i) { v[i] -= mean; q = fmaf(v[i], v[i], q); }
+  const float rstd = rsqrtf(wave_sum(q) * (1.f / D) + eps);
+#pragma unroll
+  for (int j = 0; j < NV; ++j) {
+    const int c = (lane + 64 * j) * 4;
+    const float4 g = *(const float4*)(gamma + c), b = *(const float4*)(beta + c);
+    const float o[4] = {fmaf(v[4 * j] * rstd, g.x, b.x), fmaf(v[4 * j + 1] * rstd, g.y, b.y),
+                        fmaf(v[4 * j + 2] * rstd, g.z, b.z), fmaf(v[4 * j + 3] * rstd, g.w, b.w)};
+    bf16x4 oh, ol;
+#pragma unroll
+    for (int i = 0; i < 4; ++i) { oh[i] = (bf16_t)o[i]; ol[i] = (bf16_t)(o[i] - (float)oh[i]); }
+    *(bf16x4*)(yh + row * D + c) = oh;
+    *(bf16x4*)(yl + row * D + c) = ol;
   }
 }
 template <int VPT>
@@ -331,23 +355,31 @@
     v[4 * j] = t.x; v[4 * j + 1] = t.y; v[4 * j + 2] = t.z; v[4 * j + 3] = t.w;
     s += (t.x + t.y) + (t.z + t.w);
   }
-  const float mean = wave_sum(s) * (1.f / D);
-  float q = 0.f;
-#pragma unroll
-  for (int i = 0; i < VPT; ++i) { v[i] -= mean; q = fmaf(v[i], v[i], q); }
-  const float rstd = rsqrtf(wave_sum(q) * (1.f / D) + eps);
-#pragma unroll
-  for (int j = 0; j < NV; ++j) {
-    const int c = (lane + 64 * j) * 4;
-    const float4 g = *(const float4*)(gamma + c), b = *(const float4*)(beta + c);
-    const float o[4] = {fmaf(v[4 * j] * rstd, g.x, b.x), fmaf(v[4 * j + 1] * rstd, g.y, b.y),
-                        fmaf(v[4 * j + 2] * rstd, g.z, b.z), fmaf(v[4 * j + 3] * rstd, g.w, b.w)};
-    bf16x4 oh, ol;
-#pragma unroll
-    for (int i = 0; i < 4; ++i) { oh[i] = (bf16_t)o[i]; ol[i] = (bf16_t)(o[i] - (float)oh[i]); }
-    *(bf16x4*)(yh + row * D + c) = oh;
-    *(bf16x4*)(yl + row * D + c) = ol;
-  }
+  ln_row_to_hilo<VPT>(v, s, lane, row, gamma, beta, eps, yh, yl);
+}
+template <int VPT>
+__global__ __launch_bounds__(256) void posconv_add_layernorm_hilo_kernel(const float* h, const bf16_t* y, int B, int T, int G, int P, int Tq,
+                                                                         const float* gamma, const float* beta, float eps, bf16_t* yh, bf16_t* yl) {
+  constexpr int D = 64 * VPT, NV = VPT / 4;
+  const int lane = threadIdx.x & 63;
+  const int64_t row = (int64_t)blockIdx.x * 4 + (threadIdx.x >> 6);
+  if (row >= (int64_t)B * T) return;
+  const int cg = D / G;
+  const int t = (int)(row % T), b = (int)(row / T);
+  const int q = t / P, jf = t - q * P;
+  float v[VPT];
+  float s = 0.f;
+#pragma unroll
+  for (int j = 0; j < NV; ++j) {
+    const int ch = (lane + 64 * j) * 4;
+    const int g = ch / cg, c = ch - g * cg;
+    const bf16x4 a = *(const bf16x4*)(y + (((int64_t)g * B + b) * Tq + q) * (P * cg) + jf * cg + c);
+    const float4 hv = ((const float4*)(h + row * D))[lane + 64 * j];
+    const float4 t4 = float4{hv.x + (float)a[0], hv.y + (float)a[1], hv.z + (float)a[2], hv.w + (float)a[3]};
+    v[4 * j] = t4.x; v[4 * j + 1] = t4.y; v[4 * j + 2] = t4.z; v[4 * j + 3] = t4.w;
+    s += (t4.x + t4.y) + (t4.z + t4.w);
+  }
+  ln_row_to_hilo<VPT>(v, s, lane, row, gamma, beta, eps, yh, yl);
 }
 }
 bool layernorm_hilo_ok(int D) { return D == 512 || D == 768 || D == 1024; }
@@ -362,11 +394,13 @@
   return 0;
 }
 int launch_layernorm_hilo(const bf16_t* branch, const bf16_t* rh, const bf16_t* rl, const float* x32, int64_t rows, int D,
-                          const float* gamma, const float* beta, float eps, bf16_t* yh, bf16_t* yl, float* yF, hipStream_t s) {
+                          const float* gamma, const float* beta, float eps, bf16_t* yh, bf16_t* yl, float* yF, hipStream_t s,
+                          int f32_only) {
   const dim3 grid((unsigned)((rows + 3) / 4)), grid2((unsigned)((rows + 7) / 8)), block(256);
   ln_width(D, [&](auto vpt) {
     constexpr int VPT = decltype(vpt)::value;
     if (x32) hipLaunchKernelGGL((layernorm_f32_to_hilo_kernel<VPT>), grid, block, 0, s, x32, rows, gamma, beta, eps, yh, yl);
+    else if (f32_only && yF && g_side_passes && g_ln_two_rows && aligned(15, branch, rh, rl, yF, gamma, beta)) hipLaunchKernelGGL((layernorm_hilo2_kernel<64 * VPT, false, true>), grid2, block, 0, s, branch, rh, rl, rows, gamma, beta, eps, yh, yl, yF);
     else if (g_ln_two_rows && aligned(15, branch, rh, rl, yh, yl, yF, gamma, beta)) hipLaunchKernelGGL((layernorm_hilo2_kernel<64 * VPT>), grid2, block, 0, s, branch, rh, rl, rows, gamma, beta, eps, yh, yl, yF);
     else hipLaunchKernelGGL((layernorm_hilo_kernel<VPT>), grid, block, 0, s, branch, rh, rl, rows, gamma, beta, eps, yh, yl, yF);
   });
@@ -374,4 +408,16 @@
   return 0;
 }
 
-}
+bool posconv_add_layernorm_hilo_ok(int D, int G) { return g_side_passes && layernorm_hilo_ok(D) && G > 0 && D % G == 0 && (D / G) % 4 == 0; }
+int launch_posconv_add_layernorm_hilo(const float* h, const bf16_t* y, int B, int T, int D, int G, int P, int Tq, const float* gamma,
+                                      const float* beta, float eps, bf16_t* yh, bf16_t* yl, hipStream_t s) {
+  if (!posconv_add_layernorm_hilo_ok(D, G) || P < 1 || !aligned(15, h, gamma, beta) || !aligned(7, y, yh, yl)) { set_error("posconv + layernorm: geometry / alignment"); return -1; }
+  const dim3 grid((unsigned)(((int64_t)B * T + 3) / 4)), block(256);
+  ln_width(D, [&](auto vpt) {
+    hipLaunchKernelGGL((posconv_add_layernorm_hilo_kernel<decltype(vpt)::value>), grid, block, 0, s, h, y, B, T, G, P, Tq, gamma, beta, eps, yh, yl);
+  });
+  SVT_LAUNCH_CHECK();
+  return 0;
+}
+
+}
diff --git a/svt_speechbrain_amd/csrc/stats.hip b/svt_speechbrain_amd/csrc/stats.hip
--- a/svt_speechbrain_amd/csrc/stats.hip
+++ b/svt_speechbrain_amd/csrc/stats.hip
@@ -29,7 +29,10 @@
   return 0;
 }
 
+int g_side_passes = 1;
+
 namespace {
+template <int U>
 __global__ __launch_bounds__(256) void moments_kernel(const float* x, int64_t n, double* mom, double* part, unsigned* ticket) {
   __shared__ double sh[2][4];
   x += (int64_t)blockIdx.y * n;
@@ -40,12 +43,18 @@
   const float4* x4 = (const float4*)x;
   int64_t i = (int64_t)blockIdx.x * blockDim.x + threadIdx.x;
   const int64_t stride = (int64_t)gridDim.x * blockDim.x;
-  for (; i < n4; i += stride) {
-    const float4 v = x4[i];
-    const float a = (v.x + v.y) + (v.z + v.w);
-    const float b = (v.x * v.x + v.y * v.y) + (v.z * v.z + v.w * v.w);
-    s += (double)a;
-    ss += (double)b;
+  for (; i < n4; i += U * stride) {
+    float4 v[U];
+#pragma unroll
+    for (int j = 0; j < U; ++j) v[j] = i + j * stride < n4 ? x4[i + j * stride] : float4{0.f, 0.f, 0.f, 0.f};
+#pragma unroll
+    for (int j = 0; j < U; ++j) {
+      if (i + j * stride >= n4) break;
+      const float a = (v[j].x + v[j].y) + (v[j].z + v[j].w);
+      const float b = (v[j].x * v[j].x + v[j].y * v[j].y) + (v[j].z * v[j].z + v[j].w * v[j].w);
+      s += (double)a;
+      ss += (double)b;
+    }
   }
   if (blockIdx.x == 0 && threadIdx.x == 0) {
     for (int64_t j = n4 << 2; j < n; ++j) { s += (double)x[j]; ss += (double)x[j] * (double)x[j]; }
@@ -108,7 +117,8 @@
   if (moments_ticket_bytes(groups_max) + (size_t)gx * groups * 2 * sizeof(double) > moments_scratch_bytes(groups_max)) { set_error("moments: scratch too small"); return -1; }
   unsigned* ticket = (unsigned*)scratch;
   double* part = (double*)((char*)scratch + moments_ticket_bytes(groups_max));
-  hipLaunchKernelGGL(moments_kernel, dim3(gx, groups), dim3(256), 0, s, x, n, moments, part, ticket);
+  if (g_side_passes) hipLaunchKernelGGL(moments_kernel<8>, dim3(gx, groups), dim3(256), 0, s, x, n, moments, part, ticket);
+  else hipLaunchKernelGGL(moments_kernel<1>, dim3(gx, groups), dim3(256), 0, s, x, n, moments, part, ticket);
   SVT_LAUNCH_CHECK();
   return 0;
 }
@@ -242,6 +252,36 @@
 }
 
 namespace {
+__device__ __forceinline__ void head_group_moments(int64_t rows, int64_t rows_per_group, int NW, const double* slots, int slots_per_group,
+                                                   double* mom, int lane, int wave) {
+  const int64_t n_groups = (rows + rows_per_group - 1) / rows_per_group;
+  for (int64_t g = wave; g < n_groups; g += 4) {
+    const int64_t a = g * rows_per_group, b = (g + 1) * rows_per_group < rows ? (g + 1) * rows_per_group : rows;
+    const int64_t nj = ((b - 1) >> 2) - (a >> 2) + 1;
+    const int n = (int)(nj < NW ? nj : NW);
+    const double* sl = slots + (size_t)g * slots_per_group * 2;
+    double ta = 0.0, tq = 0.0;
+    int i = lane;
+    for (; i + 15 * 64 < n; i += 16 * 64) {
+      double va[16], vq[16];
+#pragma unroll
+      for (int j = 0; j < 16; ++j) { va[j] = ld_partial(sl + 2 * (i + 64 * j)); vq[j] = ld_partial(sl + 2 * (i + 64 * j) + 1); }
+#pragma unroll
+      for (int j = 0; j < 16; ++j) { ta += va[j]; tq += vq[j]; }
+    }
+    for (; i + 3 * 64 < n; i += 4 * 64) {
+      double va[4], vq[4];
+#pragma unroll
+      for (int j = 0; j < 4; ++j) { va[j] = ld_partial(sl + 2 * (i + 64 * j)); vq[j] = ld_partial(sl + 2 * (i + 64 * j) + 1); }
+#pragma unroll
+      for (int j = 0; j < 4; ++j) { ta += va[j]; tq += vq[j]; }
+    }
+    for (; i < n; i += 64) { ta += ld_partial(sl + 2 * i); tq += ld_partial(sl + 2 * i + 1); }
+    ta = wave_sum(ta);
+    tq = wave_sum(tq);
+    if (lane == 0) { mom[2 * g] = ta; mom[2 * g + 1] = tq; }
+  }
+}
 template <int KC>
 __global__ __launch_bounds__(256) void head_dots_kernel(const float* __restrict__ x, int64_t rows, const float* __restrict__ w, int N,
                                                         float* __restrict__ dots, double* __restrict__ mom, int64_t rows_per_group,
@@ -358,6 +398,129 @@
   }
 }
 
+__device__ __forceinline__ float fold_swap32(float a, float b) {
+  asm("s_nop 1\n\tv_permlane32_swap_b32 %0, %1\n\ts_nop 1" : "+v"(a), "+v"(b));
+  return a + b;
+}
+__device__ __forceinline__ float fold_swap16(float a, float b) {
+  asm("s_nop 1\n\tv_permlane16_swap_b32 %0, %1\n\ts_nop 1" : "+v"(a), "+v"(b));
+  return a + b;
+}
+__device__ __forceinline__ float mul_rn(float a, float b) {
+  float r;
+  asm("v_mul_f32 %0, %1, %2" : "=v"(r) : "v"(a), "v"(b));
+  return r;
+}
+template <int CTRL> __device__ __forceinline__ float dpp_of(float v) {
+  return __builtin_bit_cast(float, __builtin_amdgcn_update_dpp(0, __builtin_bit_cast(int, v), CTRL, 0xf, 0xf, false));
+}
+template <int KC>
+__global__ __launch_bounds__(256) void head_dots_rows8_kernel(const float* __restrict__ x, int64_t rows, const float* __restrict__ w, int N,
+                                                              float* __restrict__ dots, double* __restrict__ mom, int64_t rows_per_group,
+                                                              double* __restrict__ slots, unsigned* __restrict__ ticket, int slots_per_group) {
+  constexpr int K = KC * 256;
+  extern __shared__ __attribute__((aligned(16))) float wl[];
+  const int lane = threadIdx.x & 63, wave = threadIdx.x >> 6;
+  const bool hi8 = (lane & 8) != 0;
+  const int NW = (int)gridDim.x * 4, W = (int)blockIdx.x * 4 + wave;
+  const int64_t step = (int64_t)NW * 4;
+  float4 xv[8][KC];
+  const auto xrs = __builtin_amdgcn_make_buffer_rsrc((void*)x, 0, 0x7FFFFFF0, 0x00020000);
+  auto load_rows = [&](int64_t r0) {
+#pragma unroll
+    for (int rr = 0; rr < 8; ++rr) {
+      const int64_t r = r0 + (rr >> 2) * step + (rr & 3);
+      const int64_t row = r < rows ? r : rows - 1;
+#pragma unroll
+      for (int c = 0; c < KC; ++c) {
+        typedef float f4v __attribute__((ext_vector_type(4)));
+        const f4v t = __builtin_bit_cast(f4v, __builtin_amdgcn_raw_buffer_load_b128(xrs, (unsigned)((row * K + c * 256 + lane * 4) * 4), 0, 0));
+        xv[rr][c] = float4{t[0], t[1], t[2], t[3]};
+      }
+    }
+  };
+  if ((int64_t)W * 4 < rows) load_rows((int64_t)W * 4);
+  for (int i = threadIdx.x * 4; i < N * K; i += 1024) *(float4*)(wl + i) = *(const float4*)(w + i);
+  __syncthreads();
+  int64_t cur_g = -1, g_end = 0;
+  float la = 0.f, lq = 0.f;
+  auto flush = [&]() {
+    if (cur_g < 0) return;
+    const double sa = wave_sum((double)la), sq = wave_sum((double)lq);
+    if (lane == 0) {
+      const int64_t ja = (cur_g * rows_per_group) >> 2;
+      const int p = (int)(((W - ja) % NW + NW) % NW);
+      double* sl = slots + ((size_t)cur_g * slots_per_group + p) * 2;
+      st_partial(sl, sa);
+      st_partial(sl + 1, sq);
+    }
+    la = 0.f; lq = 0.f;
+  };
+  for (int64_t r0 = (int64_t)W * 4; r0 < rows; r0 += 2 * step) {
+    if (r0 != (int64_t)W * 4) load_rows(r0);
+    if (mom) {
+#pragma unroll
+      for (int rr = 0; rr < 8; ++rr) {
+        const int64_t r = r0 + (rr >> 2) * step + (rr & 3);
+        if (r >= rows) break;
+        if (r >= g_end || cur_g < 0) {
+          flush();
+          cur_g = r / rows_per_group;
+          g_end = (cur_g + 1) * rows_per_group;
+        }
+        float a = 0.f, q = 0.f;
+#pragma unroll
+        for (int c = 0; c < KC; ++c) {
+          const float4 v = xv[rr][c];
+          a += (v.x + v.y) + (v.z + v.w);
+          q += (mul_rn(v.x, v.x) + mul_rn(v.y, v.y)) + (c == 0 ? fmaf(v.z, v.z, mul_rn(v.w, v.w)) : mul_rn(v.z, v.z) + mul_rn(v.w, v.w));
+        }
+        la += a;
+        lq += q;
+      }
+    }
+    float out[4] = {0.f, 0.f, 0.f, 0.f};
+    for (int n = 0; n < N; ++n) {
+      float sacc[8] = {0.f, 0.f, 0.f, 0.f, 0.f, 0.f, 0.f, 0.f};
+#pragma unroll
+      for (int c = 0; c < KC; ++c) {
+        const float4 wv = *(const float4*)(wl + n * K + c * 256 + lane * 4);
+#pragma unroll
+        for (int rr = 0; rr < 8; ++rr) {
+          sacc[rr] = fmaf(xv[rr][c].x, wv.x, sacc[rr]);
+          sacc[rr] = fmaf(xv[rr][c].y, wv.y, sacc[rr]);
+          sacc[rr] = fmaf(xv[rr][c].z, wv.z, sacc[rr]);
+          sacc[rr] = fmaf(xv[rr][c].w, wv.w, sacc[rr]);
+        }
+      }
+      float k[4], m[2];
+#pragma unroll
+      for (int i = 0; i < 4; ++i) k[i] = fold_swap32(sacc[i], sacc[4 + i]);
+#pragma unroll
+      for (int i = 0; i < 2; ++i) m[i] = fold_swap16(k[i], k[2 + i]);
+      float v = (hi8 ? m[1] : m[0]) + dpp_of<0x128>(hi8 ? m[0] : m[1]);
+      v += __builtin_bit_cast(float, __builtin_amdgcn_ds_swizzle(__builtin_bit_cast(int, v), 0x101F));
+      v += dpp_of<0x4E>(v);
+      v += dpp_of<0xB1>(v);
+      const bool mine = (lane & 7) == (n & 7);
+#pragma unroll
+      for (int q = 0; q < 4; ++q) out[q] = (mine && (n >> 3) == q) ? v : out[q];
+    }
+    const int myrow = ((lane >> 5) & 1) * 4 + ((lane >> 4) & 1) * 2 + ((lane >> 3) & 1);
+    const int64_t row = r0 + (myrow >> 2) * step + (myrow & 3);
+    if (row < rows) {
+#pragma unroll
+      for (int q = 0; q < 4; ++q)
+        if ((lane & 7) + 8 * q < N) dots[row * N + (lane & 7) + 8 * q] = out[q];
+    }
+  }
+  if (mom) {
+    flush();
+    if (!last_workgroup(ticket, gridDim.x)) return;
+    head_group_moments(rows, rows_per_group, NW, slots, slots_per_group, mom, lane, wave);
+  }
+}
+
 __global__ void head_finish_kernel(const float* __restrict__ dots, int64_t rows, int N, const float* __restrict__ wsum,
                                    const float* __restrict__ bias, const double* __restrict__ mom, int64_t rows_per_group,
                                    double group_elems, float eps, float* __restrict__ logits, FrameOut* __restrict__ frames,
@@ -419,14 +582,17 @@
 static int launch_head_dots_kc(const float* x, int64_t rows, const float* w, int N, float* dots, double* mom, int64_t rpg, void* scratch,
                                hipStream_t s) {
   const size_t lds = (size_t)N * KC * 256 * 4;
-  if (int r_ = ensure_dyn_lds((const void*)head_dots_kernel<KC>, 32 * KC * 256 * 4)) return r_;
+  const bool rows8 = g_side_passes != 0;
+  if (int r_ = ensure_dyn_lds(rows8 ? (const void*)head_dots_rows8_kernel<KC> : (const void*)head_dots_kernel<KC>, 32 * KC * 256 * 4)) return r_;
   const unsigned grid = head_dots_grid(rows);
   if (mom && (!scratch || ((uintptr_t)scratch & 7))) { set_error("head_fused: scratch"); return -1; }
   if ((unsigned long)rows * KC * 256 * 4 > 0x7FFFFFF0ul) { set_error("head_fused: more than 2 GiB of encoder output (32-bit buffer offsets)"); return -1; }
   unsigned* ticket = (unsigned*)scratch;
   double* slots = scratch ? (double*)((char*)scratch + 256) : nullptr;
-  hipLaunchKernelGGL((head_dots_kernel<KC>), dim3(grid), dim3(256), lds, s, x, rows, w, N, dots, mom, rpg, slots, ticket,
-                     mom ? head_slots_per_group(rows, rpg) : 0);
+  if (rows8) hipLaunchKernelGGL((head_dots_rows8_kernel<KC>), dim3(grid), dim3(256), lds, s, x, rows, w, N, dots, mom, rpg, slots, ticket,
+                                mom ? head_slots_per_group(rows, rpg) : 0);
+  else hipLaunchKernelGGL((head_dots_kernel<KC>), dim3(grid), dim3(256), lds, s, x, rows, w, N, dots, mom, rpg, slots, ticket,
+                          mom ? head_slots_per_group(rows, rpg) : 0);
   SVT_LAUNCH_CHECK();
   return 0;
 }
```

Result: no change. 5981 clips/s (median of 6 runs) (+0.7%).
